# ooshyun/Speech-Enhancement-Pytorch

Measured on AMD Instinct MI355X. Metric: audio-sec/sec training, DCCRN 16kHz 2s bs32, higher is better.
Workload: dtype bf16; 1 GPU; DCCRN (kernel_num 16-32-64-128-256-256, complex LSTM 128, mask E) train step, 16 kHz 2-s clips, SI-SNR, Adam 3e-4, clip 5; per_gpu_batch=32, global_batch=32, samples_per_clip=32000, parallelism=dp1, launch=eager, inputs=resident in HBM

## Files before the change

### include/sehip.h

```cpp
#ifndef SEHIP_H
#define SEHIP_H
#include <stdint.h>

#ifdef __cplusplus
extern "C" {
#endif

const char* sehip_last_error(void);
const char* sehip_last_kernel(void);
int sehip_version(void);
int sehip_check_device(int device);

void* sehip_event_create(void);
int sehip_event_destroy(void* event);
int sehip_stream_depend(void* to_stream, void* from_stream, void* event);
int sehip_event_record(void* event, void* stream);
int sehip_stream_wait_event(void* stream, void* event);
void* sehip_stream_create(int priority_class);
int sehip_stream_destroy(void* stream);

int sehip_stft_frames(int n_samples, int win_len, int hop);
int sehip_stft_fwd(const float* wav , const float* window , int B, int N, int win_len, int hop,
                   int fft_len, float* spec , void* enc_in_bf16 , void* stream);
int sehip_istft_fwd(const float* spec, const float* mask , const float* window,
                    const float* inv_coff , int B, int T, int win_len, int hop, int fft_len, int length,
                    int masking_mode , float* frames_ws , float* wav ,
                    void* stream);
int sehip_istft_bwd(const float* dwav, const float* wav, const float* spec, const float* mask, const float* window,
                    const float* inv_coff, int B, int T, int win_len, int hop, int fft_len, int length,
                    int masking_mode, void* dmask_bf16 , void* stream);

int sehip_stft_custom_frames(int n_samples, int n_fft, int hop, int center);
int sehip_stft_custom_fwd(const float* wav, int rows, int n_samples, int n_fft, int hop, int win_length, int center,
                          float* spec, void* stream);
int sehip_istft_custom_fwd(const float* spec, int rows, int n_frames, int n_fft, int hop, int win_length, int center,
                           int length, float* frames_ws, float* wav, void* stream);

int sehip_wav_row_stats(const float* raw, const long* row_off, int rows, float* stats, void* stream);
int sehip_wav_collate(const float* raw, const long* row_off, const int* out_row, const long* out_start, const int* out_valid,
                      const float* stats, int mode, float eps, int seg, int out_rows, float* out, void* stream);

long sehip_resample_out_len(long n, int old_sr, int new_sr);
int sehip_resample_frac(const float* raw, const long* row_off, int rows, const float* kernels, int old_sr, int new_sr, int width,
                        float* out, const long* out_off, void* stream);

int sehip_sisnr_fwd(const float* est, const float* ref, int rows, int n, float* rowstat, float* loss, void* stream);
int sehip_sisdr_metric(const float* reference, const float* estimation, int rows, int n, float* ratios, float* out, void* stream);
int sehip_sisnr_bwd(const float* est, const float* ref, const float* rowstat, const float* upstream ,
                    int rows, int n, float* dest, void* stream);

int sehip_sisnr_pit_fwd(const float* est, const float* ref, int B, int S, int C, int n, float* rowstat, float* pairloss,
                        int* perm, float* loss, void* stream);
int sehip_sisnr_pit_bwd(const float* est, const float* ref, const float* rowstat, const int* perm, const float* upstream ,
                        int B, int S, int C, int n, float* dest, void* stream);

int sehip_pit_pointwise_blocks(int B, int S, int C, int n);
int sehip_pit_pointwise_fwd(const float* est, const float* ref, int B, int S, int C, int n, int mode, float* partials,
                            float* pairloss, int* perm, float* loss, void* stream);
int sehip_pit_pointwise_bwd(const float* est, const float* ref, const int* perm, const float* upstream ,
                            int B, int S, int C, int n, int mode, float* dest, void* stream);

int sehip_psa_loss_fwd(const float* enh, const float* tgt, const float* mix, long ncomplex, double* acc, float* loss, void* stream);
int sehip_psa_loss_bwd(const float* enh, const float* tgt, const float* mix, long ncomplex, const float* upstream, float* denh, void* stream);
int sehip_pointwise_loss_fwd(const float* x, const float* y, long n, int mode, double* acc_scratch, float* loss, void* stream);
int sehip_pointwise_loss_bwd(const float* x, const float* y, long n, int mode, const float* upstream, float* dx, void* stream);

int sehip_grad_sumsq(const float* grads, long n, double* sumsq_out, void* stream);
int sehip_opt_step(float* params, float* grads, float* m, float* v, long n, const double* sumsq, float max_norm,
                   float lr, float beta1, float beta2, float eps, int step, const int* step_dev ,
                   float weight_decay, int mode, float grad_scale, void* stream);
int sehip_opt_step_g(float* params, float* grads, float* m, float* v, long n, const double* sumsq, float max_norm,
                     float lr, float beta1, float beta2, float eps, int step, const int* step_dev, float weight_decay, int mode,
                     float grad_scale, const unsigned* guard, void* stream);
int sehip_opt_step_m(float* params, float* grads, float* m, float* v, long n, const double* sumsq, float max_norm, float lr,
                     float beta1, float beta2, float eps, int step, const int* step_dev, float weight_decay, int mode,
                     float grad_scale, const unsigned* guard, const float* tensor_sums, int ntensors, float* metric,
                     double* next_sumsq, float* next_tensor_sums, void* stream);
int sehip_opt_begin_g(int* counter, int value, double* sumsq, float* tensor_sums, int ntensors, const unsigned* guard, void* stream);
int sehip_counter_add(int* counter, int value, void* stream);
int sehip_zero_regions(void* p0, long b0, void* p1, long b1, void* p2, long b2, void* p3, long b3, void* stream);
int sehip_init(void);
int sehip_grad_metric(const float* grads, const long* offsets , int ntensors, long max_tensor_numel,
                      const double* sumsq,
                      float* tensor_sums , float* metric , void* stream);
int sehip_opt_begin(int* counter, int value, double* sumsq, float* tensor_sums, int ntensors, void* stream);
int sehip_grad_sumsq_acc(const float* grads, long n, double* sumsq_out, void* stream);
int sehip_grad_metric_acc(const float* grads, const long* offsets, int ntensors, long max_tensor_numel, const double* sumsq,
                          float* tensor_sums, float* metric, void* stream);

int sehip_comm_unique_id(void* id128);
int sehip_comm_init(const void* id128, int world, int rank, void** comm_out);
int sehip_allreduce_f32(void* comm, float* buf, long n, void* stream);
int sehip_allreduce_i32_max(void* comm, int* buf, long n, void* stream);
int sehip_comm_info(void* comm, int* nranks, int* rank, int* device);
int sehip_comm_destroy(void* comm);

typedef struct {
    const void* ptr;
    int32_t T;
    int32_t tlo, thi;
    int32_t F;
    int32_t C;
    int32_t pad_;
} sehip_src;

typedef struct {
    int32_t src;
    int32_t toff;
    int32_t fadd;
    int32_t coff;
} sehip_kchunk;

typedef struct {
    void* ptr;
    int32_t T, F, C;
    int32_t toff;
    int32_t fmul, fadd;
    int32_t is_f32;
    int32_t tmul;
} sehip_dst;

typedef struct {
    int32_t dst;
    int32_t coff;
    int32_t nvalid;
    int32_t pad_;
} sehip_nchunk;

typedef struct {
    sehip_src src[4];
    sehip_dst dst[2];
    const sehip_kchunk* ktab;
    const sehip_nchunk* ntab;
    const void* W;
    const float* bias;
    float* dW;
    float* dbias;
    int32_t M, N, Npad, K;
    int32_t TT, J, fmul;
    int32_t tmul;
    int32_t cv_nf, cv_fadd;
    int32_t cv_toff[2][2];
    const void* res;
    float* stats;
    int32_t stats_cr;
    int32_t cv2_nkt, cv2_nf, cv2_fadd, cv2_t0;
    int32_t w_tiled;
    int32_t wg_hint;
    int32_t dense_rows;
    int64_t dw_split_stride;
    const void* bn_dz;
    const void* bn_y;
    const float* bn_coef;
    const float* bn_bcoef;
    const float* bn_slope;
    const void* bnr_y;
    const float* bnr_coef;
    const float* bnr_slope;
    float* bnr_part;
    double* gln_stats;
    const float* gln_slope;
} sehip_gemm_desc;

int sehip_gemm_desc_size(void);
int sehip_bnr_rows(const sehip_gemm_desc* a, const sehip_gemm_desc* b );
int sehip_gemm_takes_gln_stats(const sehip_gemm_desc* desc);
int sehip_set_deterministic(int on);
int sehip_get_deterministic(void);
int sehip_gemm(const sehip_gemm_desc* desc, void* stream);
int sehip_gemm_pair(const sehip_gemm_desc* a, const sehip_gemm_desc* b, void* stream);
int sehip_conv_small_takes(const sehip_gemm_desc* a, const sehip_gemm_desc* b );
int sehip_wgrad(const sehip_gemm_desc* desc, void* stream);
int sehip_wgrad_pair(const sehip_gemm_desc* a, const sehip_gemm_desc* b, void* stream);
long sehip_wgrad_group_bytes(int n);
int sehip_wgrad_group_prepare(const sehip_gemm_desc* descs, int n, void* dev_buf, int* total_blocks);
int sehip_wgrad_group(const void* dev_buf, int n, int total_blocks, void* stream);
long sehip_wgrad_dense_group_bytes(int n);
int sehip_wgrad_dense_group_prepare(const sehip_gemm_desc* descs, int n, void* dev_buf, long dev_bytes, int* info);
int sehip_wgrad_dense_group(const void* dev_buf, int n, const int* info, float* scratch, void* stream);

int sehip_pack_bf16(const float* params, const int* table, long n, void* out_bf16, void* stream);
int sehip_pack_f32(const float* params, const int* table2 , long n, float* out, void* stream);
int sehip_pack_head(const float* params, const int* wtable, long nw, void* wout_bf16, const int* btable2, long nb, float* bout,
                    float* zero, long nz, void* stream);
int sehip_unpack_grad(const float* packed, const int* table4 , long n, float* grads, void* stream);
int sehip_unpack_grad_sums(const float* packed, const int* table4, long n, float* grads, const long* offsets, int ntensors,
                           double* sumsq, float* tensor_sums, int* counter, const unsigned* guard, void* stream);
int sehip_unpack_grad_sums_perm(const float* packed, const int* table4, const int* perm, long n, float* grads, const long* offsets,
                                int ntensors, double* sumsq, float* tensor_sums, int* counter, const unsigned* guard, void* stream);
int sehip_unpack_grad1_sums(const float* packed, const int* table1, long n, float* grads, const long* offsets, int ntensors, double* sumsq,
                            float* tensor_sums, int* counter, const unsigned* guard, void* stream);
int sehip_unpack_grad_list_sums(const float* packed, const int* list, const int* table4, long m, float* grads, const long* offsets,
                                int ntensors, double* sumsq, float* tensor_sums, void* stream);
int sehip_unpack_grad1(const float* packed, const int* table1, long n, float* grads, void* stream);
int sehip_unpack_grad_list(const float* packed, const int* list, const int* table4, long m, float* grads, void* stream);
int sehip_pack_bf16_runs(const float* params, const int* runs2 , const int* side, long n, void* out_bf16, void* stream);
int sehip_pack_bf16_runs_to(const float* params, const int* runs2 , const int* dst_run , const int* side, long n,
                            void* out_base, void* stream);

long sehip_cbn_scratch_floats(long rows, int Cr);
int sehip_cbn_stats(const void* y, long rows, int Cr, float* part, void* stream);
int sehip_cbn_finalize(const float* part, const float* Wrr, const float* Wri, const float* Wii, const float* Br,
                       const float* Bi, float* RMr, float* RMi, float* RVrr, float* RVri, float* RVii, long* nbt,
                       long rows, int Cr, float eps, float momentum, int training, float* coef , void* stream);
int sehip_cbn_finalize_n(const float* part, int nblk, const float* Wrr, const float* Wri, const float* Wii, const float* Br,
                       const float* Bi, float* RMr, float* RMi, float* RVrr, float* RVri, float* RVii, long* nbt,
                       long rows, int Cr, float eps, float momentum, int training, float* coef , void* stream);
int sehip_cbn_apply(const void* y, const float* coef, const float* slope, long rows, int Cr, void* z, void* stream);
int sehip_cbn_finalize_apply_n(const void* y, const float* part, int nblk, const float* Wrr, const float* Wri, const float* Wii,
                               const float* Br, const float* Bi, float* RMr, float* RMi, float* RVrr, float* RVri, float* RVii,
                               long* nbt, long rows, int Cr, float eps, float momentum, int training, float* coef ,
                               const float* slope, void* z, void* stream);
int sehip_cbn_bwd_reduce(const void* dz, const void* dz2 , const void* y, const float* coef, const float* slope,
                         long rows, int Cr, int F, int Tst, int tfirst, float* part, void* stream);
int sehip_cbn_bwd_finalize(const float* part, const float* coef, const float* Wrr, const float* Wri, const float* Wii,
                           long rows, int Cr, float* gWrr, float* gWri, float* gWii, float* gBr, float* gBi, float* gslope,
                           float* bcoef , void* stream);
int sehip_cbn_bwd_finalize_n(const float* part, int nblk, const float* coef, const float* Wrr, const float* Wri, const float* Wii,
                             long rows, int Cr, float* gWrr, float* gWri, float* gWii, float* gBr, float* gBi, float* gslope,
                             float* bcoef , void* stream);
int sehip_cbn_bwd_fused(const void* dz, const void* dz2 , const void* y, const float* coef, const float* Wrr, const float* Wri,
                        const float* Wii, const float* slope, long rows, int Cr, int F, int Tst, int tfirst, float* rep, float* rep_next,
                        int nrep,
                        float* gWrr, float* gWri, float* gWii, float* gBr, float* gBi, float* gslope, void* dy, void* stream);
int sehip_cbn_bwd_reduce_fin(const void* dz, const void* dz2 , const void* y, const float* coef, const float* Wrr,
                             const float* Wri, const float* Wii, const float* slope, long rows, int Cr, int F, int Tst, int tfirst,
                             float* rep, int nrep, unsigned* ticket, float* gWrr, float* gWri, float* gWii, float* gBr, float* gBi,
                             float* gslope, float* bcoef , void* stream);
int sehip_cbn_bwd_apply(const void* dz, const void* dz2, const void* y, const float* coef, const float* bcoef,
                        const float* slope, long rows, int Cr, int F, int Tst, int tfirst, void* dy, void* stream);

long sehip_rbn_scratch_floats(long rows, int Cs);
int sehip_rbn_stats(const void* y, long rows, int Cs, int Cr, float* part, void* stream);
int sehip_rbn_finalize(const float* part, const float* w_re, const float* b_re, const float* w_im, const float* b_im, float* rm_re,
                       float* rv_re, float* rm_im, float* rv_im, long* nbt_re, long* nbt_im, long rows, int Cs, int Cr, float eps,
                       float momentum, int training, float* coef, void* stream);
int sehip_rbn_finalize_s(const float* part, const float* w_re, const float* b_re, const float* w_im, const float* b_im, float* rm_re,
                         float* rv_re, float* rm_im, float* rv_im, long* nbt_re, long* nbt_im, long rows, int Cs, int Cr, float eps,
                         float momentum, int training, const float* shift, float* coef, void* stream);
int sehip_rbn_apply(const void* y, const float* coef, long rows, int Cs, int Cr, void* z, void* stream);
int sehip_rbn_bwd_reduce(const void* dz, const void* y, const float* coef, long rows, int Cs, int Cr, float* part, void* stream);
int sehip_rbn_bwd_reduce_fin(const void* dz, const void* y, const float* coef, long rows, int Cs, int Cr, float* part, unsigned* ticket,
                             float* gw_re, float* gb_re, float* gw_im, float* gb_im, float* bcoef, void* stream);
int sehip_rbn_bwd_finalize(const float* part, const float* coef, long rows, int Cs, int Cr, float* gw_re, float* gb_re, float* gw_im,
                           float* gb_im, float* bcoef, void* stream);
int sehip_rbn_bwd_apply(const void* dz, const void* y, const float* coef, const float* bcoef, long rows, int Cs, int Cr, void* dy,
                        void* stream);

int sehip_dcunet_pack_input(const float* spec, int R, int F, int T, void* out_bf16, void* stream);
int sehip_dcunet_mask_fwd(const void* z_bf16, const float* w_re, const float* w_im, const float* b_re, const float* b_im,
                          const float* spec, int R, int F, int T, int Cs, int Cr, int mode, float* mask_ws, float* out, void* stream);
int sehip_dcunet_mask_bwd(const float* dout, const float* spec, const float* mask_ws, const void* z_bf16, const float* w_re,
                          const float* w_im, int R, int F, int T, int Cs, int Cr, int mode, void* dz_bf16, float* gacc, void* stream);
int sehip_dcunet_mask_fwd_bn(const void* y_bf16, const float* coef, const float* w_re, const float* w_im, const float* b_re,
                             const float* b_im, const float* spec, int R, int F, int T, int Cs, int Cr, int mode, float* mask_ws,
                             float* out, void* stream);
long sehip_dcunet_tail_scratch_floats(int R, int F, int T, int Cs);
int sehip_dcunet_tail_bwd(const float* dout, const float* spec, float* mask_ws, const void* y_bf16, const float* coef, const float* w_re,
                          const float* w_im, int R, int F, int T, int Cs, int Cr, int mode, float* scratch, float* gw_re, float* gb_re,
                          float* gw_im, float* gb_im, float* bcoef, void* dy_bf16, float* gacc, void* stream);

int sehip_ctn_encoder_fwd(const float* wav, const float* U, const float* gamma, const float* beta, int M, int ac, int T, int N, int L,
                          float* w, void* cln_bf16, void* stream);
long sehip_ctn_codec_bwd_scratch_floats(int M, int K, int N, int L, int ac);
int sehip_ctn_encoder_bwd(const float* wav, const float* w, const void* dcln_bf16, const float* dw_dec, const float* gamma, int M, int ac,
                          int T, int N, int L, float* gacc, float* scratch, void* stream);
int sehip_ctn_gln_stats(const void* h, const float* slope, int M, int K, int C, double* stats, void* stream);
int sehip_ctn_dwconv_fwd(const void* h1, const float* slope1, const double* stats1, const float* gamma, const float* beta, const float* Wd,
                         int P, int dilation, const float* slope2, int M, int K, int C, void* h2, double* stats2, void* stream);
int sehip_ctn_gln_apply(const void* h, const float* slope, const double* stats, const float* gamma, const float* beta, int M, int K, int C,
                        void* u, void* stream);
long sehip_ctn_gln_bwd_scratch_floats(int M, int K, int C);
int sehip_ctn_gln_bwd(const void* g, const void* h, const float* slope, const double* stats, const float* gamma, const float* beta,
                      const float* Wd, int P, int dilation, int dw, int M, int K, int C, double* sums, float* gch, void* dh, float* dslope,
                      float* scratch, void* stream);
int sehip_ctn_dwconv_fwd_causal(const void* h1, const float* slope1, const double* stats1, const float* gamma, const float* beta,
                                const float* Wd, int P, int dilation, const float* slope2, int M, int K, int C, void* h2, double* stats2,
                                void* stream);
int sehip_ctn_gln_bwd_causal(const void* g, const void* h, const float* slope, const double* stats, const float* gamma, const float* beta,
                             const float* Wd, int P, int dilation, int dw, int M, int K, int C, double* sums, float* gch, void* dh,
                             float* dslope, float* scratch, void* stream);
int sehip_ctn_cln_apply(const void* h, const float* slope, const float* gamma, const float* beta, int M, int K, int C, void* u, void* stream);
int sehip_ctn_cln_dwconv_fwd(const void* h1, const float* slope1, const float* gamma, const float* beta, const float* Wd, int P,
                             int dilation, int causal, int M, int K, int C, void* h2, void* stream);
long sehip_ctn_cln_bwd_scratch_floats(int M, int K, int C);
int sehip_ctn_cln_bwd(const void* g, const void* h, const float* slope, const float* gamma, const float* beta, const float* Wd, int P,
                      int dilation, int dw, int causal, int M, int K, int C, float* gch, void* dh, float* dslope, float* scratch,
                      void* stream);
int sehip_ctns_encoder(const float* x, float* carry, const int* phase, const float* U, const float* gamma, const float* beta, int S, int ac,
                       int Kc, int N, int L, float* w, void* cln_bf16, void* stream);
int sehip_ctns_dwconv(const void* h1, void* hist, const int* phase, const int* pos, const float* slope1, const float* gamma,
                      const float* beta, const float* Wd, int P, int dilation, int S, int Kc, int C, void* h2, void* stream);
int sehip_ctns_decoder(const float* w, const void* mask_bf16, const float* V, float* tail, const int* phase, const int* pos, int S, int Kc,
                       int N, int L, int ac, int Cs, float* out, void* stream);
int sehip_ctns_advance(int* pos, int* phase, int S, int Kc, void* stream);
int sehip_dcs_analysis(const float* x, float* carry, const int* phase, const float* window, int S, int Kc, int win, int hop, float* spec,
                       float* ring, void* enc_bf16, void* enc_hist_bf16, void* stream);
int sehip_dcs_norm_hist(const void* y, const float* coef, const float* slope, void* hist, const int* phase, const int* pos, const int* end,
                        int lag, int S, int Kc, int H, int F, int Cr, void* z, void* stream);
int sehip_dcs_lstm_carry(void* h_bf16, float* c, int S, int Kc, int hidden, void* stream);
int sehip_dcs_synthesis(const float* spec, const float* ring, const float* mask, const float* window, const float* inv_coff, float* tail,
                        const int* phase, const int* pos, const int* end, int S, int Kc, int win, int hop, int mode, float* frames_ws,
                        float* out, void* stream);
int sehip_dcs_mark_end(const int* pos, int* end, int S, int extra, void* stream);
int sehip_dcs_advance(int* pos, int* phase, int S, int Kc, void* stream);
int sehip_ctn_mask_softmax_fwd(const void* score_bf16, long rows, int Cs, int N, void* out_bf16, void* stream);
int sehip_ctn_mask_softmax_bwd(const void* soft_bf16, void* g_bf16, long rows, int Cs, int N, void* stream);
int sehip_ctn_decoder_fwd(const float* w, const void* mlin_bf16, const float* V, int M, int K, int N, int L, int ac, int Cs, int T,
                          float* out, void* stream);
int sehip_ctn_decoder_bwd(const float* dout, const float* w, const void* mlin_bf16, const float* V, int M, int K, int N, int L, int ac,
                          int Cs, int T, void* dmlin_bf16, float* dw_dec, float* gacc, float* scratch, void* stream);

int sehip_lstm_fwd(const float* pre_r, const float* pre_i, const void* whh_bf16 , int B, int T, int hidden,
                   void* h_bf16, void* gates_bf16, float* c, void* stream);
int sehip_lstm_bwd(const void* dh_a_bf16, const void* dh_b_bf16, const void* whhT_bf16 ,
                   const void* gates_bf16, const float* c, int B, int T, int hidden, void* dpre_r_bf16, void* dpre_i_bf16,
                   void* stream);
int sehip_lstm_fwd_chunk(const float* pre_r, const float* pre_i, const void* whh_bf16, int B, int T, int hidden, int t0, int t1,
                         void* h_bf16, void* gates_bf16, float* c, void* stream);
int sehip_lstm_bwd_chunk(const void* dh_a_bf16, const void* dh_b_bf16, const void* whhT_bf16, const void* gates_bf16,
                         const float* c, int B, int T, int hidden, int t0, int t1, float* state, void* dpre_r_bf16,
                         void* dpre_i_bf16, void* stream);
int sehip_rlstm_fwd(const float* pre, const void* whh_bf16, int B, int T, int hidden, void* h_bf16, void* gates_bf16, float* c, void* stream);
int sehip_rlstm_bwd(const void* dh_bf16, const void* whhT_bf16, const void* gates_bf16, const float* c, int B, int T, int hidden,
                    void* dpre_bf16, void* stream);
long sehip_lstm2_gran_bytes(int B, int T, int backward);
int sehip_lstm2_sync_bytes(void);
int sehip_lstm2_fwd(const float* pre_r, const float* pre_i, const void* whh1, const void* whh2, const void* wih2, const float* bias2,
                    int B, int T, int hidden, void* h1, void* gates1, float* c1, void* h2, void* gates2, float* c2, void* gran,
                    unsigned* sync, unsigned epoch, void* stream);
int sehip_lstm2_bwd(const void* dh_a, const void* dh_b, const void* whhT1, const void* whhT2, const void* wihT2, const void* gates1,
                    const float* c1, const void* gates2, const float* c2, int B, int T, int hidden, void* dpre1_r, void* dpre1_i,
                    void* dpre2_r, void* dpre2_i, void* gran, unsigned* sync, unsigned epoch, void* stream);

int sehip_dmx_prep(const float* mix, int B, int ac, int acp, int T, int padl, int Tv, int normalize, int up, const float* kup, int width,
                   int KL, double* acc , float* ms, void* x_bf16, void* stream);
int sehip_dmx_post(const float* y, const float* ms, int B, int co, int cop, long Tf, int padl, int T, int down, const float* kdn, int width,
                   int KL, float* out, void* stream);
int sehip_dmx_post_bwd(const float* dout, const float* ms, int B, int co, int cop, long Tf, int padl, int T, int down, const float* kdn,
                       int width, int KL, void* dy_bf16, void* stream);
int sehip_dmx_gn_stats(const void* y, int B, int T, int C, int G, double* stats, void* stream);
int sehip_dmx_act_fwd(const void* y, const double* stats, const float* gamma, const float* beta, int G, float eps, int mode,
                      const float* scale, const void* resid, const void* add, int B, int T, int C, void* out, void* stream);
int sehip_dmx_act_bwd(const void* dz, const void* y, const double* stats, const float* gamma, const float* beta, int G, float eps, int mode,
                      const float* scale, int B, int T, int C, double* sums, float* gch, void* dy, void* stream);
int sehip_dmx_add(const void* a, const void* b, long n, void* out, void* stream);
int sehip_dmx_f32_to_bf16(const float* a, long n, void* out, void* stream);
int sehip_dmx_frames(int mode, const void* a, const void* b, int B, int T, int C, int nf, int W, int S, void* out, void* stream);
int sehip_dmx_lstm_sync_bytes(void);
// ... 109 lines not shown
```

### speech-enhancement-pytorch_amd/sehip/_lib.py

```python
import ctypes as C
import os

import torch

_HERE = os.path.dirname(os.path.abspath(__file__))
LIB_PATH = os.environ.get("SEHIP_LIB") or os.path.join(_HERE, "libsehip.so")


class SehipError(RuntimeError):
    pass


_lib = None

P = C.c_void_p
I = C.c_int
L = C.c_long
F = C.c_float
U = C.c_uint
D = C.c_double

_PROTOS = {
    "sehip_version": [],
    "sehip_check_device": [I],
    "sehip_set_deterministic": [I],
    "sehip_get_deterministic": [],
    "sehip_event_create": [],
    "sehip_stream_create": [C.c_int],
    "sehip_stream_destroy": [P],
    "sehip_event_destroy": [P],
    "sehip_stream_depend": [P, P, P],
    "sehip_event_record": [P, P],
    "sehip_stream_wait_event": [P, P],
    "sehip_stft_frames": [I, I, I],
    "sehip_stft_custom_frames": [I, I, I, I],
    "sehip_stft_custom_fwd": [P, I, I, I, I, I, I, P, P],
    "sehip_istft_custom_fwd": [P, I, I, I, I, I, I, I, P, P, P],
    "sehip_comm_unique_id": [P],
    "sehip_comm_init": [P, I, I, P],
    "sehip_allreduce_f32": [P, P, L, P],
    "sehip_allreduce_i32_max": [P, P, L, P],
    "sehip_comm_info": [P, P, P, P],
    "sehip_comm_destroy": [P],
    "sehip_wav_row_stats": [P, P, I, P, P],
    "sehip_wav_collate": [P, P, P, P, P, P, I, F, I, I, P, P],
    "sehip_resample_out_len": [L, I, I],
    "sehip_resample_frac": [P, P, I, P, I, I, I, P, P, P],
    "sehip_sisnr_fwd": [P, P, I, I, P, P, P],
    "sehip_sisdr_metric": [P, P, I, I, P, P, P],
    "sehip_stoi_out_len": [L, I],
    "sehip_stoi_frames": [L],
    "sehip_stoi_segment_blocks": [I, I],
    "sehip_stoi_resample": [P, P, I, L, P, I, I, I, P, P],
    "sehip_stoi_levels": [P, I, L, P, P],
    "sehip_stoi_select": [P, I, I, P, P, P],
    "sehip_stoi_bands": [P, P, I, L, P, P, P, P],
    "sehip_stoi_segments": [P, P, I, I, I, P, P, P, P],
    "sehip_sisnr_bwd": [P, P, P, P, I, I, P, P],
    "sehip_sisnr_pit_fwd": [P, P, I, I, I, I, P, P, P, P, P],
    "sehip_sisnr_pit_bwd": [P, P, P, P, P, I, I, I, I, P, P],
    "sehip_pit_pointwise_blocks": [I, I, I, I],
    "sehip_pit_pointwise_fwd": [P, P, I, I, I, I, I, P, P, P, P, P],
    "sehip_pit_pointwise_bwd": [P, P, P, P, I, I, I, I, I, P, P],
    "sehip_psa_loss_fwd": [P, P, P, L, P, P, P],
    "sehip_psa_loss_bwd": [P, P, P, L, P, P, P],
    "sehip_pointwise_loss_fwd": [P, P, L, I, P, P, P],
    "sehip_pointwise_loss_bwd": [P, P, L, I, P, P, P],
    "sehip_grad_sumsq": [P, L, P, P],
    "sehip_opt_step": [P, P, P, P, L, P, F, F, F, F, F, I, P, F, I, F, P],
    "sehip_opt_step_g": [P, P, P, P, L, P, F, F, F, F, F, I, P, F, I, F, P, P],
    "sehip_opt_step_m": [P, P, P, P, L, P, F, F, F, F, F, I, P, F, I, F, P, P, I, P, P, P, P],
    "sehip_opt_begin_g": [P, I, P, P, I, P, P],
    "sehip_counter_add": [P, I, P],
    "sehip_zero_regions": [P, L, P, L, P, L, P, L, P],
    "sehip_gemm_takes_gln_stats": [P],
    "sehip_init": [],
    "sehip_grad_metric": [P, P, I, L, P, P, P, P],
    "sehip_opt_begin": [P, I, P, P, I, P],
    "sehip_grad_sumsq_acc": [P, L, P, P],
    "sehip_grad_metric_acc": [P, P, I, L, P, P, P, P],
    "sehip_cbn_scratch_floats": [L, I],
    "sehip_stft_fwd": [P, P, I, I, I, I, I, P, P, P],
    "sehip_istft_fwd": [P, P, P, P, I, I, I, I, I, I, I, P, P, P],
    "sehip_istft_bwd": [P, P, P, P, P, P, I, I, I, I, I, I, I, P, P],
    "sehip_gemm": [P, P],
    "sehip_gemm_pair": [P, P, P],
    "sehip_wgrad": [P, P],
    "sehip_wgrad_pair": [P, P, P],
    "sehip_bnr_rows": [P, P],
    "sehip_cbn_bwd_finalize_n": [P, I, P, P, P, P, L, I, P, P, P, P, P, P, P, P],
    "sehip_wgrad_group_bytes": [I],
    "sehip_wgrad_group_prepare": [P, I, P, P],
    "sehip_wgrad_group": [P, I, I, P],
    "sehip_wgrad_dense_group_bytes": [I],
    "sehip_wgrad_dense_group_prepare": [P, I, P, L, P],
    "sehip_wgrad_dense_group": [P, I, P, P, P],
    "sehip_gemm_desc_size": [],
    "sehip_conv_small_takes": [P, P],
    "sehip_pack_bf16": [P, P, L, P, P],
    "sehip_pack_f32": [P, P, L, P, P],
    "sehip_pack_head": [P, P, L, P, P, L, P, P, L, P],
    "sehip_unpack_grad": [P, P, L, P, P],
    "sehip_unpack_grad_sums": [P, P, L, P, P, I, P, P, P, P, P],
    "sehip_unpack_grad_sums_perm": [P, P, P, L, P, P, I, P, P, P, P, P],
    "sehip_unpack_grad1": [P, P, L, P, P],
    "sehip_unpack_grad1_sums": [P, P, L, P, P, I, P, P, P, P, P],
    "sehip_unpack_grad_list_sums": [P, P, P, L, P, P, I, P, P, P],
    "sehip_unpack_grad_list": [P, P, P, L, P, P],
    "sehip_pack_bf16_runs": [P, P, P, L, P, P],
    "sehip_pack_bf16_runs_to": [P, P, P, P, L, P, P],
    "sehip_cbn_stats": [P, L, I, P, P],
    "sehip_cbn_finalize": [P, P, P, P, P, P, P, P, P, P, P, P, L, I, F, F, I, P, P],
    "sehip_cbn_finalize_n": [P, I, P, P, P, P, P, P, P, P, P, P, P, L, I, F, F, I, P, P],
    "sehip_cbn_apply": [P, P, P, L, I, P, P],
    "sehip_cbn_finalize_apply_n": [P, P, I, P, P, P, P, P, P, P, P, P, P, P, L, I, F, F, I, P, P, P, P],
    "sehip_cbn_bwd_reduce": [P, P, P, P, P, L, I, I, I, I, P, P],
    "sehip_cbn_bwd_finalize": [P, P, P, P, P, L, I, P, P, P, P, P, P, P, P],
    "sehip_cbn_bwd_apply": [P, P, P, P, P, P, L, I, I, I, I, P, P],
    "sehip_cbn_bwd_fused": [P, P, P, P, P, P, P, P, L, I, I, I, I, P, P, I, P, P, P, P, P, P, P, P],
    "sehip_cbn_bwd_reduce_fin": [P, P, P, P, P, P, P, P, L, I, I, I, I, P, I, P, P, P, P, P, P, P, P, P],
    "sehip_rbn_scratch_floats": [L, I],
    "sehip_rbn_stats": [P, L, I, I, P, P],
    "sehip_rbn_finalize": [P, P, P, P, P, P, P, P, P, P, P, L, I, I, F, F, I, P, P],
    "sehip_rbn_finalize_s": [P, P, P, P, P, P, P, P, P, P, P, L, I, I, F, F, I, P, P, P],
    "sehip_rbn_apply": [P, P, L, I, I, P, P],
    "sehip_rbn_bwd_reduce": [P, P, P, L, I, I, P, P],
    "sehip_rbn_bwd_reduce_fin": [P, P, P, L, I, I, P, P, P, P, P, P, P, P],
    "sehip_rbn_bwd_finalize": [P, P, L, I, I, P, P, P, P, P, P],
    "sehip_rbn_bwd_apply": [P, P, P, P, L, I, I, P, P],
    "sehip_dcunet_pack_input": [P, I, I, I, P, P],
    "sehip_dcunet_mask_fwd": [P, P, P, P, P, P, I, I, I, I, I, I, P, P, P],
    "sehip_dcunet_mask_bwd": [P, P, P, P, P, P, I, I, I, I, I, I, P, P, P],
    "sehip_dcunet_mask_fwd_bn": [P, P, P, P, P, P, P, I, I, I, I, I, I, P, P, P],
    "sehip_dcunet_tail_scratch_floats": [I, I, I, I],
    "sehip_dcunet_tail_bwd": [P, P, P, P, P, P, P, I, I, I, I, I, I, P, P, P, P, P, P, P, P, P],
    "sehip_ctn_encoder_fwd": [P, P, P, P, I, I, I, I, I, P, P, P],
    "sehip_ctn_encoder_bwd": [P, P, P, P, P, I, I, I, I, I, P, P, P],
    "sehip_ctn_codec_bwd_scratch_floats": [I, I, I, I, I],
    "sehip_ctn_gln_stats": [P, P, I, I, I, P, P],
    "sehip_ctn_dwconv_fwd": [P, P, P, P, P, P, I, I, P, I, I, I, P, P, P],
    "sehip_ctn_gln_apply": [P, P, P, P, P, I, I, I, P, P],
    "sehip_ctn_gln_bwd": [P, P, P, P, P, P, P, I, I, I, I, I, I, P, P, P, P, P, P],
    "sehip_ctn_gln_bwd_scratch_floats": [I, I, I],
    "sehip_ctn_dwconv_fwd_causal": [P, P, P, P, P, P, I, I, P, I, I, I, P, P, P],
    "sehip_ctn_gln_bwd_causal": [P, P, P, P, P, P, P, I, I, I, I, I, I, P, P, P, P, P, P],
    "sehip_ctn_cln_apply": [P, P, P, P, I, I, I, P, P],
    "sehip_ctn_cln_dwconv_fwd": [P, P, P, P, P, I, I, I, I, I, I, P, P],
    "sehip_ctn_cln_bwd_scratch_floats": [I, I, I],
    "sehip_ctn_cln_bwd": [P, P, P, P, P, P, I, I, I, I, I, I, I, P, P, P, P, P],
    "sehip_ctn_mask_softmax_fwd": [P, L, I, I, P, P],
    "sehip_ctn_mask_softmax_bwd": [P, P, L, I, I, P],
    "sehip_ctn_decoder_fwd": [P, P, P, I, I, I, I, I, I, I, P, P],
    "sehip_ctn_decoder_bwd": [P, P, P, P, I, I, I, I, I, I, I, P, P, P, P, P],
    "sehip_ctns_encoder": [P, P, P, P, P, P, I, I, I, I, I, P, P, P],
    "sehip_ctns_dwconv": [P, P, P, P, P, P, P, P, I, I, I, I, I, P, P],
    "sehip_ctns_decoder": [P, P, P, P, P, P, I, I, I, I, I, I, P, P],
    "sehip_ctns_advance": [P, P, I, I, P],
    "sehip_dcs_analysis": [P, P, P, P, I, I, I, I, P, P, P, P, P],
    "sehip_dcs_norm_hist": [P, P, P, P, P, P, P, I, I, I, I, I, I, P, P],
    "sehip_dcs_lstm_carry": [P, P, I, I, I, P],
    "sehip_dcs_synthesis": [P, P, P, P, P, P, P, P, P, I, I, I, I, I, P, P, P],
    "sehip_dcs_mark_end": [P, P, I, I, P],
    "sehip_dcs_advance": [P, P, I, I, P],
    "sehip_dmx_prep": [P, I, I, I, I, I, I, I, I, P, I, I, P, P, P, P],
    "sehip_dmx_post": [P, P, I, I, I, L, I, I, I, P, I, I, P, P],
    "sehip_dmx_post_bwd": [P, P, I, I, I, L, I, I, I, P, I, I, P, P],
    "sehip_dmx_gn_stats": [P, I, I, I, I, P, P],
    "sehip_dmx_act_fwd": [P, P, P, P, I, F, I, P, P, P, I, I, I, P, P],
    "sehip_dmx_act_bwd": [P, P, P, P, P, I, F, I, P, I, I, I, P, P, P, P],
    "sehip_dmx_add": [P, P, L, P, P],
    "sehip_dmx_f32_to_bf16": [P, L, P, P],
    "sehip_dmx_frames": [I, P, P, I, I, I, I, I, I, P, P],
    "sehip_dmx_lstm_sync_bytes": [],
    "sehip_dmx_lstm_fwd": [P, P, I, I, I, P, P, P, P],
    "sehip_dmx_lstm_bwd": [P, P, P, P, I, I, I, P, P, P, P],
    "sehip_dmx_attn_fwd": [P, I, I, I, I, I, I, P, P],
    "sehip_dmx_attn_bwd_scratch_floats": [I, I, I],
    "sehip_dmx_attn_bwd": [P, P, I, I, I, I, I, I, P, P, P],
    "sehip_lstm_fwd": [P, P, P, I, I, I, P, P, P, P],
    "sehip_lstm_bwd": [P, P, P, P, P, I, I, I, P, P, P],
    "sehip_rlstm_fwd": [P, P, I, I, I, P, P, P, P],
    "sehip_rlstm_bwd": [P, P, P, P, I, I, I, P, P],
    "sehip_lstm2_gran_bytes": [I, I, I],
    "sehip_lstm2_sync_bytes": [],
    "sehip_lstm2_fwd": [P, P, P, P, P, P, I, I, I, P, P, P, P, P, P, P, P, U, P],
    "sehip_lstm2_bwd": [P, P, P, P, P, P, P, P, P, I, I, I, P, P, P, P, P, P, U, P],
    "sehip_lstm_fwd_chunk": [P, P, P, I, I, I, I, I, P, P, P, P],
    "sehip_lstm_bwd_chunk": [P, P, P, P, P, I, I, I, I, I, P, P, P, P],
    "sehip_wun_bn_scratch_floats": [L, I],
    "sehip_wun_enc0_wgrad_scratch_floats": [I, I, I],
    "sehip_wun_out_bwd_scratch_floats": [L, I],
    "sehip_wun_enc0_fwd": [P, P, P, I, I, I, P, P],
    "sehip_wun_enc0_wgrad": [P, P, I, I, I, P, P, P, P],
    "sehip_wun_bn_stats": [P, L, I, P, P],
    "sehip_wun_bn_finalize": [P, P, P, P, P, P, P, L, I, F, F, I, P, P],
    "sehip_wun_bn_apply": [P, P, L, I, P, P],
    "sehip_wun_bn_apply_up2": [P, P, I, I, I, P, P],
    "sehip_wun_up2_bwd": [P, I, I, I, P, P],
    "sehip_wun_bn_bwd_reduce": [P, P, P, P, L, I, P, P],
    "sehip_wun_bn_bwd_finalize": [P, P, L, I, P, P, P, P],
    "sehip_wun_bn_bwd_apply": [P, P, P, P, P, L, I, P, P],
    "sehip_wun_out_fwd": [P, P, P, P, L, I, P, P],
    "sehip_wun_out_bwd": [P, P, P, P, P, L, I, P, P, P, P, P],
    "sehip_rsm_sum_scratch_floats": [L, I],
    "sehip_rsm_counter_next": [P, P, P],
    "sehip_rsm_features": [P, I, I, I, I, P, P],
    "sehip_rsm_pack_w": [P, I, I, I, I, P, P],
    "sehip_rsm_gemm_nt": [P, I, P, I, I, I, I, I, P, P, I, P],
    "sehip_rsm_gemm_tn": [P, I, P, I, I, I, I, I, I, P, I, P],
    "sehip_rsm_rnn_fwd": [I, P, P, P, P, P, P, I, I, I, I, U, U, P, I, U, F, P],
    "sehip_rsm_rnn_bwd": [I, P, P, P, P, P, P, I, I, I, I, U, U, P, I, U, F, P],
    "sehip_rsm_colsum": [P, I, P, P, L, I, P, P],
    "sehip_rsm_colsum_finalize": [P, L, I, P, P, P, P, P, P],
    "sehip_rsm_bn_apply": [P, P, L, I, P, P],
    "sehip_rsm_bn_bwd_apply": [P, P, P, P, L, I, P, P],
    "sehip_rsm_mask_fwd": [P, P, I, I, I, I, I, I, P, P],
    "sehip_rsm_mask_bwd": [P, P, P, I, I, I, I, I, I, P, P],
    "sehip_rsm_elman_fwd": [P, P, P, P, I, I, I, I, P],
    "sehip_rsm_elman_bwd": [P, P, P, P, I, I, I, I, P],
    "sehip_rsm_gemm_nt_head": [P, I, P, I, I, I, I, I, P, P, I, P, I, P],
    "sehip_rsm_mask_bwd_sigmoid": [P, P, P, I, I, I, I, I, I, P, P],
    "sehip_ha_fir_fwd": [P, L, L, P, I, I, P, P, P],
    "sehip_ha_fir_adj": [P, L, L, P, I, I, P, P, P],
    "sehip_ha_compressor_ws_doubles": [L, L, I],
    "sehip_ha_compressor_fwd": [P, L, L, I, D, D, D, D, I, P, P, P, P],
    "sehip_ha_compressor_bwd": [P, P, P, L, I, P, P],
    "sehip_has_state_bytes": [L, I, I, I],
    "sehip_has_fir": [P, L, I, I, P, I, I, I, P, P, P, P, P, P],
    "sehip_has_compress": [P, L, I, I, I, P, P, D, D, D, D, I, P, P, P, P],
    "sehip_has_advance": [P, P, P, L, I, P],
    "sehip_rss_delay_frames": [I, I, I],
    "sehip_rss_state_bytes": [L, I, I, I, I],
    "sehip_rss_feed": [P, L, I, I, P, I, I, I, P, P, L, P, P],
    "sehip_rss_advance": [P, L, I, P],
    "sehip_unet_features": [P, I, I, I, I, I, P, P],
    "sehip_unet_mask_fwd": [P, P, P, I, I, I, I, I, P, P],
    "sehip_unet_mask_bwd": [P, P, I, I, I, I, I, P, P],
    "sehip_unet_bn_finalize": [P, P, P, P, P, P, P, L, I, I, F, F, I, P, P],
    "sehip_unet_bn_act": [P, P, L, I, U, U, P, I, U, F, P, P],
    "sehip_unet_bn_act_pool": [P, P, I, I, I, I, U, U, P, I, U, F, P, P, P],
    "sehip_unet_bn_bwd_reduce": [P, P, P, P, I, I, I, I, U, U, P, I, U, F, P, P],
    "sehip_unet_bn_bwd_apply": [P, P, P, P, P, I, I, I, I, U, U, P, I, U, F, P, P],
}
_RESTYPE = {"sehip_resample_out_len": C.c_long, "sehip_stoi_out_len": C.c_long,"sehip_ha_compressor_ws_doubles": C.c_long, "sehip_has_state_bytes": C.c_long, "sehip_rss_delay_frames": C.c_long, "sehip_rss_state_bytes": C.c_long, "sehip_rsm_sum_scratch_floats": C.c_long, "sehip_wun_bn_scratch_floats": C.c_long, "sehip_wun_enc0_wgrad_scratch_floats": C.c_long, "sehip_wun_out_bwd_scratch_floats": C.c_long,
            "sehip_lstm2_gran_bytes": C.c_long, "sehip_dmx_attn_bwd_scratch_floats": C.c_long, "sehip_ctn_codec_bwd_scratch_floats": C.c_long, "sehip_ctn_gln_bwd_scratch_floats": C.c_long, "sehip_ctn_cln_bwd_scratch_floats": C.c_long, "sehip_wgrad_group_bytes": C.c_long, "sehip_wgrad_dense_group_bytes": C.c_long, "sehip_cbn_scratch_floats": C.c_long, "sehip_rbn_scratch_floats": C.c_long, "sehip_dcunet_tail_scratch_floats": C.c_long, "sehip_event_create": C.c_void_p, "sehip_stream_create": C.c_void_p}


def lib():
    global _lib
    if _lib is None:
        if not os.path.exists(LIB_PATH):
            raise SehipError(
                f"{LIB_PATH} is missing: build it with `python {os.path.join(_HERE, 'build.py')}` "
                "(hipcc --offload-arch=gfx950). There is no CPU/PyTorch fallback for the HIP path.")
        _lib = C.CDLL(LIB_PATH)
        _lib.sehip_last_error.restype = C.c_char_p
        _lib.sehip_last_kernel.restype = C.c_char_p
        for name, args in _PROTOS.items():
            fn = getattr(_lib, name, None)
            if fn is None:
                continue
            fn.argtypes = args
            fn.restype = _RESTYPE.get(name, C.c_int)
    return _lib


def declared_symbols():
    return ["sehip_last_error", "sehip_last_kernel"] + list(_PROTOS)


def check(status, what=""):
    if status != 0:
        msg = lib().sehip_last_error().decode()
        raise SehipError(f"{what}: status {status}: {msg}")


def call(name, *args):
    fn = getattr(lib(), name)
    check(fn(*args), name)


def ptr(t):
    if t is None:
        return None
    assert t.is_contiguous(), "libsehip needs contiguous tensors"
    return t.data_ptr()


import threading

_tls = threading.local()


def stream():
    h = getattr(_tls, "handle", None)
    if h is not None:
        return h
    return torch.cuda.current_stream().cuda_stream


class stream_scope:

    def __enter__(self):
        self._prev = getattr(_tls, "handle", None)
        _tls.handle = torch.cuda.current_stream().cuda_stream
        return self

    def __exit__(self, *exc):
        cached = _tls.handle
        _tls.handle = self._prev
        if exc[0] is None and os.environ.get("SEHIP_DEBUG_STREAMS") and torch.cuda.current_stream().cuda_stream != cached:
            raise SehipError("stream_scope: torch's current stream changed inside the scope; library calls went to the stream "
                             "that was current at entry")
        return False


def require_gpu(t, what):
    if not t.is_cuda:
        raise SehipError(f"{what}: tensor is on {t.device}; the HIP path needs a gfx950 GPU (no CPU fallback)")
```

### speech-enhancement-pytorch_amd/sehip/csrc/loss.hip

```cpp
#include "common.h"

#define EPS 1e-8f

__device__ __forceinline__ float sisnr_residual(float x, float alpha, float s) {
    float t = alpha * s;
    asm volatile("" : "+v"(t));
    return x - t;
}

__global__ __launch_bounds__(1024) void sisnr_fwd_kernel(const float* __restrict__ est, const float* __restrict__ ref,
                                                        int n, int rows, float4* __restrict__ rowstat) {
    __shared__ float red[16];
    const int r = blockIdx.x;
    const float* x = est + (size_t)r * n;
    const float* s = ref + (size_t)r * n;
    float xs = 0.f, ss = 0.f;
    const int n4 = n >> 2;
    const float4* x4 = reinterpret_cast<const float4*>(x);
    const float4* s4 = reinterpret_cast<const float4*>(s);
    const bool vec = ((n & 3) == 0) && ((((uintptr_t)x | (uintptr_t)s) & 15) == 0);
    if (vec) {
        for (int i = threadIdx.x; i < n4; i += 1024) {
            float4 a = x4[i], b = s4[i];
            xs += a.x * b.x + a.y * b.y + a.z * b.z + a.w * b.w;
            ss += b.x * b.x + b.y * b.y + b.z * b.z + b.w * b.w;
        }
    } else {
        for (int i = threadIdx.x; i < n; i += 1024) { xs += x[i] * s[i]; ss += s[i] * s[i]; }
    }
    xs = block_sum<16>(xs, red);
    ss = block_sum<16>(ss, red);
    const float alpha = xs / (ss + EPS);
    float et = 0.f, en = 0.f, es = 0.f;
    if (vec) {
        for (int i = threadIdx.x; i < n4; i += 1024) {
            float4 a = x4[i], b = s4[i];
            float t0 = alpha * b.x, t1 = alpha * b.y, t2 = alpha * b.z, t3 = alpha * b.w;
            float e0 = sisnr_residual(a.x, alpha, b.x), e1 = sisnr_residual(a.y, alpha, b.y), e2 = sisnr_residual(a.z, alpha, b.z),
                  e3 = sisnr_residual(a.w, alpha, b.w);
            et += t0 * t0 + t1 * t1 + t2 * t2 + t3 * t3;
            en += e0 * e0 + e1 * e1 + e2 * e2 + e3 * e3;
            es += e0 * b.x + e1 * b.y + e2 * b.z + e3 * b.w;
        }
    } else {
        for (int i = threadIdx.x; i < n; i += 1024) {
            float t = alpha * s[i], e = sisnr_residual(x[i], alpha, s[i]);
            et += t * t; en += e * e; es += e * s[i];
        }
    }
    et = block_sum<16>(et, red);
    en = block_sum<16>(en, red);
    es = block_sum<16>(es, red);
    if (threadIdx.x == 0) {
        const float ratio = et / (en + EPS);
        const float l = 10.f * log10f(ratio + EPS);
        const float c = -(1.0f / rows) * 10.f / (2.302585092994046f * (ratio + EPS));
        const float q = et / ((en + EPS) * (en + EPS));
        const float a = c * (-2.f * q);
        const float b = c * (2.f * alpha * ss / ((ss + EPS) * (en + EPS)) + 2.f * q * es / (ss + EPS));
        rowstat[r] = make_float4(a, b, l, alpha);
    }
}

__global__ void sisnr_finalize_kernel(const float4* __restrict__ rowstat, int rows, float* __restrict__ loss) {
    float acc = 0.f;
    for (int i = threadIdx.x; i < rows; i += 64) acc += rowstat[i].z;
    acc = wave_sum(acc);
    if (threadIdx.x == 0) loss[0] = -acc / rows;
}

__global__ __launch_bounds__(256) void sisnr_bwd_kernel(const float* __restrict__ est, const float* __restrict__ ref,
                                                        const float4* __restrict__ rowstat, const float* __restrict__ upstream,
                                                        int n, float* __restrict__ dest) {
    const int r = blockIdx.y;
    const float4 st = rowstat[r];
    const float up = upstream ? upstream[0] : 1.f;
    const float a = st.x * up, b = st.y * up, alpha = st.w;
    const size_t base = (size_t)r * n;
    for (int i = blockIdx.x * 256 + threadIdx.x; i < n; i += gridDim.x * 256) {
        const float s = ref[base + i];
        dest[base + i] = a * sisnr_residual(est[base + i], alpha, s) + b * s;
    }
}

#define SDR_EPS 1.1920929e-07f
__global__ __launch_bounds__(256) void sisdr_metric_kernel(const float* __restrict__ ref, const float* __restrict__ est, int n,
                                                           float* __restrict__ ratios) {
    __shared__ float red[4];
    const int r = blockIdx.x;
    const float* s = ref + (size_t)r * n;
    const float* x = est + (size_t)r * n;
    float xs = 0.f, ss = 0.f;
    for (int i = threadIdx.x; i < n; i += 256) { xs += x[i] * s[i]; ss += s[i] * s[i]; }
    xs = block_sum<4>(xs, red);
    ss = block_sum<4>(ss, red);
    const float alpha = xs / (ss + SDR_EPS);
    float et = 0.f, en = 0.f;
    for (int i = threadIdx.x; i < n; i += 256) {
        const float t = alpha * s[i], e = x[i] - t;
        et += t * t; en += e * e;
    }
    et = block_sum<4>(et, red);
    en = block_sum<4>(en, red);
    if (threadIdx.x == 0) ratios[r] = et / (en + SDR_EPS);
}

__global__ void sisdr_metric_finalize_kernel(const float* __restrict__ ratios, int rows, float* __restrict__ out) {
    float acc = 0.f;
    for (int i = threadIdx.x; i < rows; i += 64) acc += ratios[i];
    acc = wave_sum(acc);
    if (threadIdx.x == 0) out[0] = 10.f * log10f(acc / rows + SDR_EPS);
}

extern "C" int sehip_sisdr_metric(const float* reference, const float* estimation, int rows, int n, float* ratios, float* out,
                                  void* stream) {
    SEHIP_REQUIRE(rows > 0 && n > 0, "sisdr_metric: empty input (rows=%d n=%d)", rows, n);
    hipStream_t st = (hipStream_t)stream;
    sisdr_metric_kernel<<<rows, 256, 0, st>>>(reference, estimation, n, ratios);
    sisdr_metric_finalize_kernel<<<1, 64, 0, st>>>(ratios, rows, out);
    SEHIP_CHECK_LAUNCH("sisdr_metric");
    return 0;
}

extern "C" int sehip_sisnr_fwd(const float* est, const float* ref, int rows, int n, float* rowstat, float* loss,
                               void* stream) {
    SEHIP_REQUIRE(rows > 0 && n > 0, "sisnr_fwd: empty input (rows=%d n=%d)", rows, n);
    hipStream_t st = (hipStream_t)stream;
    sisnr_fwd_kernel<<<rows, 1024, 0, st>>>(est, ref, n, rows, (float4*)rowstat);
    sisnr_finalize_kernel<<<1, 64, 0, st>>>((const float4*)rowstat, rows, loss);
    SEHIP_CHECK_LAUNCH("sisnr_fwd");
    return 0;
}

extern "C" int sehip_sisnr_bwd(const float* est, const float* ref, const float* rowstat, const float* upstream, int rows,
                               int n, float* dest, void* stream) {
    SEHIP_REQUIRE(rows > 0 && n > 0, "sisnr_bwd: empty input (rows=%d n=%d)", rows, n);
    dim3 grid(cdiv(n, 256 * 8), rows);
    sisnr_bwd_kernel<<<grid, 256, 0, (hipStream_t)stream>>>(est, ref, (const float4*)rowstat, upstream, n, dest);
    SEHIP_CHECK_LAUNCH("sisnr_bwd");
    return 0;
}

#define PIT_MAXS 6
__global__ __launch_bounds__(256) void sisnr_pit_rows_kernel(const float* __restrict__ est, const float* __restrict__ ref, int B, int S,
                                                             int C, int n, float4* __restrict__ rowstat) {
    __shared__ float red[4];
    const int R = B * C;
    const int r = blockIdx.x, pair = blockIdx.y;
    const int i = pair / S, j = pair - i * S;
    const int b = r / C, c = r - b * C;
    const float* x = est + (((size_t)b * S + i) * C + c) * n;
    const float* s = ref + (((size_t)b * S + j) * C + c) * n;
    float xs = 0.f, ss = 0.f;
    for (int k = threadIdx.x; k < n; k += 256) { xs += x[k] * s[k]; ss += s[k] * s[k]; }
    xs = block_sum<4>(xs, red);
    ss = block_sum<4>(ss, red);
    const float alpha = xs / (ss + EPS);
    float et = 0.f, en = 0.f, es = 0.f;
    for (int k = threadIdx.x; k < n; k += 256) {
        const float t = alpha * s[k], e = sisnr_residual(x[k], alpha, s[k]);
        et += t * t; en += e * e; es += e * s[k];
    }
    et = block_sum<4>(et, red);
    en = block_sum<4>(en, red);
    es = block_sum<4>(es, red);
    if (threadIdx.x == 0) {
        const float ratio = et / (en + EPS);
        const float l = 10.f * log10f(ratio + EPS);
        const float cc = -(1.0f / ((float)S * (float)R)) * 10.f / (2.302585092994046f * (ratio + EPS));
        const float q = et / ((en + EPS) * (en + EPS));
        const float a = cc * (-2.f * q);
        const float bb = cc * (2.f * alpha * ss / ((ss + EPS) * (en + EPS)) + 2.f * q * es / (ss + EPS));
        rowstat[(size_t)pair * R + r] = make_float4(a, bb, l, alpha);
    }
}

__device__ void pit_best_permutation(const float* m, int S, int* best) {
    int cur[PIT_MAXS];
    for (int k = 0; k < S; ++k) cur[k] = best[k] = k;
    float lmin = 1e9f;
    for (;;) {
        float l = 0.f;
        for (int j = 0; j < S; ++j) l += m[cur[j] * S + j];
        if (lmin > l) {
            lmin = l;
            for (int k = 0; k < S; ++k) best[k] = cur[k];
        }
        int k = S - 2;
        while (k >= 0 && cur[k] > cur[k + 1]) --k;
        if (k < 0) break;
        int l2 = S - 1;
        while (cur[l2] < cur[k]) --l2;
        int t = cur[k]; cur[k] = cur[l2]; cur[l2] = t;
        for (int a = k + 1, b = S - 1; a < b; ++a, --b) { t = cur[a]; cur[a] = cur[b]; cur[b] = t; }
    }
}

__global__ void sisnr_pit_select_kernel(const float4* __restrict__ rowstat, int R, int S, float* __restrict__ pairloss,
                                        int* __restrict__ perm, float* __restrict__ loss) {
    __shared__ float m[PIT_MAXS * PIT_MAXS];
    for (int pair = 0; pair < S * S; ++pair) {
        float acc = 0.f;
        for (int r = threadIdx.x; r < R; r += 64) acc += rowstat[(size_t)pair * R + r].z;
        acc = wave_sum(acc);
        if (threadIdx.x == 0) { m[pair] = -acc / R; pairloss[pair] = -acc / R; }
    }
    __syncthreads();
    if (threadIdx.x != 0) return;
    int best[PIT_MAXS];
    pit_best_permutation(m, S, best);
    float tot = 0.f;
    for (int j = 0; j < S; ++j) { perm[j] = best[j]; tot += m[best[j] * S + j]; }
    loss[0] = tot / S;
}

__global__ __launch_bounds__(256) void sisnr_pit_bwd_kernel(const float* __restrict__ est, const float* __restrict__ ref,
                                                            const float4* __restrict__ rowstat, const int* __restrict__ perm,
                                                            const float* __restrict__ upstream, int B, int S, int C, int n,
                                                            float* __restrict__ dest) {
    const int R = B * C;
    const int r = blockIdx.y, i = blockIdx.z;
    int j = 0;
    for (int k = 0; k < S; ++k)
        if (perm[k] == i) j = k;
    const int b = r / C, c = r - b * C;
    const float4 st = rowstat[(size_t)(i * S + j) * R + r];
    const float up = upstream ? upstream[0] : 1.f;
    const float a = st.x * up, bb = st.y * up, alpha = st.w;
    const size_t xb = (((size_t)b * S + i) * C + c) * n, sb = (((size_t)b * S + j) * C + c) * n;
    for (int k = blockIdx.x * 256 + threadIdx.x; k < n; k += gridDim.x * 256) {
        const float s = ref[sb + k];
        dest[xb + k] = a * sisnr_residual(est[xb + k], alpha, s) + bb * s;
    }
}

extern "C" int sehip_sisnr_pit_fwd(const float* est, const float* ref, int B, int S, int C, int n, float* rowstat, float* pairloss,
                                   int* perm, float* loss, void* stream) {
    SEHIP_REQUIRE(B > 0 && C > 0 && n > 0 && S >= 1 && S <= PIT_MAXS, "sisnr_pit_fwd: bad shape (B=%d S=%d C=%d n=%d; S <= %d)", B, S,
                  C, n, PIT_MAXS);
    hipStream_t st = (hipStream_t)stream;
    sisnr_pit_rows_kernel<<<dim3(B * C, S * S), 256, 0, st>>>(est, ref, B, S, C, n, (float4*)rowstat);
    sisnr_pit_select_kernel<<<1, 64, 0, st>>>((const float4*)rowstat, B * C, S, pairloss, perm, loss);
    SEHIP_CHECK_LAUNCH("sisnr_pit_fwd");
    return 0;
}

extern "C" int sehip_sisnr_pit_bwd(const float* est, const float* ref, const float* rowstat, const int* perm, const float* upstream,
                                   int B, int S, int C, int n, float* dest, void* stream) {
    SEHIP_REQUIRE(B > 0 && C > 0 && n > 0 && S >= 1 && S <= PIT_MAXS, "sisnr_pit_bwd: bad shape (B=%d S=%d C=%d n=%d)", B, S, C, n);
    dim3 grid(cdiv(n, 256 * 8), B * C, S);
    sisnr_pit_bwd_kernel<<<grid, 256, 0, (hipStream_t)stream>>>(est, ref, (const float4*)rowstat, perm, upstream, B, S, C, n, dest);
    SEHIP_CHECK_LAUNCH("sisnr_pit_bwd");
    return 0;
}

__global__ __launch_bounds__(256) void pointwise_loss_fwd_kernel(const float* __restrict__ x, const float* __restrict__ y, long n,
                                                                 int mode, double* __restrict__ acc) {
    __shared__ float red[4];
    float a = 0.f;
    for (long i = blockIdx.x * 256L + threadIdx.x; i < n; i += gridDim.x * 256L) {
        const float d = x[i] - y[i];
        a += mode == 0 ? fabsf(d) : d * d;
    }
    a = block_sum<4>(a, red);
    if (threadIdx.x == 0) atomicAdd(acc, (double)a);
}

__global__ void pointwise_loss_finalize_kernel(const double* __restrict__ acc, long n, float* __restrict__ loss) {
    loss[0] = (float)(acc[0] / (double)n);
}

__global__ __launch_bounds__(256) void pointwise_loss_bwd_kernel(const float* __restrict__ x, const float* __restrict__ y, long n,
                                                                 int mode, const float* __restrict__ upstream,
                                                                 float* __restrict__ dx) {
    const float up = (upstream ? upstream[0] : 1.f) / (float)n;
    for (long i = blockIdx.x * 256L + threadIdx.x; i < n; i += gridDim.x * 256L) {
        const float d = x[i] - y[i];
        dx[i] = mode == 0 ? (d > 0.f ? up : (d < 0.f ? -up : 0.f)) : 2.f * d * up;
    }
}

__device__ __forceinline__ float psa_residual(float2 e, float2 t, float2 m, float& ae) {
    const float am = tanhf(m.y / (m.x + 1e-9f)), at = tanhf(t.y / (t.x + 1e-9f));
    ae = sqrtf(e.y * e.y + e.x * e.x);
    return ae - sqrtf(t.y * t.y + t.x * t.x) * cosf(at - am);
}

__global__ __launch_bounds__(256) void psa_loss_fwd_kernel(const float2* __restrict__ enh, const float2* __restrict__ tgt,
                                                           const float2* __restrict__ mix, long n, double* __restrict__ acc) {
    __shared__ float red[4];
    float a = 0.f;
    for (long i = blockIdx.x * 256L + threadIdx.x; i < n; i += gridDim.x * 256L) {
        float ae;
        const float d = psa_residual(enh[i], tgt[i], mix[i], ae);
        a += d * d;
    }
    a = block_sum<4>(a, red);
    if (threadIdx.x == 0) atomicAdd(acc, (double)a);
}

__global__ __launch_bounds__(256) void psa_loss_bwd_kernel(const float2* __restrict__ enh, const float2* __restrict__ tgt,
                                                           const float2* __restrict__ mix, long n, const float* __restrict__ upstream,
                                                           float2* __restrict__ denh) {
    const float up = 2.f * (upstream ? upstream[0] : 1.f) / (float)n;
    for (long i = blockIdx.x * 256L + threadIdx.x; i < n; i += gridDim.x * 256L) {
        const float2 e = enh[i];
        float ae;
        const float d = psa_residual(e, tgt[i], mix[i], ae);
        const float k = ae > 0.f ? up * d / ae : 0.f;
        denh[i] = make_float2(k * e.x, k * e.y);
    }
}

extern "C" int sehip_psa_loss_fwd(const float* enh, const float* tgt, const float* mix, long ncomplex, double* acc, float* loss, void* stream) {
    SEHIP_REQUIRE(ncomplex > 0 && enh && tgt && mix, "psa_loss_fwd: bad arguments (n=%ld)", ncomplex);
    hipStream_t st = (hipStream_t)stream;
    hipError_t e = hipMemsetAsync(acc, 0, sizeof(double), st);
    SEHIP_REQUIRE(e == hipSuccess, "psa_loss_fwd: memset failed: %s", hipGetErrorString(e));
    int grid = cdiv(ncomplex, 256 * 8);
    if (grid > 1024) grid = 1024;
    if (sehip_deterministic()) grid = 1;
    psa_loss_fwd_kernel<<<grid, 256, 0, st>>>((const float2*)enh, (const float2*)tgt, (const float2*)mix, ncomplex, acc);
    pointwise_loss_finalize_kernel<<<1, 1, 0, st>>>(acc, ncomplex, loss);
    SEHIP_CHECK_LAUNCH("psa_loss_fwd");
    return 0;
}

extern "C" int sehip_psa_loss_bwd(const float* enh, const float* tgt, const float* mix, long ncomplex, const float* upstream, float* denh,
                                  void* stream) {
    SEHIP_REQUIRE(ncomplex > 0 && enh && tgt && mix && denh, "psa_loss_bwd: bad arguments (n=%ld)", ncomplex);
    int grid = cdiv(ncomplex, 256 * 4);
    if (grid > 2048) grid = 2048;
    psa_loss_bwd_kernel<<<grid, 256, 0, (hipStream_t)stream>>>((const float2*)enh, (const float2*)tgt, (const float2*)mix, ncomplex, upstream,
                                                             (float2*)denh);
    SEHIP_CHECK_LAUNCH("psa_loss_bwd");
    return 0;
}

extern "C" int sehip_pointwise_loss_fwd(const float* x, const float* y, long n, int mode, double* acc, float* loss,
                                        void* stream) {
    SEHIP_REQUIRE(n > 0 && (mode == 0 || mode == 1), "pointwise_loss_fwd: bad arguments (n=%ld mode=%d)", n, mode);
    hipStream_t st = (hipStream_t)stream;
    hipError_t e = hipMemsetAsync(acc, 0, sizeof(double), st);
    SEHIP_REQUIRE(e == hipSuccess, "pointwise_loss_fwd: memset failed: %s", hipGetErrorString(e));
    int grid = cdiv(n, 256 * 16);
    if (grid > 1024) grid = 1024;
    if (sehip_deterministic()) grid = 1;
    pointwise_loss_fwd_kernel<<<grid, 256, 0, st>>>(x, y, n, mode, acc);
    pointwise_loss_finalize_kernel<<<1, 1, 0, st>>>(acc, n, loss);
    SEHIP_CHECK_LAUNCH("pointwise_loss_fwd");
    return 0;
}

extern "C" int sehip_pointwise_loss_bwd(const float* x, const float* y, long n, int mode, const float* upstream, float* dx,
                                        void* stream) {
    SEHIP_REQUIRE(n > 0 && (mode == 0 || mode == 1), "pointwise_loss_bwd: bad arguments (n=%ld mode=%d)", n, mode);
    int grid = cdiv(n, 256 * 8);
    if (grid > 2048) grid = 2048;
    pointwise_loss_bwd_kernel<<<grid, 256, 0, (hipStream_t)stream>>>(x, y, n, mode, upstream, dx);
    SEHIP_CHECK_LAUNCH("pointwise_loss_bwd");
    return 0;
}

#define PITPW_THREADS 256
#define PITPW_CHUNK 2048L
#define PITPW_MAXBLOCKS 1024L
#define PITPW_MAXROWS (1L << 20)
#define PITPW_MAXN (0x7fffffff - 64 * 4 * PITPW_THREADS)

static long pitpw_chunk(long rows, long n) {
    long chunk = PITPW_CHUNK;
    while (rows * ((n + chunk - 1) / chunk) > PITPW_MAXBLOCKS && chunk < n) chunk *= 2;
    return chunk;
}

extern "C" int sehip_pit_pointwise_blocks(int B, int S, int C, int n) {
    if (B <= 0 || C <= 0 || n <= 0 || S < 1 || S > PIT_MAXS || (long)B * C > PITPW_MAXROWS || n > PITPW_MAXN) return 0;
    const long rows = (long)B * C, chunk = pitpw_chunk(rows, n);
    return (int)(rows * ((n + chunk - 1) / chunk));
}

template <int MODE>
__device__ __forceinline__ float pitpw_term(float e, float t) {
    const float d = e - t;
    return MODE == 0 ? fabsf(d) : d * d;
}

template <int S, int MODE, bool VEC>
__global__ __launch_bounds__(PITPW_THREADS) void pit_pointwise_pairs_kernel(const float* __restrict__ est, const float* __restrict__ ref,
                                                                            int C, int n, int chunk, float* __restrict__ partials) {
    __shared__ float red[PITPW_THREADS / 64][S * S];
    const int r = blockIdx.x, b = r / C, c = r - b * C;
    const size_t row0 = ((size_t)b * S * C + c) * n, sstride = (size_t)C * n;
    const int k0 = blockIdx.y * chunk;
    const int k1 = n - k0 < chunk ? n : k0 + chunk;
    float acc[S * S];
#pragma unroll
    for (int p = 0; p < S * S; ++p) acc[p] = 0.f;
    if (VEC) {
        for (int k = k0 + 4 * (int)threadIdx.x; k < k1; k += 4 * PITPW_THREADS) {
            float4 e[S], t[S];
#pragma unroll
            for (int i = 0; i < S; ++i) {
                e[i] = *reinterpret_cast<const float4*>(est + row0 + i * sstride + k);
                t[i] = *reinterpret_cast<const float4*>(ref + row0 + i * sstride + k);
            }
#pragma unroll
            for (int i = 0; i < S; ++i)
#pragma unroll
                for (int j = 0; j < S; ++j)
                    acc[i * S + j] += (pitpw_term<MODE>(e[i].x, t[j].x) + pitpw_term<MODE>(e[i].y, t[j].y)) +
                                      (pitpw_term<MODE>(e[i].z, t[j].z) + pitpw_term<MODE>(e[i].w, t[j].w));
        }
    } else {
        for (int k = k0 + (int)threadIdx.x; k < k1; k += PITPW_THREADS) {
            float e[S], t[S];
#pragma unroll
            for (int i = 0; i < S; ++i) {
                e[i] = est[row0 + i * sstride + k];
                t[i] = ref[row0 + i * sstride + k];
            }
#pragma unroll
            for (int i = 0; i < S; ++i)
#pragma unroll
                for (int j = 0; j < S; ++j) acc[i * S + j] += pitpw_term<MODE>(e[i], t[j]);
        }
    }
    const int w = threadIdx.x >> 6;
#pragma unroll
    for (int p = 0; p < S * S; ++p) {
        const float v = wave_sum(acc[p]);
        if ((threadIdx.x & 63) == 0) red[w][p] = v;
    }
// ... 128 lines not shown
```

### speech-enhancement-pytorch_amd/sehip/csrc/stft.hip

```cpp
#include "common.h"

#include "fft512.h"
#include "mask.h"

__global__ __launch_bounds__(256) void stft_fwd_kernel(const float* __restrict__ wav, const float* __restrict__ window,
                                                       int B, int N, int T, int win, int hop,
                                                       float2* __restrict__ spec, unsigned* __restrict__ enc_in) {
    const int lane = threadIdx.x & 63;
    const int frame = blockIdx.x * 4 + (threadIdx.x >> 6);
    if (frame >= B * T) return;
    const int b = frame / T, t = frame - b * T;
    FftTw tw;
    fft_twiddles<-1>(tw, lane);
    float re[8], im[8];
    const int pad = win - hop;
    const float* x = wav + (size_t)b * N;
#pragma unroll
    for (int r = 0; r < 8; ++r) {
        const int n = lane + 64 * r;
        const int s = t * hop + n - pad;
        float v = 0.f;
        if (n < win && s >= 0 && s < N) v = x[s] * window[n];
        re[r] = v; im[r] = 0.f;
    }
    fft512_wave<-1>(re, im, tw, lane);
    __shared__ float2 srow[4][264 + 33];
    __shared__ unsigned senc[4][256];
    const int w = threadIdx.x >> 6;
    const int k0 = 8 * brev6(lane);
    constexpr int brev3[8] = {0, 4, 2, 6, 1, 5, 3, 7};
    if (k0 <= 256) {
#pragma unroll
        for (int j = 0; j < 8; ++j) {
            const int k = k0 + brev3[j];
            if (k <= 256) {
                srow[w][k + (k >> 3)] = make_float2(re[j], im[j]);
                if (k >= 1) senc[w][k - 1] = pack_bf2(re[j], im[j]);
            }
        }
    }
    __builtin_amdgcn_fence(__ATOMIC_RELEASE, "wavefront");
    __builtin_amdgcn_wave_barrier();
    __builtin_amdgcn_fence(__ATOMIC_ACQUIRE, "wavefront");
    float2* so = spec + (size_t)frame * NBIN;
    unsigned* eo = enc_in + (size_t)frame * 256;
#pragma unroll
    for (int j = 0; j < 4; ++j) {
        const int k = lane + 64 * j;
        so[k] = srow[w][k + (k >> 3)];
    }
    if (lane == 0) so[256] = srow[w][256 + 32];
    *reinterpret_cast<uint4*>(eo + 4 * lane) = *reinterpret_cast<const uint4*>(&senc[w][4 * lane]);
}

__global__ __launch_bounds__(256) void istft_frames_kernel(const float2* __restrict__ spec, const float2* __restrict__ mask,
                                                           const float* __restrict__ window, int nframes, int win, int mode,
                                                           float* __restrict__ frames) {
    const int lane = threadIdx.x & 63;
    const int frame = blockIdx.x * 4 + (threadIdx.x >> 6);
    if (frame >= nframes) return;
    FftTw tw;
    fft_twiddles<1>(tw, lane);
    float re[8], im[8];
    const float2* sp = spec + (size_t)frame * NBIN;
    const float2* mk = mask + (size_t)frame * 256;
#pragma unroll
    for (int r = 0; r < 8; ++r) {
        const int k = lane + 64 * r;
        float er = 0.f, ei = 0.f;
        if (k >= 1 && k <= 256) {
            const float2 z = sp[k];
            const float2 m = mk[k - 1];
            apply_mask(mode, z.x, z.y, m.x, m.y, er, ei);
        }
        re[r] = er; im[r] = ei;
    }
    fft512_wave<1>(re, im, tw, lane);
    const int n0 = 8 * brev6(lane);
    constexpr int brev3[8] = {0, 4, 2, 6, 1, 5, 3, 7};
    float u[8];
    float s1 = 0.f, s2 = 0.f;
#pragma unroll
    for (int j = 0; j < 8; ++j) {
        const int n = n0 + brev3[j];
        u[brev3[j]] = re[j];
        if (n < win) { s1 += re[j]; s2 += (n & 1) ? -re[j] : re[j]; }
    }
    s1 = wave_sum(s1);
    s2 = wave_sum(s2);
    const float c = 1.0f / (float)(FFT_N + win);
    float* fo = frames + (size_t)frame * win;
    if (n0 + 8 <= win && (win & 3) == 0) {
        float o[8];
#pragma unroll
        for (int q = 0; q < 8; ++q) {
            const int n = n0 + q;
            const float corr = c * (s1 + ((n & 1) ? -s2 : s2));
            o[q] = window[n] * (1.0f / 256.0f) * (u[q] - corr);
        }
        *reinterpret_cast<float4*>(fo + n0) = make_float4(o[0], o[1], o[2], o[3]);
        *reinterpret_cast<float4*>(fo + n0 + 4) = make_float4(o[4], o[5], o[6], o[7]);
        return;
    }
#pragma unroll
    for (int q = 0; q < 8; ++q) {
        const int n = n0 + q;
        if (n < win) {
            const float corr = c * (s1 + ((n & 1) ? -s2 : s2));
            fo[n] = window[n] * (1.0f / 256.0f) * (u[q] - corr);
        }
    }
}

__global__ __launch_bounds__(256) void istft_ola_kernel(const float* __restrict__ frames, const float* __restrict__ inv_coff,
                                                        int T, int win, int hop, int length, float* __restrict__ wav) {
    const int b = blockIdx.y;
    const int pad = win - hop;
    for (int i = blockIdx.x * 256 + threadIdx.x; i < length; i += gridDim.x * 256) {
        const int s = i + pad;
        int t_hi = s / hop;
        int t_lo = (s - win + hop) / hop;
        if (s - win + 1 <= 0) t_lo = 0;
        if (t_hi > T - 1) t_hi = T - 1;
        float acc = 0.f;
        for (int t = t_lo; t <= t_hi; ++t) acc += frames[((size_t)b * T + t) * win + (s - t * hop)];
        acc *= inv_coff[i];
        wav[(size_t)b * length + i] = fminf(1.f, fmaxf(-1.f, acc));
    }
}

__global__ __launch_bounds__(256) void istft_bwd_kernel(const float* __restrict__ dwav, const float* __restrict__ wav,
                                                        const float* __restrict__ inv_coff, const float* __restrict__ window,
                                                        const float2* __restrict__ spec, const float2* __restrict__ mask,
                                                        int B, int T, int win, int hop, int length, int mode,
                                                        unsigned* __restrict__ dmask_bf16) {
    const int lane = threadIdx.x & 63;
    const int frame = blockIdx.x * 4 + (threadIdx.x >> 6);
    if (frame >= B * T) return;
    const int b = frame / T, t = frame - b * T;
    FftTw tw;
    fft_twiddles<-1>(tw, lane);
    const int pad = win - hop;
    float re[8], im[8];
    float s1 = 0.f, s2 = 0.f;
#pragma unroll
    for (int r = 0; r < 8; ++r) {
        const int n = lane + 64 * r;
        const int i = t * hop + n - pad;
        float v = 0.f;
        if (n < win && i >= 0 && i < length) {
            const size_t o = (size_t)b * length + i;
            const float y = wav[o];
            if (y > -1.f && y < 1.f) v = dwav[o] * inv_coff[i] * window[n] * (1.0f / 256.0f);
        }
        re[r] = v; im[r] = 0.f;
        s1 += v; s2 += (n & 1) ? -v : v;
    }
    s1 = wave_sum(s1);
    s2 = wave_sum(s2);
    const float c = 1.0f / (float)(FFT_N + win);
#pragma unroll
    for (int r = 0; r < 8; ++r) {
        const int n = lane + 64 * r;
        if (n < win) re[r] -= c * (s1 + ((n & 1) ? -s2 : s2));
    }
    const float2* sp = spec + (size_t)frame * NBIN;
    const float2* mk = mask + (size_t)frame * 256;
    float2 spv[4], mkv[4];
#pragma unroll
    for (int j = 0; j < 4; ++j) { spv[j] = sp[1 + lane + 64 * j]; mkv[j] = mk[lane + 64 * j]; }
    fft512_wave<-1>(re, im, tw, lane);
    __shared__ float2 ssp[4][256 + 32], smk[4][256 + 32];
    __shared__ unsigned sdm[4][256];
    const int w = threadIdx.x >> 6;
#pragma unroll
    for (int j = 0; j < 4; ++j) {
        const int i = lane + 64 * j;
        ssp[w][i + (i >> 3)] = spv[j];
        smk[w][i + (i >> 3)] = mkv[j];
    }
    __builtin_amdgcn_fence(__ATOMIC_RELEASE, "wavefront");
    __builtin_amdgcn_wave_barrier();
    __builtin_amdgcn_fence(__ATOMIC_ACQUIRE, "wavefront");
    const int k0 = 8 * brev6(lane);
    constexpr int brev3[8] = {0, 4, 2, 6, 1, 5, 3, 7};
    if (k0 <= 256) {
#pragma unroll
        for (int j = 0; j < 8; ++j) {
            const int k = k0 + brev3[j];
            if (k < 1 || k > 256) continue;
            const float dr = re[j], di = im[j];
            const int i = k - 1;
            const float2 z = ssp[w][i + (i >> 3)];
            const float2 m = smk[w][i + (i >> 3)];
            float gmr, gmi;
            mask_grad(mode, z.x, z.y, m.x, m.y, dr, di, gmr, gmi);
            sdm[w][i] = pack_bf2(gmr, gmi);
        }
    }
    __builtin_amdgcn_fence(__ATOMIC_RELEASE, "wavefront");
    __builtin_amdgcn_wave_barrier();
    __builtin_amdgcn_fence(__ATOMIC_ACQUIRE, "wavefront");
    unsigned* dm = dmask_bf16 + (size_t)frame * 256;
    *reinterpret_cast<uint4*>(dm + 4 * lane) = *reinterpret_cast<const uint4*>(&sdm[w][4 * lane]);
}

static int check_stft_cfg(const char* who, int win, int hop, int fft) {
    SEHIP_REQUIRE(fft == FFT_N, "%s: only fft_len 512 is built (got %d)", who, fft);
    SEHIP_REQUIRE(win > 0 && win <= FFT_N && (win % 2) == 0, "%s: win_len must be even and <= 512 (got %d)", who, win);
    SEHIP_REQUIRE(hop > 0 && hop <= win, "%s: bad hop %d", who, hop);
    return 0;
}

extern "C" int sehip_stft_frames(int n_samples, int win, int hop) { return (n_samples + 2 * (win - hop) - win) / hop + 1; }

extern "C" int sehip_stft_fwd(const float* wav, const float* window, int B, int N, int win, int hop, int fft, float* spec,
                              void* enc_in_bf16, void* stream) {
    if (int e = check_stft_cfg("stft_fwd", win, hop, fft)) return e;
    SEHIP_REQUIRE(B > 0 && N > 0, "stft_fwd: empty input");
    const int T = sehip_stft_frames(N, win, hop);
    SEHIP_REQUIRE(T > 0, "stft_fwd: input shorter than one frame");
    stft_fwd_kernel<<<cdiv((long)B * T, 4), 256, 0, (hipStream_t)stream>>>(wav, window, B, N, T, win, hop, (float2*)spec,
                                                                           (unsigned*)enc_in_bf16);
    SEHIP_CHECK_LAUNCH("stft_fwd");
    return 0;
}

extern "C" int sehip_istft_fwd(const float* spec, const float* mask, const float* window, const float* inv_coff, int B,
                               int T, int win, int hop, int fft, int length, int mode, float* frames_ws, float* wav,
                               void* stream) {
    if (int e = check_stft_cfg("istft_fwd", win, hop, fft)) return e;
    SEHIP_REQUIRE(B > 0 && T > 0 && length > 0, "istft_fwd: empty input");
    SEHIP_REQUIRE(mode >= 0 && mode <= 2, "istft_fwd: masking mode must be 0(E) 1(C) 2(R)");
    SEHIP_REQUIRE(length <= (T - 1) * hop + win - (win - hop), "istft_fwd: length %d exceeds the synthesised signal", length);
    hipStream_t st = (hipStream_t)stream;
    istft_frames_kernel<<<cdiv((long)B * T, 4), 256, 0, st>>>((const float2*)spec, (const float2*)mask, window, B * T, win,
                                                             mode, frames_ws);
    dim3 grid(cdiv(length, 256 * 4), B);
    istft_ola_kernel<<<grid, 256, 0, st>>>(frames_ws, inv_coff, T, win, hop, length, wav);
    SEHIP_CHECK_LAUNCH("istft_fwd");
    return 0;
}

extern "C" int sehip_istft_bwd(const float* dwav, const float* wav, const float* spec, const float* mask,
                               const float* window, const float* inv_coff, int B, int T, int win, int hop, int fft,
                               int length, int mode, void* dmask_bf16, void* stream) {
    if (int e = check_stft_cfg("istft_bwd", win, hop, fft)) return e;
    SEHIP_REQUIRE(B > 0 && T > 0 && length > 0, "istft_bwd: empty input");
    SEHIP_REQUIRE(mode >= 0 && mode <= 2, "istft_bwd: masking mode must be 0(E) 1(C) 2(R)");
    istft_bwd_kernel<<<cdiv((long)B * T, 4), 256, 0, (hipStream_t)stream>>>(dwav, wav, inv_coff, window, (const float2*)spec,
                                                                            (const float2*)mask, B, T, win, hop, length, mode,
                                                                            (unsigned*)dmask_bf16);
    SEHIP_CHECK_LAUNCH("istft_bwd");
    return 0;
}
```

### speech-enhancement-pytorch_amd/sehip/model/dccrn.py

```python
import os
import numpy as np
import torch
from torch import nn

from .. import plan, ops
from .._lib import SehipError
from .flat import FlatModule, _Node

class DCCRN(FlatModule):
    plan_name = "DCCRN"

    def __init__(self, rnn_layers=2, rnn_units=128, win_len=400, win_inc=100, fft_len=512, length=16384, win_type="hann",
                 masking_mode="E", use_clstm=True, use_cbn=True, kernel_size=5, kernel_num=[16, 32, 64, 128, 256, 256],
                 *args, **kwargs):
        super().__init__()
        self.cfg = cfg = plan.DCCRNConfig(rnn_layers=rnn_layers, rnn_units=rnn_units, win_len=win_len, win_inc=win_inc,
                                          fft_len=fft_len, length=length, win_type=win_type, masking_mode=masking_mode,
                                          use_clstm=use_clstm, use_cbn=use_cbn, kernel_size=kernel_size,
                                          kernel_num=list(kernel_num))
        self.win_len, self.win_inc, self.fft_len, self.rnn_units = win_len, win_inc, fft_len, rnn_units
        self.masking_mode, self.kernel_num = masking_mode, cfg.kernel_num
        self.static = self._static_for(cfg)
        self.grad_range_hook = None

        an, sy, win = _stft_bases(win_len, fft_len, win_type)
        self.stft = _Node()
        self.stft.register_buffer("weight", torch.from_numpy(an[:, None, :]))
        self.istft = _Node()
        self.istft.register_buffer("weight", torch.from_numpy(sy[:, None, :]))
        self.istft.register_buffer("window", torch.from_numpy(win[None, :, None]))
        self.istft.register_buffer("enframe", torch.eye(win_len)[:, None, :])
        self._build_flat(list_roots=("encoder", "decoder"))
        self.reset_parameters()

    def _static_for(self, cfg, deterministic=False):
        switches = tuple(os.environ.get(k) for k in ("SEHIP_NO_FUSE_STATS", "SEHIP_NO_FUSE_STATS64", "SEHIP_NO_FUSE_STATS32", "SEHIP_DEC_SPLIT"))
        key = (tuple(cfg.kernel_num), cfg.rnn_layers, cfg.rnn_units, cfg.win_len, cfg.win_inc, cfg.fft_len, cfg.length, cfg.masking_mode, str(cfg.win_type), bool(cfg.use_cbn), bool(cfg.use_clstm), switches,
               bool(deterministic))
        return self._static(key, lambda: plan.DCCRNStatic(cfg, deterministic=deterministic))

    def reset_parameters(self):
        h = self.cfg.hid
        with torch.no_grad():
            for name, p in self._params:
                leaf = name.split(".")[-1]
                if "conv.weight" in name:
                    p.normal_(0.0, 0.05)
                elif "conv.bias" in name or leaf in ("Br", "Bi") or name.endswith(".1.bias"):
                    p.zero_()
                elif leaf in ("Wrr", "Wii") or name.endswith(".1.weight"):
                    p.fill_(1.0)
                elif leaf == "Wri":
                    p.uniform_(-0.9, 0.9)
                elif name.endswith("2.weight"):
                    p.fill_(0.25)
                elif "lstm" in name or name.startswith("enhance."):
                    p.uniform_(-1.0 / h ** 0.5, 1.0 / h ** 0.5)
                elif "trans" in name or name.startswith("tranform."):
                    p.uniform_(-1.0 / h ** 0.5, 1.0 / h ** 0.5)
                else:
                    raise KeyError(name)
            for name, node, leaf in self._buffers_named:
                getattr(node, leaf).fill_(1.0 if leaf in ("RVrr", "RVii", "running_var") else 0.0)
            self._nbt.zero_()

    def workspace(self, batch, nsample):
        dev = self._require_gpu()
        if self._tables is None:
            self._tables = plan.DeviceTables(self.static, dev)
        return self._lru_get((batch, nsample), lambda: plan.DCCRNWorkspace(self.static, self._tables, batch, nsample, dev))

    def set_deterministic(self, on=True):
        on = bool(on)
        if on == self.static.deterministic:
            return self
        self.static = self._static_for(self.cfg, deterministic=on)
        self._tables = None
        for ws in list(self._ws.values()):
            ws.close()
        self._ws.clear()
        self._last_ws = None
        return self

    step_guard_early = True

    def step_guard(self):
        ws = getattr(self, "_last_ws", None)
        return ws.l2_sync[0:1] if ws is not None and hasattr(ws, "l2_sync") else None

    def check_health(self):
        from ..distrib import global_flag
        ws = getattr(self, "_last_ws", None)
        if ws is None:
            return global_flag(False, self._flat.device if self._flat is not None else None)
        lost = bool(ws.check_lstm_handoffs(recover=True, global_flag=global_flag))
        self._note_graph_epoch(ws)
        return lost

    def _run_forward(self, wav):
        ws = self.workspace(wav.shape[0], wav.shape[-1])
        self._last_ws = ws
        ws.generation += 1
        x = wav.reshape(wav.shape[0], wav.shape[-1]).contiguous().float()
        ws.forward(x, self._flat, self._bflat, self._nbt, training=self.training)
        return ws

    def _output(self, ws, x):
        return ws.wav.view(x.shape[0], 1, -1).clone()

    def _run_backward(self, ws, grad_out):
        if not self.training:
            raise SehipError("DCCRN.backward in eval mode (running-statistics BatchNorm) is not built")
        g = grad_out.reshape(ws.B, ws.length).contiguous().float()
        hook = self.grad_range_hook if not (self._grads_live and self._params[0][1].grad is not None) else None
        tail = self._tail_for_backward()
        self._backward_into_flat(lambda dst: ws.backward(g, self._flat, dst, range_ready=hook, tail=tail))
        self._tail_mark(tail)

    def forward(self, inputs, lens=None):
        if inputs.dim() == 2:
            inputs = inputs.unsqueeze(1)
        return self._run_plan(inputs, torch.is_grad_enabled() and self.training)

    def get_params(self, weight_decay=0.0):
        weights, biases = [], []
        for name, p in self.named_parameters():
            (biases if "bias" in name else weights).append(p)
        return [{"params": weights, "weight_decay": weight_decay}, {"params": biases, "weight_decay": 0.0}]


def _stft_bases(win_len, fft_len, win_type="hann"):
    n = np.arange(win_len, dtype=np.float64)[None, :]
    k = np.arange(fft_len // 2 + 1, dtype=np.float64)[:, None]
    ang = 2.0 * np.pi * k * n / fft_len
    basis = np.concatenate([np.cos(ang), -np.sin(ang)], axis=0)
    win = ops.window_of(win_type, win_len).astype(np.float64)
    return ((basis * win).astype(np.float32), (np.linalg.pinv(basis).T * win).astype(np.float32), win.astype(np.float32))
```

### speech-enhancement-pytorch_amd/sehip/model/flat.py

```python
import os
from collections import OrderedDict

import numpy as np
import torch
from torch import nn

from .._lib import SehipError, stream_scope

_STATIC_CACHE = {}


class _Node(nn.Module):

    def __getitem__(self, idx):
        return getattr(self, str(idx))


def _clone_state_hook(module, state_dict, prefix, local_metadata):
    for k in list(state_dict.keys()):
        state_dict[k] = state_dict[k].detach().clone()
    return state_dict


class _PlanFunction(torch.autograd.Function):

    @staticmethod
    def forward(ctx, model, x, anchor):
        ctx.model = model
        ctx.ws = model._run_forward(x)
        ctx.generation = ctx.ws.generation
        return model._output(ctx.ws, x)

    @staticmethod
    def backward(ctx, grad_out):
        if ctx.generation != ctx.ws.generation or ctx.ws.closed:
            raise SehipError(f"{ctx.model.plan_name}.backward: the workspace of this forward was overwritten by a later forward of the same "
                             "shape (or evicted); run backward before the next forward of that shape")
        with stream_scope():
            ctx.model._run_backward(ctx.ws, grad_out)
        return None, None, None


class _EvalGuard(torch.autograd.Function):

    @staticmethod
    def forward(ctx, x, name):
        ctx.name = name
        return x.view_as(x)

    @staticmethod
    def backward(ctx, g):
        raise SehipError(f"{ctx.name}.backward in eval mode: the backward pass is built for batch statistics only (call model.train())")


class FlatModule(nn.Module):
    plan_name = None
    ws_cache_default = 4

    def _static(self, key, make):
        key = (type(self), key)
        if key not in _STATIC_CACHE:
            _STATIC_CACHE[key] = make()
        return _STATIC_CACHE[key]

    def _build_flat(self, list_roots=()):
        L = self.static.layout
        self._flat = torch.zeros(L.n_params)
        self._gflat = self._tables = None
        self._bflat = torch.zeros(max(L.n_buffers, 1))
        self._nbt = torch.zeros(len(L.nbt_names), dtype=torch.int64)
        self._ws = OrderedDict()
        self._ws_cap = max(1, int(os.environ.get("SEHIP_WS_CACHE", self.ws_cache_default)))
        self.storage_epoch = 0
        self._anchor = None
        self._grads_live = False
        self._tail_sink, self._tail_done = None, False
        self._tail_counted = self._tail_dirty = False
        for name in list_roots:
            setattr(self, name, nn.ModuleList())
        self._params, self._buffers_named, self._nbt_named = [], [], []
        for name, shape, kind in L.specs:
            parts = name.split(".")
            node = self._descend(parts[:-1])
            if kind == "param":
                off, _ = L.param_off[name]
                p = nn.Parameter(self._flat[off:off + int(np.prod(shape))].view(shape))
                node.register_parameter(parts[-1], p)
                self._params.append((name, p))
            elif kind == "buffer":
                off, _ = L.buffer_off[name]
                node.register_buffer(parts[-1], self._bflat[off:off + int(np.prod(shape))].view(shape))
                self._buffers_named.append((name, node, parts[-1]))
            else:
                node.register_buffer(parts[-1], self._nbt[L.nbt_idx[name]])
                self._nbt_named.append((name, node, parts[-1]))
        self._register_state_dict_hook(_clone_state_hook)

    def _tail_for_backward(self):
        accumulating = self._grads_live and self._params[0][1].grad is not None
        if accumulating or getattr(self, "grad_range_hook", None) is not None:
            return None
        return self._tail_sink

    def _tail_mark(self, tail):
        if tail is not None:
            self._tail_done = self._tail_counted = self._tail_dirty = True
        else:
            self._tail_done = False

    def _descend(self, parts):
        node = self
        for key in parts:
            if isinstance(node, nn.ModuleList):
                while len(node) <= int(key):
                    node.append(_Node())
                node = node[int(key)]
            else:
                if not hasattr(node, key):
                    node.add_module(key, _Node())
                node = getattr(node, key)
        return node

    def _apply(self, fn, *a, **k):
        super()._apply(fn, *a, **k)
        L = self.static.layout
        dev = self._params[0][1].device
        flat = torch.zeros(L.n_params, device=dev)
        for name, p in self._params:
            off, shape = L.param_off[name]
            v = flat[off:off + p.numel()].view(shape)
            v.copy_(p.data)
            p.data = v
            p.grad = None
        bflat = torch.zeros(max(L.n_buffers, 1), device=dev)
        for name, node, leaf in self._buffers_named:
            off, shape = L.buffer_off[name]
            v = bflat[off:off + int(np.prod(shape))].view(shape)
            v.copy_(getattr(node, leaf))
            node._buffers[leaf] = v
        nbt = torch.zeros(len(L.nbt_names), dtype=torch.int64, device=dev)
        for name, node, leaf in self._nbt_named:
            i = L.nbt_idx[name]
            nbt[i] = getattr(node, leaf).to(torch.int64)
            node._buffers[leaf] = nbt[i]
        self._flat, self._bflat, self._nbt = flat, bflat, nbt
        for ws in self._ws.values():
            ws.close()
        self._gflat, self._tables, self._ws, self._anchor, self._grads_live = None, None, OrderedDict(), None, False
        self.storage_epoch += 1
        return self

    @property
    def flat_params(self):
        return self._flat

    @property
    def flat_grads(self):
        if self._gflat is None or self._gflat.device != self._flat.device:
            self._gflat = torch.zeros_like(self._flat)
        return self._gflat

    def bind_grads(self):
        L = self.static.layout
        g = self.flat_grads
        for name, p in self._params:
            off, shape = L.param_off[name]
            p.grad = g[off:off + p.numel()].view(shape)

    def _require_gpu(self):
        dev = self._flat.device
        if dev.type != "cuda":
            raise SehipError(f"{self.plan_name} parameters are on {dev}: the HIP path needs a gfx950 GPU (no CPU fallback); "
                             "call model.to('cuda') first")
        return dev

    def _grad_anchor(self, device):
        if self._anchor is None or self._anchor.device != device:
            self._anchor = torch.zeros(1, device=device, requires_grad=True)
        return self._anchor

    def _output(self, ws, x):
        return ws.out.clone()

    def _run_plan(self, x, train_step, **forward_only):
        if not x.is_cuda:
            raise SehipError(f"{self.plan_name}.forward got a CPU tensor: the HIP path needs a gfx950 GPU (no CPU fallback)")
        if train_step:
            return _PlanFunction.apply(self, x, self._grad_anchor(x.device))
        return self._output(self._run_forward(x, **forward_only), x)

    def _eval_guarded(self, out):
        return _EvalGuard.apply(out.requires_grad_(True), self.plan_name)

    def _lru_get(self, key, make):
        ws = self._ws.get(key)
        if ws is None:
            while len(self._ws) >= self._ws_cap:
                victim = next((k for k, w in self._ws.items() if not w.pinned), None)
                if victim is None:
                    break
                self._ws.pop(victim).close()
            ws = self._ws[key] = make()
        else:
            self._ws.move_to_end(key)
        return ws

    def _note_graph_epoch(self, ws):
        ge = getattr(ws, "graph_epoch", 0)
        if ws is not None and ge != getattr(ws, "_graph_epoch_seen", 0):
            ws._graph_epoch_seen = ge
            self.storage_epoch += 1

    def _backward_into_flat(self, run):
        accumulate = self._grads_live and self._params[0][1].grad is not None
        if accumulate:
            tmp = torch.empty_like(self.flat_grads)
            run(tmp)
            self.flat_grads.add_(tmp)
        else:
            run(self.flat_grads)
        self.bind_grads()
        self._grads_live = True
```

### speech-enhancement-pytorch_amd/sehip/plan.py

```python
import ctypes as C
import os
import math

import numpy as np
import torch

from . import _lib
from ._lib import call, ptr, stream, SehipError
from . import ops
from .gemmdesc import (BF16, CSrc, CDst, CGemmDesc, ParamLayout, Arena, enc_entry, npad_of, round_up, dense_ntab, wide_chunks, pad_ktab,
                       bind_chunk_table, upload_chunk_table, row_ptr, fill_desc, wgrad_twin, UnpackTable, check_unpack_coverage)
from .workspace import Buf, GemmDeviceTables, GemmWorkspace, gather_ordered_unpack_table


FUSE_SKIP_GRAD = not os.environ.get("SEHIP_NO_FUSE_SKIP")
FUSE_ENC0_BN_WGRAD = FUSE_SKIP_GRAD and bool(os.environ.get("SEHIP_FUSE_ENC0_BN"))
BWD_REPLICAS = int(os.environ.get("SEHIP_BWD_REPLICAS", "8"))
PARALLEL_HEAD = not os.environ.get("SEHIP_NO_PARALLEL_HEAD")
L2_GRAPH_EPOCH = 65535
TILE_WEIGHTS = not any(os.environ.get(k) for k in ("SEHIP_NO_CONV_V3", "SEHIP_NO_PATCH", "SEHIP_NO_TILE_WEIGHTS"))


class DCCRNConfig:

# ... 327 lines not shown
            last = j == 5
            for p in (0, 1):
                ds = (-1, 0, 1) if p == 0 else (0, 1)
                rows = []
                cols_i, cols_n = [], []
                for kt in (0, 1):
                    for d in ds:
                        kf = p + 2 - 2 * d
                        base_t = (1 if last else 0) - kt
                        rows += wide_chunks(0, base_t + (0 if j == 0 else 1), d, 0, c1)
                        rows += wide_chunks(1, base_t, d, 0, c2)
                        cols_i += [full[cat1, :, kf, kt].T, full[cat2, :, kf, kt].T]
                        cols_n += [neg[cat1, :, kf, kt].T, neg[cat2, :, kf, kt].T]
                widx, wneg = np.concatenate(cols_i, 1), np.concatenate(cols_n, 1)
                if last:
                    nt = np.zeros((4, 4), dtype=np.int32)
                    nt[0] = (0, 0, 2, 0)
                    dst = [("mask", 0, 2, p)]
                    tt = "T"
                else:
                    nt = None
                    dst = [(f"yd{j}", 0, 2, p)]
                    tt = "T+1"
                bt = 1 if last else 0
                self.specs[f"dec{j}.fwd{p}"] = GemmSpec(f"dec{j}.fwd{p}", rows, widx, wneg, co, eff_bias(pre, co // 2), tt,
                                                        f_in, 1, [(s1, s1_mode), (s2, "all")], dst, ntab=nt,
                                                        conv=(len(ds), ds[0], [[bt + (0 if j == 0 else 1), bt - 1 + (0 if j == 0 else 1)],
                                                                               [bt, bt - 1]]))
            if not last:
                self.bn.append((pre, co // 2))
                self._maybe_fuse_stats(pre, [f"dec{j}.fwd0", f"dec{j}.fwd1"], co, [c1, c2], f_in)
                self._maybe_split_decoder(j, pre, full, neg, cat1, cat2, c1, c2, co, f_in, s1, s1_mode, s2, eff_bias(pre, co // 2))
            gsrc = "dmask" if last else f"dyd{j}"
            if co >= 8:
                rows = []
                for kt in (0, 1):
                    for kf in range(5):
                        rows += wide_chunks(0, kt, kf - 2, 0, co)
                w = full.transpose(0, 3, 2, 1).reshape(c1 + c2, -1)
                wn = neg.transpose(0, 3, 2, 1).reshape(c1 + c2, -1)
            else:
                assert co == 2
                rows, w, wn = [], np.full((c1 + c2, 32), -1, np.int64), np.zeros((c1 + c2, 32), np.int64)
                for kt in (0, 1):
                    rows += [(0, kt - 1, -2, 4), (0, kt - 1, 2, 1)]
                    for kf in range(5):
                        for c in range(2):
                            w[:, kt * 16 + kf * 2 + c] = full[:, c, kf, kt]
                            wn[:, kt * 16 + kf * 2 + c] = neg[:, c, kf, kt]
            order = np.concatenate([cat1, cat2])
            d1 = ("dP", 0, 1, 0) if j == 0 else (f"dzd{j - 1}", 1, 1, 0)
            nt = np.concatenate([dense_ntab(c1, c1, 0, 0), dense_ntab(c2, c2, 1, 0)])
            assert npad_of(c1 + c2) == c1 + c2
            self.specs[f"dec{j}.dg"] = GemmSpec(f"dec{j}.dg", rows, w[order], wn[order], c1 + c2, None, "T", f_in, 2,
                                                [(gsrc, "all")], [d1, (f"dskip{5 - j}", 0, 1, 0)], ntab=nt, kind="dgrad",
                                                conv=(5, -2, [[0, 1], [0, 0]]) if co >= 8 else (5, -2, [[-1, 0], [0, 0]]))

        c5 = kn[6]
        cp = c5 // 2
        h = cfg.hid
        lstm = ("real_lstm", "imag_lstm")

        if not cfg.use_clstm:
            def bias_pairs_real(layer):
                bp = np.empty((4 * h, 2), dtype=np.int32)
                bp[:, 0] = enc_entry(ia(f"enhance.bias_ih_l{layer}"), 0)
                bp[:, 1] = enc_entry(ia(f"enhance.bias_hh_l{layer}"), 0)
                return bp

            zero = lambda a: np.zeros_like(a)
            w1 = ia("enhance.weight_ih_l0").reshape(4 * h, c5, 4).transpose(0, 2, 1).reshape(4 * h, -1)
            rows = []
            for f in range(4):
                rows += wide_chunks(0, 0, f, 0, c5)
            self.specs["ih1"] = GemmSpec("ih1", rows, w1, zero(w1), 4 * h, bias_pairs_real(0), "T", 1, 1, [("z5", "all")],
                                         [("pre1", 0, 1, 0)])
            self.specs["dx1"] = GemmSpec("dx1", wide_chunks(0, 0, 0, 0, 4 * h), w1.T.copy(), zero(w1.T), 4 * c5, None, "T", 1, 1,
                                         [("dpre1", "all")], [("dz5l", 0, 1, 0)], kind="dgrad", res="dskip5" if FUSE_SKIP_GRAD else None)
            w2 = ia("enhance.weight_ih_l1")
            self.specs["ih2"] = GemmSpec("ih2", wide_chunks(0, 0, 0, 0, h), w2, zero(w2), 4 * h, bias_pairs_real(1), "T", 1, 1,
                                         [("h1_0", "all")], [("pre2", 0, 1, 0)])
            self.specs["dx2"] = GemmSpec("dx2", wide_chunks(0, 0, 0, 0, 4 * h), w2.T.copy(), zero(w2.T), h, None, "T", 1, 1,
                                         [("dpre2", "all")], [("dx2", 0, 1, 0)], kind="dgrad")
            tr = ia("tranform.weight")
            wt = tr.reshape(c5, 4, h).transpose(1, 0, 2).reshape(4 * c5, h)
            bp = np.full((4 * c5, 2), -1, dtype=np.int32)
            bp[:, 0] = enc_entry(ia("tranform.bias").reshape(c5, 4).T.reshape(-1), 0)
            self.specs["proj"] = GemmSpec("proj", wide_chunks(0, 0, 0, 0, h), wt, zero(wt), 4 * c5, bp, "T", 1, 1, [("h2_0", "all")],
                                          [("P", 0, 1, 0)])
            rows = []
            for d in range(4):
                rows += wide_chunks(0, 0, d, 0, c5)
            self.specs["dproj"] = GemmSpec("dproj", rows, wt.T.copy(), zero(wt.T), h, None, "T", 1, 1, [("dP", "all")],
                                           [("dxo", 0, 1, 0)], kind="dgrad")
            for layer in (1, 2):
                hh = ia(f"enhance.weight_hh_l{layer - 1}")
                self.specs[f"hh{layer}"] = GemmSpec(f"hh{layer}", wide_chunks(0, -1, 0, 0, h), hh, zero(hh), 4 * h, None, "T", 1, 1,
                                                    [(f"h{layer}_0", "all")], [(f"dpre{layer}", 0, 1, 0)],
                                                    ntab=dense_ntab(4 * h, 4 * h, 0, 0), kind="wgrad_only")
        else:
            def ih(layer, l):
                return ia(f"enhance.{layer}.{lstm[l]}.weight_ih_l0")

            def bias_pairs_lstm(layer):
                bp = np.empty((2 * 4 * h, 2), dtype=np.int32)
                for l in (0, 1):
                    bp[l * 4 * h:(l + 1) * 4 * h, 0] = enc_entry(ia(f"enhance.{layer}.{lstm[l]}.bias_ih_l0"), 0)
                    bp[l * 4 * h:(l + 1) * 4 * h, 1] = enc_entry(ia(f"enhance.{layer}.{lstm[l]}.bias_hh_l0"), 0)
                return bp

            zero = lambda a: np.zeros_like(a)
            w1 = np.concatenate([ih(0, l).reshape(4 * h, cp, 4).transpose(0, 2, 1).reshape(4 * h, -1) for l in (0, 1)])
            for q, tag in enumerate("ri"):
                rows = []
                for f in range(4):
                    rows += wide_chunks(0, 0, f, q * cp, cp)
                self.specs[f"ih1_{tag}"] = GemmSpec(f"ih1_{tag}", rows, w1, zero(w1), 8 * h, bias_pairs_lstm(0), "T", 1, 1,
                                                    [("z5", "all")], [(f"pre1_{tag}", 0, 1, 0)])
                nt = np.zeros((4 * cp // 4, 4), dtype=np.int32)
                for n4 in range(4 * cp // 4):
                    f, c = divmod(4 * n4, cp)
                    nt[n4] = (0, f * c5 + q * cp + c, 4, 0)
                self.specs[f"dx1_{tag}"] = GemmSpec(f"dx1_{tag}", wide_chunks(0, 0, 0, 0, 8 * h), w1.T.copy(), zero(w1.T), 4 * cp,
                                                    None, "T", 1, 1, [(f"dpre1_{tag}", "all")], [("dz5l", 0, 1, 0)], ntab=nt,
                                                    kind="dgrad", res="dskip5" if FUSE_SKIP_GRAD else None)
            combos = {"r": (0, 3, 1), "i": (2, 1, 0)}
            L = cfg.rnn_layers
            for tag, (ca, cb, ng) in combos.items():
                rows = wide_chunks(0, 0, 0, 0, h) + wide_chunks(1, 0, 0, 0, h)
                for layer in range(2, L + 1):
                    w2 = np.concatenate([ih(layer - 1, l) for l in (0, 1)])
                    wi = np.concatenate([w2, w2], 1)
                    wn = np.concatenate([zero(w2), zero(w2) + ng], 1)
                    self.specs[f"ih{layer}_{tag}"] = GemmSpec(f"ih{layer}_{tag}", rows, wi, wn, 8 * h, bias_pairs_lstm(layer - 1), "T", 1, 1,
                                                              [(f"h{layer - 1}_{ca}", "all"), (f"h{layer - 1}_{cb}", "all")],
                                                              [(f"pre{layer}_{tag}", 0, 1, 0)])
                    self.specs[f"dx{layer}_{tag}"] = GemmSpec(f"dx{layer}_{tag}", wide_chunks(0, 0, 0, 0, 8 * h), w2.T.copy(), zero(w2.T), h,
                                                              None, "T", 1, 1, [(f"dpre{layer}_{tag}", "all")],
                                                              [(f"dx{layer}_{tag}", 0, 1, 0)], kind="dgrad")
                q = 0 if tag == "r" else 1
                tr = ia(f"enhance.{L - 1}.{tag}_trans.weight")
                trb = ia(f"enhance.{L - 1}.{tag}_trans.bias")
                wt = tr.reshape(cp, 4, h).transpose(1, 0, 2).reshape(4 * cp, h)
                bt = trb.reshape(cp, 4).T.reshape(-1)
                bp = np.full((4 * cp, 2), -1, dtype=np.int32)
                bp[:, 0] = enc_entry(bt, 0)
                nt = np.zeros((4 * cp // 4, 4), dtype=np.int32)
                for n4 in range(4 * cp // 4):
                    d, c = divmod(4 * n4, cp)
                    nt[n4] = (0, d * c5 + q * cp + c, 4, 0)
                self.specs[f"proj_{tag}"] = GemmSpec(f"proj_{tag}", rows, np.concatenate([wt, wt], 1),
                                                     np.concatenate([zero(wt), zero(wt) + ng], 1), 4 * cp, bp, "T", 1, 1,
                                                     [(f"h{L}_{ca}", "all"), (f"h{L}_{cb}", "all")], [("P", 0, 1, 0)], ntab=nt)
                rows = []
                for d in range(4):
                    rows += wide_chunks(0, 0, d, q * cp, cp)
                self.specs[f"dproj_{tag}"] = GemmSpec(f"dproj_{tag}", rows, wt.T.copy(), zero(wt.T), h, None, "T", 1, 1,
                                                      [("dP", "all")], [(f"dxo_{tag}", 0, 1, 0)], kind="dgrad")
            for layer in range(1, L + 1):
                for combo in range(4):
                    part, l = combo >> 1, combo & 1
                    hh = ia(f"enhance.{layer - 1}.{lstm[l]}.weight_hh_l0")
                    nt = dense_ntab(4 * h, 4 * h, 0, l * 4 * h)
                    self.specs[f"hh{layer}_{combo}"] = GemmSpec(f"hh{layer}_{combo}", wide_chunks(0, -1, 0, 0, h), hh, zero(hh),
                                                                4 * h, None, "T", 1, 1, [(f"h{layer}_{combo}", "all")],
                                                                [(f"dpre{layer}_{'ri'[part]}", 0, 1, 0)], ntab=nt, kind="wgrad_only")

        wa, ba, ga = Arena(64), Arena(16), Arena(16)
        kta, nta = Arena(1), Arena(1)
        self.wgrad_of = {}
        for name, s in self.specs.items():
            s.kt_off = kta.add(s.ktab)
            s.nt_off = nta.add(s.ntab)
            if s.kind != "wgrad_only":
                if TILE_WEIGHTS and s.v3_channels() is not None and not s.stream_takes():
                    s.tile_weights()
                    s.w_off = wa.add(enc_entry(s.widx_packed, s.wneg_packed).reshape(-1))
                else:
                    s.w_off = wa.add(enc_entry(s.widx, s.wneg).reshape(-1))
            if s.bias_pairs is not None:
                s.b_off = ba.add(s.bias_pairs)
            if s.kind in ("fwd", "wgrad_only"):
                s.dw_off = ga.reserve(s.Npad * s.K)
                if s.bias_pairs is not None:
                    s.db_off = ga.reserve(s.Npad)
        self.whh_off, self.whhT_off = {}, {}
        for layer in range(1, cfg.rnn_layers + 1):
            if cfg.use_clstm:
                hh = np.stack([ia(f"enhance.{layer - 1}.{lstm[l]}.weight_hh_l0") for l in (0, 1)])
            else:
                hh = ia(f"enhance.weight_hh_l{layer - 1}")
            self.whh_off[layer] = wa.add(enc_entry(hh, 0).reshape(-1))
            self.whhT_off[layer] = wa.add(enc_entry(np.swapaxes(hh, -1, -2), 0).reshape(-1))
        if cfg.use_clstm and cfg.rnn_layers == 2 and h == 64:
            ih2 = np.stack([ia(f"enhance.1.{lstm[l]}.weight_ih_l0") for l in (0, 1)])
            self.wih2_off = wa.add(enc_entry(ih2, 0).reshape(-1))
            self.wihT2_off = wa.add(enc_entry(ih2.transpose(0, 2, 1), 0).reshape(-1))
        self.bn_g_off = {}
        for pre, cr in self.bn:
            self.bn_g_off[pre] = {k: ga.reserve(cr) for k in ("Wrr", "Wri", "Wii", "Br", "Bi")}
            self.bn_g_off[pre]["slope"] = ga.reserve(1)
        self.n_wpack, self.n_bpack, self.n_gpack = wa.size, ba.size, ga.size
        self.wtab = wa.build(np.int32)
        self.btab = ba.build(np.int32, 2)
        self.ktab = kta.build(np.int32, 4)
        self.ntab = nta.build(np.int32, 4, fill=0)
        self.utab = self._build_unpack_table()

    def _build_unpack_table(self):
        L = self.layout
        ut = UnpackTable(L.n_params)
        for s in self.specs.values():
            if s.dw_off is not None:
                s.put_unpack(ut)
        for pre, cr in self.bn:
            for k in ("Wrr", "Wri", "Wii", "Br", "Bi"):
                f = L.bn_field(pre, "1." + k, cr)
                if f is None:
                    continue
                ut.put(L.index_array(f[0]).reshape(-1)[f[1]:f[1] + cr], self.bn_g_off[pre][k] + np.arange(cr))
            ut.put(L.index_array(pre + "2.weight"), self.bn_g_off[pre]["slope"])
        check_unpack_coverage(L, ut.count, what="DCCRN")
        return ut.tab


class DeviceTables(GemmDeviceTables):
    def __init__(self, st: DCCRNStatic, device):
        super().__init__(st, st.layout, device)
        self.ktab = self.to_device(st.ktab)
        self.window = self.to_device(ops.window_of(st.cfg.win_type, st.cfg.win_len))


class DCCRNWorkspace(GemmWorkspace):
    event_attrs = ("_events", "_fs_events")
    event_pool = 32

    def __init__(self, st: DCCRNStatic, tables: DeviceTables, B, N, device):
        super().__init__()
        cfg = st.cfg
        self.st, self.tb, self.B, self.N, self.device = st, tables, B, N, device
        self.side, self._side_handle = None, None
        self.T = T = ops.stft_frames(N, cfg.win_len, cfg.win_inc)
        if T < 1:
            raise SehipError(f"input of {N} samples is shorter than one frame")
        max_len = (T - 1) * cfg.win_inc + cfg.win_len - (cfg.win_len - cfg.win_inc)
        self.length = min(cfg.length, max_len)
        kn = cfg.kernel_num
        F0 = st.F0
        self.bufs = {}

        Bp = round_up(B, 16)

        def add(name, tst, f, c, t0=0, dtype=BF16, lead=None, batch=None):
            bb = B if batch is None else batch
            shape = (bb, tst, f, c) if lead is None else (lead, bb, tst, f, c)
            t = torch.zeros(shape, dtype=dtype, device=device)
            if lead is None:
                self.bufs[name] = Buf(t, tst, f, c, t0)
            else:
                for q in range(lead):
                    self.bufs[f"{name}_{q}"] = Buf(t[q], tst, f, c, t0)
                self.bufs[name] = Buf(t, tst, f, c, t0)
            return t

        add("enc_in", T, F0, 2)
        for i in range(6):
            f, c = F0 >> (i + 1), kn[i + 1]
            add(f"y{i}", T, f, c); add(f"z{i}", T, f, c)
            add(f"dye{i}", T, f, c); add(f"dskip{i}", T, f, c)
            if i < 5:
                add(f"dz{i}", T, f, c)
        c5, h = kn[6], cfg.hid
        add("dz5l", T, 4, c5); add("P", T, 4, c5); add("dP", T, 4, c5)
        L = cfg.rnn_layers
        if not cfg.use_clstm:
            for layer in (1, 2):
                add(f"pre{layer}", T, 1, 4 * h, dtype=torch.float32)
                add(f"dpre{layer}", T, 1, 4 * h)
                add(f"h{layer}", T, 1, h, lead=1)
                add(f"gates{layer}", T, 1, 4 * h, lead=1, batch=Bp)
                add(f"c{layer}", T, 1, h, dtype=torch.float32, lead=1, batch=Bp)
            add("dxo", T, 1, h); add("dx2", T, 1, h)
        for layer in range(1, L + 1 if cfg.use_clstm else 0):
            for tag in "ri":
                add(f"pre{layer}_{tag}", T, 1, 8 * h, dtype=torch.float32)
                add(f"dpre{layer}_{tag}", T, 1, 8 * h)
            add(f"h{layer}", T, 1, h, lead=4)
            add(f"gates{layer}", T, 1, 4 * h, lead=4, batch=Bp)
            add(f"c{layer}", T, 1, h, dtype=torch.float32, lead=4, batch=Bp)
        for tag in ("ri" if cfg.use_clstm else ""):
            add(f"dxo_{tag}", T, 1, h)
            for layer in range(2, L + 1):
                add(f"dx{layer}_{tag}", T, 1, h)
        for j in range(5):
            idx = 6 - j
            f, c = (F0 >> idx) * 2, kn[idx - 1]
            add(f"yd{j}", T + 1, f, c, 1); add(f"zd{j}", T + 1, f, c, 1)
            add(f"dyd{j}", T + 1, f, c, 1); add(f"dzd{j}", T + 1, f, c, 1)
            if j in st.dec_split:
                add(f"pd{j}", T + 1, f, c, 1)
        add("mask", T, F0, 2, dtype=torch.float32)
        add("dmask", T, F0, 2)
        self.spec = torch.empty(B, T, 257, 2, dtype=torch.float32, device=device)
        self.frames = torch.empty(B, T, cfg.win_len, dtype=torch.float32, device=device)
        self.wav = torch.empty(B, self.length, dtype=torch.float32, device=device)
        self.inv_coff = torch.from_numpy(ops.inv_window_energy(cfg.win_len, cfg.win_inc, T, self.length, cfg.win_type)).to(device)
        self.gpack = torch.zeros(st.n_gpack, dtype=torch.float32, device=device)
        maxcr = max(cr for _, cr in st.bn)
        lib = _lib.lib()
        need = 16
        for pre, cr in st.bn:
            src = self.bufs[("y" if pre.startswith("encoder") else "yd") + pre.split(".")[1]]
            need = max(need, int(lib.sehip_cbn_scratch_floats(src.t.numel() // (2 * cr), cr)))
        self.bn_acc = torch.zeros(need, dtype=torch.float32, device=device)
        self.bn_coef = {pre: torch.zeros(cr, 16, dtype=torch.float32, device=device) for pre, cr in st.bn}
        offs, tot = {}, 0
        for pre, cr in st.bn:
            if pre in st.fused_stats or pre in st.small_stats:
                offs[pre] = tot
                tot += 8 * 5 * cr
        self.bn_stats_all = torch.zeros(max(tot, 1), dtype=torch.float32, device=device)
        self.fuse_finalize = not os.environ.get("SEHIP_NO_FUSE_FINALIZE")
        self.fuse_bwd_finalize = (self.fuse_finalize and not st.deterministic and bool(os.environ.get("SEHIP_FUSE_BWD_FINALIZE")))
        self.bn_reduce_fin = (self.fuse_finalize and not st.deterministic and not self.fuse_bwd_finalize
                              and bool(os.environ.get("SEHIP_BN_REDUCE_FIN")))
        self.bn_ticket = torch.zeros(len(st.bn) + 1, dtype=torch.int32, device=device)
        self._bn_index = {pre: i for i, (pre, _) in enumerate(st.bn)}
        self.fuse_bwd_all = bool(os.environ.get("SEHIP_FUSE_BWD_ALL"))
        self.bn_brep = {pre: torch.zeros(2, BWD_REPLICAS * (6 * cr + 1), dtype=torch.float32, device=device) for pre, cr in st.bn}
        self._brep_turn = {pre: 0 for pre, _ in st.bn}
        self.bn_stats = {pre: self.bn_stats_all[o:o + 8 * 5 * cr] for (pre, cr) in st.bn if pre in offs for o in [offs[pre]]}
        self.bn_bcoef = torch.zeros(maxcr, 16, dtype=torch.float32, device=device)
        self.bn_eps = 1e-5 if cfg.use_cbn else -1e-5
        self.bn_zero = torch.zeros(maxcr, dtype=torch.float32, device=device)
        self.bn_dummy = torch.zeros(maxcr, dtype=torch.float32, device=device)
        self._bn_cr = {pre: cr for pre, cr in st.bn}
        self.mode = {"E": 0, "C": 1, "R": 2}[cfg.masking_mode]
        if not os.environ.get("SEHIP_NO_SIDE_STREAM"):
            if os.environ.get("SEHIP_SIDE_PRIORITY"):
                with torch.cuda.device(device):
                    h = _lib.lib().sehip_stream_create(int(os.environ["SEHIP_SIDE_PRIORITY"]))
                if not h:
                    raise SehipError("sehip_stream_create: " + _lib.lib().sehip_last_error().decode())
                self._side_handle = h
                self.side = torch.cuda.ExternalStream(h, device=device)
            else:
                self.side = torch.cuda.Stream(device=device)
        self.comm = None
        chunk = int(os.environ.get("SEHIP_LSTM_CHUNK", "0"))
        if chunk < 0:
            chunk = (T + 2) // 3 if T >= 96 else 0
        self.lstm_chunks = [(t, min(T, t + chunk)) for t in range(0, T, chunk)] if chunk > 0 else [(0, T)]
        if len(self.lstm_chunks) > 1 and self.lstm_chunks[-1][1] - self.lstm_chunks[-1][0] < chunk // 4:
            last = self.lstm_chunks.pop()
            self.lstm_chunks[-1] = (self.lstm_chunks[-1][0], last[1])
        self.lstm_stream = self.lstm_gemm_stream = None
        if len(self.lstm_chunks) > 1 and not os.environ.get("SEHIP_NO_SIDE_STREAM"):
            hi = torch.cuda.Stream.priority_range()[1]
            self.lstm_stream = torch.cuda.Stream(device=device, priority=hi)
            self.lstm_gemm_stream = torch.cuda.Stream(device=device, priority=hi)
        self.lstm_state = {layer: torch.zeros(4 * ((B + 3) // 4) * 4 * st.cfg.hid * 2, dtype=torch.float32, device=device)
                           for layer in range(1, st.cfg.rnn_layers + 1)}
        self.lstm_fused = (len(self.lstm_chunks) == 1 and not os.environ.get("SEHIP_NO_LSTM_FUSE") and T < 65535
                           and st.cfg.rnn_layers == 2 and st.cfg.hid == 64 and st.cfg.use_clstm)
        self.l2_epoch = 0
        self.graph_epoch = 0
        if self.lstm_fused:
            lib_ = _lib.lib()
            self.l2_gran_f = torch.zeros(int(lib_.sehip_lstm2_gran_bytes(B, T, 0)) // 8, dtype=torch.int64, device=device)
            self.l2_gran_b = torch.zeros(int(lib_.sehip_lstm2_gran_bytes(B, T, 1)) // 8, dtype=torch.int64, device=device)
            self.l2_sync = torch.zeros(int(lib_.sehip_lstm2_sync_bytes()) // 4, dtype=torch.int32, device=device)
        self.enc0_bn_in_wgrad = (FUSE_ENC0_BN_WGRAD and not self.fuse_bwd_finalize and int(st.cfg.kernel_num[1]) == 16
                                 and (st.F0 >> 1) % 32 == 0 and (st.F0 >> 1) <= 128)
        self._bind()

    def close(self):
        super().close()
        if self._side_handle:
            _lib.lib().sehip_stream_destroy(self._side_handle)
            self._side_handle = None

    def _side_in_use(self):
        return self.side is not None

    def _bind(self):
        st, tb, B, T = self.st, self.tb, self.B, self.T
        self.desc = {}
        self._wgrad_on_chain = set((os.environ.get("SEHIP_WGRAD_ON_CHAIN", "enc0.fwd") or "").split(",")) - {"", "none"}
        self._chunk_cache = {}
        self._wg_groups = {}
        self.ktab_dev = upload_chunk_table(st.ktab, st.specs.values(), lambda s: [(self.bufs[b].F, self.bufs[b].C) for b, _ in s.srcs],
                                           self.device)
        for name, s in st.specs.items():
            tt = T if s.tt == "T" else T + 1
            srcs, dsts = [], []
            for bname, mode in s.srcs:
                b = self.bufs[bname]
                srcs.append((b.ptr, b.Tst, b.F, b.C) + ((1, T + 1) if mode == "drop1" else (0, b.Tst)))
            for bname, toff, fmul, fadd in s.dsts:
                b = self.bufs[bname]
                fc = (1, b.F * b.C) if s.J == 1 else (b.F, b.C)
                dsts.append((b.ptr, b.Tst) + fc + (toff, fmul, fadd, 0, 1 if b.t.dtype == torch.float32 else 0))
            res = None
            if s.res is not None:
                rb, db_ = self.bufs[s.res], self.bufs[s.dsts[0][0]]
                assert (rb.Tst, rb.F, rb.C) == (db_.Tst, db_.F, db_.C) and rb.t.dtype == torch.bfloat16
                res = rb.ptr
            d = fill_desc(srcs, dsts, row_ptr(self.ktab_dev, s.kt_off), row_ptr(tb.ntab, s.nt_off), row_ptr(tb.wpack, s.w_off),
                          row_ptr(tb.bpack, s.b_off), B * tt * s.J, s.N, s.Npad, s.K, tt, s.J, s.fmul, 0, res)
            d.w_tiled = 1 if s.w_tiled else 0
            if s.stats_of is not None:
                d.stats = self.bn_stats[s.stats_of].data_ptr()
                d.stats_cr = s.N // 2
            if s.conv is not None:
                d.cv_nf, d.cv_fadd = s.conv[0], s.conv[1]
                for q in range(2):
                    for kt in range(2):
                        d.cv_toff[q][kt] = s.conv[2][q][kt]
            self.desc[name] = d
            if s.dw_off is not None:
                w = wgrad_twin(d, row_ptr(self.gpack, s.dw_off), row_ptr(self.gpack, s.db_off),
                               self.bufs[self._grad_buffer_of(s.dsts[0][0])].ptr if s.kind == "fwd" else None)
                if name == "enc0.fwd" and self.enc0_bn_in_wgrad:
                    zb, yb, gb = self.bufs["dz0"], self.bufs["y0"], self.bufs["dye0"]
                    assert (zb.Tst, zb.F, zb.C) == (gb.Tst, gb.F, gb.C) == (yb.Tst, yb.F, yb.C) and zb.t.dtype == yb.t.dtype == BF16
                    w.bn_dz, w.bn_y = zb.ptr, yb.ptr
                    w.bn_coef, w.bn_bcoef = ptr(self.bn_coef["encoder.0."]), ptr(self.bn_bcoef)
                self.desc[name + ".wg"] = w
        self.fused_small = set()
        lib = _lib.lib()
        for pre, names in st.small_stats.items():
            ds = [self.desc[nm] for nm in names]
            for d in ds:
                d.stats = self.bn_stats[pre].data_ptr()
                d.stats_cr = d.Npad // 2
            if lib.sehip_conv_small_takes(C.byref(ds[0]), C.byref(ds[1]) if len(ds) == 2 else None):
                self.fused_small.add(pre)
            else:
                for d in ds:
                    d.stats = None
                    d.stats_cr = 0
        self.bnr_rows = {}
        if not os.environ.get("SEHIP_NO_BNR"):
            for j in range(1, 6):
                pre, cr = f"decoder.{j - 1}.", int(st.cfg.kernel_num[6 - j]) // 2
                d = self.desc[f"dec{j}.dg"]
                rows = int(lib.sehip_bnr_rows(C.byref(d), None))
                yb, zb = self.bufs[f"yd{j - 1}"], self.bufs[f"dzd{j - 1}"]
                if rows <= 0 or d.dst[0].ptr != zb.ptr or (yb.Tst, yb.F, yb.C) != (zb.Tst, zb.F, zb.C) or yb.C != 2 * cr:
                    continue
                if rows * (6 * cr + 1) > self.bn_acc.numel():
                    self.bn_acc = torch.zeros(rows * (6 * cr + 1), dtype=torch.float32, device=self.device)
                self.bnr_rows[pre] = (rows, f"dec{j}.dg")
            for pre, (rows, name) in self.bnr_rows.items():
                d = self.desc[name]
                d.bnr_y, d.bnr_coef, d.bnr_part = self.bufs["yd" + pre.split(".")[1]].ptr, ptr(self.bn_coef[pre]), ptr(self.bn_acc)
        if not os.environ.get("SEHIP_NO_WGRAD_GROUP"):
            nl = self.st.cfg.rnn_layers
            for layers in [(layer,) for layer in range(1, nl + 1)] + ([(2, 1)] if nl == 2 else []):
                self._wgrad_group_handle(self._lstm_wgrad_names(layers))

    def _chunk_desc(self, name, t0, t1):
        key = (name, t0, t1)
        if key in self._chunk_cache:
            return self._chunk_cache[key]
        d = CGemmDesc.from_buffer_copy(self.desc[name])
        s = self.st.specs[name]
        assert s.J == 1 and s.tt == "T"
        for q, (bname, mode) in enumerate(s.srcs):
            b = self.bufs[bname]
            d.src[q].ptr = b.ptr + t0 * b.F * b.C * b.t.element_size()
            d.src[q].thi = b.Tst - t0
        for q, (bname, toff, fmul, fadd) in enumerate(s.dsts):
            b = self.bufs[bname]
            d.dst[q].ptr = b.ptr + t0 * b.F * b.C * b.t.element_size()
        if s.res is not None:
            rb = self.bufs[s.res]
            d.res = rb.ptr + t0 * rb.F * rb.C * rb.t.element_size()
        d.TT = t1 - t0
        d.M = self.B * (t1 - t0)
        self._chunk_cache[key] = d
        return d

    @staticmethod
    def _grad_buffer_of(out_name):
        if out_name.startswith("yd"):
            return "dyd" + out_name[2:]
        if out_name.startswith("y"):
            return "dye" + out_name[1:]
        if out_name == "mask":
            return "dmask"
        if out_name.startswith("pre"):
            return "d" + out_name
        if out_name == "P":
            return "dP"
        raise KeyError(out_name)

    def gemm_pair(self, a, b):
        self._chain_dirty = True
        call("sehip_gemm_pair", C.byref(self.desc[a]), C.byref(self.desc[b]), stream())

    def wgrad(self, name):
        main = torch.cuda.current_stream()
        if self.side is None or name in self._wgrad_on_chain:
            call("sehip_wgrad", C.byref(self.desc[name + ".wg"]), main.cuda_stream)
            return
        if self._chain_dirty:
            call("sehip_stream_depend", self.side.cuda_stream, main.cuda_stream, self._event())
            self._chain_dirty = False
        call("sehip_wgrad", C.byref(self.desc[name + ".wg"]), self.side.cuda_stream)

    def wgrad_pair(self, a, b):
        main = torch.cuda.current_stream()
        if self.side is None or a in self._wgrad_on_chain:
            call("sehip_wgrad_pair", C.byref(self.desc[a + ".wg"]), C.byref(self.desc[b + ".wg"]), main.cuda_stream)
            return
        if self._chain_dirty:
            call("sehip_stream_depend", self.side.cuda_stream, main.cuda_stream, self._event())
            self._chain_dirty = False
        call("sehip_wgrad_pair", C.byref(self.desc[a + ".wg"]), C.byref(self.desc[b + ".wg"]), self.side.cuda_stream)

    def _lstm_wgrad_names(self, layers):
        if not self.st.cfg.use_clstm:
            return [nm for layer in layers for nm in (f"ih{layer}", f"hh{layer}")]
        return [nm for layer in layers for nm in [f"ih{layer}_{tag}" for tag in "ri"] + [f"hh{layer}_{combo}" for combo in range(4)]]

    def _wgrad_group_handle(self, names):
        key = tuple(names)
        g = self._wg_groups.get(key)
        if g is None:
            n = len(names)
            arr = (CGemmDesc * n)(*[CGemmDesc.from_buffer_copy(self.desc[nm + ".wg"]) for nm in names])
            buf = torch.empty(int(_lib.lib().sehip_wgrad_group_bytes(n)), dtype=torch.uint8, device=self.bufs["enc_in"].t.device)
            total = C.c_int(0)
            call("sehip_wgrad_group_prepare", C.cast(arr, C.c_void_p), n, ptr(buf), C.cast(C.pointer(total), C.c_void_p))
            dense = None
            if not os.environ.get("SEHIP_NO_DENSE_GROUP"):
                lib_ = _lib.lib()
                dbuf = torch.empty(int(lib_.sehip_wgrad_dense_group_bytes(n)), dtype=torch.uint8, device=buf.device)
                info = (C.c_int * 8)()
                call("sehip_wgrad_dense_group_prepare", C.cast(arr, C.c_void_p), n, ptr(dbuf), dbuf.numel(), C.cast(info, C.c_void_p))
                if info[0] == 1:
                    need = info[4] + (info[5] << 31)
                    if getattr(self, "_dtw_scratch", None) is None or self._dtw_scratch.numel() < need:
                        self._dtw_scratch = torch.empty(need, dtype=torch.float32, device=buf.device)
                    dense = (dbuf, info)
            g = self._wg_groups[key] = (buf, n, total.value, dense)
        return g

    def wgrad_group(self, names):
        if os.environ.get("SEHIP_NO_WGRAD_GROUP"):
            for nm in names:
                self.wgrad(nm)
            return
        buf, n, total, dense = self._wgrad_group_handle(names)
        if self.st.deterministic and dense is None:
            for nm in names:
                self.wgrad(nm)
            return
        main = torch.cuda.current_stream()

        def launch(st):
            if dense is not None:
                call("sehip_wgrad_dense_group", ptr(dense[0]), n, C.cast(dense[1], C.c_void_p), ptr(self._dtw_scratch), st)
            else:
                call("sehip_wgrad_group", ptr(buf), n, total, st)
        if self.side is None:
            launch(main.cuda_stream)
            return
        if self._chain_dirty:
            call("sehip_stream_depend", self.side.cuda_stream, main.cuda_stream, self._event())
            self._chain_dirty = False
        launch(self.side.cuda_stream)

    def launch_units(self):
        d, units = self.desc, []

        def one(fn, name):
            return (name, [name], lambda st, fn=fn, name=name: call(fn, C.byref(d[name]), st))

        def pair(fn, a, b):
            return (a + "+" + b, [a, b], lambda st, fn=fn, a=a, b=b: call(fn, C.byref(d[a]), C.byref(d[b]), st))
        for i in range(6):
            units.append(one("sehip_gemm", f"enc{i}.fwd"))
            units.append(one("sehip_wgrad", f"enc{i}.fwd.wg"))
            units.append(one("sehip_gemm", f"dec{i}.dg"))
            if i in self.st.dec_split and self.side is not None:
                units.append(pair("sehip_gemm_pair", f"dec{i}.fs0", f"dec{i}.fs1"))
                units.append(pair("sehip_gemm_pair", f"dec{i}.fm0", f"dec{i}.fm1"))
            else:
                units.append(pair("sehip_gemm_pair", f"dec{i}.fwd0", f"dec{i}.fwd1"))
            units.append(pair("sehip_wgrad_pair", f"dec{i}.fwd0.wg", f"dec{i}.fwd1.wg"))
            if i > 0:
                units.append(pair("sehip_gemm_pair", f"enc{i}.dg0", f"enc{i}.dg1"))
        if not self.st.cfg.use_clstm:
            for nm in ("ih1", "ih2", "proj", "dproj", "dx2", "dx1"):
                units.append(one("sehip_gemm", nm))
            units += [one("sehip_wgrad", nm + ".wg") for nm in ["proj"] + self._lstm_wgrad_names((2, 1))]
            return units
        for a, b in (("ih1_r", "ih1_i"), ("proj_r", "proj_i"), ("dproj_r", "dproj_i"), ("dx1_r", "dx1_i")):
            units.append(pair("sehip_gemm_pair", a, b))
        nl = self.st.cfg.rnn_layers
        if not self.lstm_fused:
            for layer in range(2, nl + 1):
                for a, b in ((f"ih{layer}_r", f"ih{layer}_i"), (f"dx{layer}_r", f"dx{layer}_i")):
                    units.append(pair("sehip_gemm_pair", a, b))
        for tag in "ri":
            units.append(one("sehip_wgrad", f"proj_{tag}.wg"))
        names = self._lstm_wgrad_names(tuple(range(nl, 0, -1)))
        if not os.environ.get("SEHIP_NO_WGRAD_GROUP") and nl <= 2:
            buf, n, total, dense = self._wgrad_group_handle(names)
            if dense is not None:
                units.append(("lstm.wg (dense group)", [nm + ".wg" for nm in names],
                              lambda st: call("sehip_wgrad_dense_group", ptr(dense[0]), n, C.cast(dense[1], C.c_void_p), ptr(self._dtw_scratch), st)))
            elif not self.st.deterministic:
                units.append(("lstm.wg (group)", [nm + ".wg" for nm in names], lambda st: call("sehip_wgrad_group", ptr(buf), n, total, st)))
            else:
                units += [one("sehip_wgrad", nm + ".wg") for nm in names]
        else:
            units += [one("sehip_wgrad", nm + ".wg") for nm in names]
        return units

    def _bn_ptrs(self, pre, params, buffers, nbt):
        L = self.st.layout
        cr = self._bn_cr[pre]

        def pp(k):
            f = L.bn_field(pre, k, cr)
            return ptr(self.bn_zero) if f is None else params.data_ptr() + 4 * (L.param_off[f[0]][0] + f[1])

        def bp(k):
            f = L.bn_field(pre, k, cr)
            return ptr(self.bn_dummy) if f is None else buffers.data_ptr() + 4 * (L.buffer_off[f[0]][0] + f[1])
        return pp, bp, nbt.data_ptr() + 8 * L.nbt_idx[pre + "1.num_batches_tracked"]

    def bn_forward(self, pre, cr, y, z, params, buffers, nbt, training):
        rows = y.t.numel() // (2 * cr)
        pp, bp, nb = self._bn_ptrs(pre, params, buffers, nbt)
        coef = self.bn_coef[pre]
        if pre in self.st.fused_stats or pre in self.fused_small:
            if self.fuse_finalize:
                call("sehip_cbn_finalize_apply_n", y.ptr, ptr(self.bn_stats[pre]), 8, pp("1.Wrr"), pp("1.Wri"), pp("1.Wii"), pp("1.Br"),
                     pp("1.Bi"), bp("1.RMr"), bp("1.RMi"), bp("1.RVrr"), bp("1.RVri"), bp("1.RVii"), nb, rows, cr, self.bn_eps, 0.1,
                     1 if training else 0, ptr(coef), pp("2.weight"), z.ptr, stream())
                return
            call("sehip_cbn_finalize_n", ptr(self.bn_stats[pre]), 8, pp("1.Wrr"), pp("1.Wri"), pp("1.Wii"), pp("1.Br"), pp("1.Bi"),
                 bp("1.RMr"), bp("1.RMi"), bp("1.RVrr"), bp("1.RVri"), bp("1.RVii"), nb, rows, cr, self.bn_eps, 0.1,
                 1 if training else 0, ptr(coef), stream())
            call("sehip_cbn_apply", y.ptr, ptr(coef), pp("2.weight"), rows, cr, z.ptr, stream())
            return
        if training:
            call("sehip_cbn_stats", y.ptr, rows, cr, ptr(self.bn_acc), stream())
        call("sehip_cbn_finalize", ptr(self.bn_acc), pp("1.Wrr"), pp("1.Wri"), pp("1.Wii"), pp("1.Br"), pp("1.Bi"),
             bp("1.RMr"), bp("1.RMi"), bp("1.RVrr"), bp("1.RVri"), bp("1.RVii"), nb, rows, cr, self.bn_eps, 0.1,
             1 if training else 0, ptr(coef), stream())
        call("sehip_cbn_apply", y.ptr, ptr(coef), pp("2.weight"), rows, cr, z.ptr, stream())

    def bn_backward(self, pre, cr, dz, dz2, y, dy, params, tfirst, apply=True):
        rows = y.t.numel() // (2 * cr)
        L, st = self.st.layout, self.st

        def pp(k):
            f = L.bn_field(pre, k, cr)
            return ptr(self.bn_zero) if f is None else params.data_ptr() + 4 * (L.param_off[f[0]][0] + f[1])
        g = lambda k: self.gpack.data_ptr() + 4 * st.bn_g_off[pre][k]
        coef = self.bn_coef[pre]
        dz2p = dz2.ptr if dz2 is not None else None
        self._chain_dirty = True
        if pre in self.bnr_rows and dz2 is None and not (self.fuse_bwd_finalize and self.fuse_bwd_all):
            call("sehip_cbn_bwd_finalize_n", ptr(self.bn_acc), self.bnr_rows[pre][0], ptr(coef), pp("1.Wrr"), pp("1.Wri"), pp("1.Wii"), rows, cr,
                 g("Wrr"), g("Wri"), g("Wii"), g("Br"), g("Bi"), g("slope"), ptr(self.bn_bcoef), stream())
            if apply:
                call("sehip_cbn_bwd_apply", dz.ptr, dz2p, y.ptr, ptr(coef), ptr(self.bn_bcoef), pp("2.weight"), rows, cr, y.F,
                     y.Tst, tfirst, dy.ptr, stream())
            return
        if self.fuse_bwd_finalize:
            rep = self.bn_brep[pre]
            if torch.cuda.is_current_stream_capturing():
                turn = 0
                rep[0].zero_()
            else:
                turn = self._brep_turn[pre]
                self._brep_turn[pre] = turn ^ 1
            call("sehip_cbn_bwd_fused", dz.ptr, dz2p, y.ptr, ptr(coef), pp("1.Wrr"), pp("1.Wri"), pp("1.Wii"), pp("2.weight"), rows, cr,
                 y.F, y.Tst, tfirst, ptr(rep[turn]), ptr(rep[turn ^ 1]), BWD_REPLICAS, g("Wrr"), g("Wri"), g("Wii"), g("Br"), g("Bi"),
                 g("slope"), dy.ptr, stream())
            return
        if self.bn_reduce_fin:
            rep = self.bn_brep[pre]
            call("sehip_cbn_bwd_reduce_fin", dz.ptr, dz2p, y.ptr, ptr(coef), pp("1.Wrr"), pp("1.Wri"), pp("1.Wii"), pp("2.weight"), rows, cr,
                 y.F, y.Tst, tfirst, ptr(rep[0]), BWD_REPLICAS, self.bn_ticket.data_ptr() + 4 * self._bn_index[pre], g("Wrr"), g("Wri"),
                 g("Wii"), g("Br"), g("Bi"), g("slope"), ptr(self.bn_bcoef), stream())
        else:
            call("sehip_cbn_bwd_reduce", dz.ptr, dz2p, y.ptr, ptr(coef), pp("2.weight"), rows, cr, y.F, y.Tst, tfirst,
                 ptr(self.bn_acc), stream())
            call("sehip_cbn_bwd_finalize", ptr(self.bn_acc), ptr(coef), pp("1.Wrr"), pp("1.Wri"), pp("1.Wii"), rows, cr,
                 g("Wrr"), g("Wri"), g("Wii"), g("Br"), g("Bi"), g("slope"), ptr(self.bn_bcoef), stream())
        if not apply:
            return
        call("sehip_cbn_bwd_apply", dz.ptr, dz2p, y.ptr, ptr(coef), ptr(self.bn_bcoef), pp("2.weight"), rows, cr, y.F,
             y.Tst, tfirst, dy.ptr, stream())

    def _lstm_fwd_call(self, layer, t0, t1, st_):
        b, cfg = self.bufs, self.st.cfg
        whh = self.tb.wpack.data_ptr() + 2 * self.st.whh_off[layer]
        call("sehip_lstm_fwd_chunk", b[f"pre{layer}_r"].ptr, b[f"pre{layer}_i"].ptr, whh, self.B, self.T, cfg.hid, t0, t1,
             b[f"h{layer}"].ptr, b[f"gates{layer}"].ptr, b[f"c{layer}"].ptr, st_)

    def _l2_next_epoch(self):
        if torch.cuda.is_current_stream_capturing():
            self.l2_gran_f.zero_(); self.l2_gran_b.zero_()
            return L2_GRAPH_EPOCH
        self.l2_epoch = self.l2_epoch % (L2_GRAPH_EPOCH - 1) + 1
        return self.l2_epoch

    def check_lstm_handoffs(self, recover=True, global_flag=None):
        has_word = hasattr(self, "l2_sync")
        tripped = has_word and int(self.l2_sync[0]) != 0
        if global_flag is not None:
            tripped = global_flag(tripped, self.device)
        if not tripped:
            return False
        if not has_word:
            return True
        if not recover:
            raise SehipError("DCCRN: a hand-off wait of the fused two-layer LSTM kernels timed out (results since then are invalid and "
                             "no optimizer step was applied); set SEHIP_NO_LSTM_FUSE=1 to use one launch per layer")
        import warnings
        warnings.warn("sehip DCCRN: a hand-off wait of the fused two-layer LSTM kernels timed out; the optimizer steps since then were "
                      "skipped on the device; falling back to one launch per LSTM layer for this workspace")
        self.lstm_fused = False
        self.l2_sync.zero_()
        self.graph_epoch += 1
        return True

    def _lstm_forward(self, B, T, h):
        self._chain_dirty = True
        main = stream()
        if not self.st.cfg.use_clstm:
            b, wp = self.bufs, self.tb.wpack.data_ptr()
            for layer in (1, 2):
                self.gemm(f"ih{layer}")
                call("sehip_rlstm_fwd", b[f"pre{layer}"].ptr, wp + 2 * self.st.whh_off[layer], B, T, h, b[f"h{layer}"].ptr,
                     b[f"gates{layer}"].ptr, b[f"c{layer}"].ptr, main)
            return
        self.gemm_pair("ih1_r", "ih1_i")
        if self.lstm_fused:
            b, st, tb = self.bufs, self.st, self.tb
            wp = tb.wpack.data_ptr()
            self._l2_cur_epoch = self._l2_next_epoch()
            call("sehip_lstm2_fwd", b["pre1_r"].ptr, b["pre1_i"].ptr, wp + 2 * st.whh_off[1], wp + 2 * st.whh_off[2],
                 wp + 2 * st.wih2_off, self.desc["ih2_r"].bias, B, T, h, b["h1"].ptr, b["gates1"].ptr, b["c1"].ptr, b["h2"].ptr,
                 b["gates2"].ptr, b["c2"].ptr, ptr(self.l2_gran_f), ptr(self.l2_sync), self._l2_cur_epoch, main)
            return
        nl = self.st.cfg.rnn_layers
        if self.lstm_stream is None or nl != 2 or torch.cuda.is_current_stream_capturing():
            self._lstm_fwd_call(1, 0, T, main)
            for layer in range(2, nl + 1):
                self.gemm_pair(f"ih{layer}_r", f"ih{layer}_i")
                self._lstm_fwd_call(layer, 0, T, main)
            return
        s2, s3 = self.lstm_stream.cuda_stream, self.lstm_gemm_stream.cuda_stream
        for (t0, t1) in self.lstm_chunks:
            self._lstm_fwd_call(1, t0, t1, main)
            call("sehip_stream_depend", s3, main, self._event())
            call("sehip_gemm_pair", C.byref(self._chunk_desc("ih2_r", t0, t1)), C.byref(self._chunk_desc("ih2_i", t0, t1)), s3)
            call("sehip_stream_depend", s2, s3, self._event())
            self._lstm_fwd_call(2, t0, t1, s2)
        call("sehip_stream_depend", main, s2, self._event())

    def _lstm_bwd_call(self, layer, t0, t1, st_):
        b, cfg = self.bufs, self.st.cfg
        dha, dhb = (b["dxo_r"], b["dxo_i"]) if layer == cfg.rnn_layers else (b[f"dx{layer + 1}_r"], b[f"dx{layer + 1}_i"])
        whhT = self.tb.wpack.data_ptr() + 2 * self.st.whhT_off[layer]
        call("sehip_lstm_bwd_chunk", dha.ptr, dhb.ptr, whhT, b[f"gates{layer}"].ptr, b[f"c{layer}"].ptr, self.B, self.T, cfg.hid,
             t0, t1, ptr(self.lstm_state[layer]), b[f"dpre{layer}_r"].ptr, b[f"dpre{layer}_i"].ptr, st_)

    def _lstm_backward(self, B, T, h):
        self._chain_dirty = True
        main = stream()
        if not self.st.cfg.use_clstm:
            b, wp = self.bufs, self.tb.wpack.data_ptr()
            for layer in (2, 1):
                dh = b["dxo"] if layer == 2 else b["dx2"]
                call("sehip_rlstm_bwd", dh.ptr, wp + 2 * self.st.whhT_off[layer], b[f"gates{layer}"].ptr, b[f"c{layer}"].ptr, B, T, h,
                     b[f"dpre{layer}"].ptr, main)
                self._chain_dirty = True
                self.wgrad_group(self._lstm_wgrad_names((layer,)))
                self.gemm(f"dx{layer}")
            return
        if self.lstm_fused:
            b, st, tb = self.bufs, self.st, self.tb
            wp = tb.wpack.data_ptr()
            call("sehip_lstm2_bwd", b["dxo_r"].ptr, b["dxo_i"].ptr, wp + 2 * st.whhT_off[1], wp + 2 * st.whhT_off[2],
                 wp + 2 * st.wihT2_off, b["gates1"].ptr, b["c1"].ptr, b["gates2"].ptr, b["c2"].ptr, B, T, h, b["dpre1_r"].ptr,
                 b["dpre1_i"].ptr, b["dpre2_r"].ptr, b["dpre2_i"].ptr, ptr(self.l2_gran_b), ptr(self.l2_sync),
                 getattr(self, "_l2_cur_epoch", 1), main)
            self._chain_dirty = True
            self.wgrad_group(self._lstm_wgrad_names((2, 1)))
            self.gemm_pair("dx1_r", "dx1_i")
            return
        nl = self.st.cfg.rnn_layers
        if self.lstm_stream is None or nl != 2 or torch.cuda.is_current_stream_capturing():
            for layer in range(nl, 0, -1):
                self._lstm_bwd_call(layer, 0, T, main)
                self.wgrad_group(self._lstm_wgrad_names((layer,)))
                self.gemm_pair(f"dx{layer}_r", f"dx{layer}_i")
            return
        s2, s3 = self.lstm_stream.cuda_stream, self.lstm_gemm_stream.cuda_stream
        for (t0, t1) in reversed(self.lstm_chunks):
            self._lstm_bwd_call(2, t0, t1, main)
            call("sehip_stream_depend", s3, main, self._event())
            call("sehip_gemm_pair", C.byref(self._chunk_desc("dx2_r", t0, t1)), C.byref(self._chunk_desc("dx2_i", t0, t1)), s3)
            call("sehip_stream_depend", s2, s3, self._event())
            self._lstm_bwd_call(1, t0, t1, s2)
        call("sehip_stream_depend", main, s2, self._event())
        self._chain_dirty = True
        self.wgrad_group(self._lstm_wgrad_names((2, 1)))
        self.gemm_pair("dx1_r", "dx1_i")

    def pack_weights(self, params):
        st, tb = self.st, self.tb
        call("sehip_pack_bf16", ptr(params), ptr(tb.wtab), st.n_wpack, ptr(tb.wpack), stream())
        call("sehip_pack_f32", ptr(params), ptr(tb.btab), st.n_bpack, ptr(tb.bpack), stream())

    def forward(self, wav_in, params, buffers, nbt, training=True):
        st, cfg, b, tb = self.st, self.st.cfg, self.bufs, self.tb
        B, T, h = self.B, self.T, cfg.hid
        zero = self.bn_stats_all if (self.st.fused_stats or self.fused_small) else None
        head = self.side.cuda_stream if (self.side is not None and PARALLEL_HEAD) else stream()
        if head != stream():
            call("sehip_stream_depend", head, stream(), self._event())
        call("sehip_pack_head", ptr(params), ptr(tb.wtab), st.n_wpack, ptr(tb.wpack), ptr(tb.btab), st.n_bpack, ptr(tb.bpack),
             ptr(zero) if zero is not None else None, zero.numel() if zero is not None else 0, head)
        if head != stream() and training:
            with torch.cuda.stream(self.side):
                self.gpack.zero_()
            self._gpack_clean = True
        call("sehip_stft_fwd", ptr(wav_in), ptr(tb.window), B, self.N, cfg.win_len, cfg.win_inc, cfg.fft_len,
             ptr(self.spec), b["enc_in"].ptr, stream())
        if head != stream():
            call("sehip_stream_depend", stream(), head, self._event())
        for i in range(6):
            self.gemm(f"enc{i}.fwd")
            self.bn_forward(f"encoder.{i}.", cfg.kernel_num[i + 1] // 2, b[f"y{i}"], b[f"z{i}"], params, buffers, nbt, training)
        split = st.dec_split if self.side is not None else []
        if split:
            sd = self.side.cuda_stream
            call("sehip_stream_depend", sd, stream(), self._event())
            if not self._fs_events:
                self._fs_events = [self._new_event() for _ in range(6)]
            for j in split:
                call("sehip_gemm_pair", C.byref(self.desc[f"dec{j}.fs0"]), C.byref(self.desc[f"dec{j}.fs1"]), sd)
                call("sehip_event_record", self._fs_events[j], sd)
        self._lstm_forward(B, T, h)
        if cfg.use_clstm:
            self.gemm_pair("proj_r", "proj_i")
        else:
            self.gemm("proj")
        for j in range(6):
            if j in split:
                call("sehip_stream_wait_event", stream(), self._fs_events[j])
                self.gemm_pair(f"dec{j}.fm0", f"dec{j}.fm1")
            else:
                self.gemm_pair(f"dec{j}.fwd0", f"dec{j}.fwd1")
            if j < 5:
                self.bn_forward(f"decoder.{j}.", cfg.kernel_num[5 - j] // 2, b[f"yd{j}"], b[f"zd{j}"], params, buffers, nbt,
                                training)
        call("sehip_istft_fwd", ptr(self.spec), b["mask"].ptr, ptr(tb.window), ptr(self.inv_coff), B, T, cfg.win_len,
             cfg.win_inc, cfg.fft_len, self.length, self.mode, ptr(self.frames), ptr(self.wav), stream())
        return self.wav

    def backward(self, dwav, params, grads, range_ready=None, tail=None):
        st, cfg, b, tb = self.st, self.st.cfg, self.bufs, self.tb
        B, T, h = self.B, self.T, cfg.hid
        if not getattr(self, "_gpack_clean", False):
            self.gpack.zero_()
        self._gpack_clean = False
        self._chain_dirty = True
        call("sehip_istft_bwd", ptr(dwav), ptr(self.wav), ptr(self.spec), b["mask"].ptr, ptr(tb.window), ptr(self.inv_coff),
             B, T, cfg.win_len, cfg.win_inc, cfg.fft_len, self.length, self.mode, b["dmask"].ptr, stream())
        for j in range(5, -1, -1):
            if j < 5:
                self.bn_backward(f"decoder.{j}.", cfg.kernel_num[5 - j] // 2, b[f"dzd{j}"], None, b[f"yd{j}"], b[f"dyd{j}"],
                                 params, 1)
            self.wgrad_pair(f"dec{j}.fwd0", f"dec{j}.fwd1")
            if j >= 1 and f"decoder.{j - 1}." in self.bnr_rows:
                self.desc[f"dec{j}.dg"].bnr_slope = params.data_ptr() + 4 * st.layout.param_off[f"decoder.{j - 1}.2.weight"][0]
            self.gemm(f"dec{j}.dg")
        if cfg.use_clstm:
            for tag in "ri":
                self.wgrad(f"proj_{tag}")
            self.gemm_pair("dproj_r", "dproj_i")
        else:
            self.wgrad("proj")
            self.gemm("dproj")
        self._lstm_backward(B, T, h)
        n_params = st.layout.n_params
        lo = st.layout.param_off["decoder.0.0.real_conv.weight"][0] if range_ready is not None else 0
        if range_ready is not None:
            L = st.layout
            if not getattr(st, "_dp_layout_checked", False):
                for nm in L.param_names:
                    early = L.param_off[nm][0] >= lo
                    if early != (not nm.startswith("encoder.")):
                        raise SehipError(f"DCCRN data-parallel hand-over: parameter {nm} at offset {L.param_off[nm][0]} is on the wrong "
                                         f"side of the decoder/LSTM split {lo}")
                st._dp_layout_checked = True
            if self.comm is None:
                self.comm = torch.cuda.Stream(device=self.device)
            cs = self.comm.cuda_stream
            call("sehip_stream_depend", cs, stream(), self._event())
            if self.side is not None:
                call("sehip_stream_depend", cs, self.side.cuda_stream, self._event())
            call("sehip_unpack_grad", ptr(self.gpack), tb.utab.data_ptr() + 16 * lo, n_params - lo, grads.data_ptr() + 4 * lo, cs)
            range_ready(lo, n_params, self.comm)
        for i in range(5, -1, -1):
            dz = b["dz5l"] if i == 5 else b[f"dz{i}"]
            dz2 = b[f"dskip{i}"] if not FUSE_SKIP_GRAD else None
            in_wgrad = i == 0 and self.enc0_bn_in_wgrad and dz2 is None
            self.bn_backward(f"encoder.{i}.", cfg.kernel_num[i + 1] // 2, dz, dz2, b[f"y{i}"], b[f"dye{i}"], params, 0, apply=not in_wgrad)
            if i == 0:
                wd = self.desc["enc0.fwd.wg"]
                wd.bn_dz = dz.ptr if in_wgrad else None
                wd.bn_slope = params.data_ptr() + 4 * self.st.layout.param_off["encoder.0.2.weight"][0] if in_wgrad else None
            self.wgrad(f"enc{i}.fwd")
            if i > 0:
                self.gemm_pair(f"enc{i}.dg0", f"enc{i}.dg1")
        self.join_side()
        if range_ready is None:
            self.unpack(grads, tail, guard=ptr(self.l2_sync) if hasattr(self, "l2_sync") else None)
        else:
            call("sehip_unpack_grad", ptr(self.gpack), ptr(tb.utab), lo, ptr(grads), stream())
            range_ready(0, lo, torch.cuda.current_stream())
            call("sehip_stream_depend", stream(), self.comm.cuda_stream, self._event())
        return grads
```

### speech-enhancement-pytorch_amd/sehip/solver.py

```python
import datetime
import json
import os
import time
from pathlib import Path
from shutil import copyfile

import numpy as np
import torch
import torch.distributed as dist

from . import distrib, plumbing
from ._lib import SehipError
from .model.types import MONARCH_SPEECH_SEPARTAION_MODELS, MULTI_SPEECH_SEPERATION_MODELS, STFT_MODELS
from .evaluate import stft_custom
from .optim import FlatOptimizer
from .utils import obj2dict

try:
    from torch.utils.tensorboard import SummaryWriter as _TBWriter
except Exception:
    _TBWriter = None


class ScalarLog:

    def __init__(self, *a, **k):
        self.scalars = []

    def add_text(self, *a, **k):
        pass

    def add_scalar(self, tag, value, step=None, *a, **k):
        self.scalars.append((tag, float(value), -1 if step is None else int(step)))

    def add_scalars(self, *a, **k):
        pass

    def add_figure(self, *a, **k):
        pass


def _cfg(obj, name, default):
    return getattr(obj, name, default)


class DevicePrefetcher:

    def __init__(self, loader, device, limit=None):
        self.it = iter(loader)
        self.device = device
        self.limit = limit
        self.taken = 0
        self.stream = torch.cuda.Stream(device=device)
        self.ready = None
        self._preload()

    def _preload(self):
        self.ready = None
        if self.limit is not None and self.taken >= self.limit:
            return
        try:
            batch = next(self.it)
        except StopIteration:
            return
        self.taken += 1
        with torch.cuda.stream(self.stream):
            self.ready = tuple(t.to(self.device, non_blocking=True) if torch.is_tensor(t) else t for t in batch)

    def __iter__(self):
        return self

    def __next__(self):
        if self.ready is None:
            raise StopIteration
        cur = torch.cuda.current_stream(self.device)
        cur.wait_stream(self.stream)
        batch = self.ready
        for t in batch:
            if torch.is_tensor(t) and t.is_cuda:
                t.record_stream(cur)
        self._preload()
        return batch


class Solver(object):
    def __init__(self, config, model, optimizer=None, loss_function=None, train_dataloader=None,
                 validation_dataloader=None, test_dataloader=None, device="gpu", writer=None):
        self.train_dataloader = train_dataloader
        self.validation_dataloader = validation_dataloader
        self.test_dataloader = test_dataloader
        self.audiogram_dataloader = None

        self.rank, self.world_size, self.local_rank = distrib.init_distributed() if device == "gpu" else (0, 1, 0)
        self.n_gpu = torch.cuda.device_count()
        if device == "gpu":
            if self.n_gpu == 0:
                raise SehipError("Solver(device='gpu'): no GPU visible and the HIP path has no CPU fallback")
            self.device = torch.device(f"cuda:{self.local_rank}")
            torch.cuda.set_device(self.device)
        else:
            self.device = torch.device(device) if not isinstance(device, torch.device) else device
            if self.device.type == "cpu" and config.model.name not in plumbing.TORCH_MODELS:
                raise SehipError(f"Solver(device='cpu'): model '{config.model.name}' runs on the HIP path only; the CPU "
                                 f"plumbing configuration exists for {plumbing.TORCH_MODELS} (BASELINE config C0)")
        self.is_main = self.rank == 0
        self.deterministic = bool(_cfg(config.solver, "cudnn_deterministic", False)) and device == "gpu"
        if self.deterministic and _cfg(config.solver, "use_graph", False):
            raise SehipError("solver.cudnn_deterministic and solver.use_graph cannot be combined: the deterministic schedule allocates its "
                             "partial-sum arrays on demand (not capturable); switch one of them off")
        if device == "gpu":
            from .utils import set_deterministic
            set_deterministic(self.deterministic)
            if hasattr(model, "set_deterministic"):
                model.set_deterministic(self.deterministic)
        if self.deterministic and not hasattr(model, "set_deterministic"):
            import warnings
            warnings.warn(f"solver.cudnn_deterministic: model '{config.model.name}' has no deterministic plan yet (its normalisation "
                          f"sums use fp32 atomics); the library-level reductions are deterministic, run-to-run bit equality is not guaranteed")

        self.optimizer = optimizer
        self.loss_function = loss_function
        self.model = model.to(self.device)
        self.flat_model = hasattr(self.model, "flat_params")
        if self.world_size > 1:
            if self.flat_model:
                distrib.broadcast_parameters(self.model.flat_params, self.model._bflat)
            else:
                for t in list(self.model.parameters()) + list(self.model.buffers()):
                    dist.broadcast(t.data, 0)

        self.epochs = config.solver.epochs
        self.save_checkpoint_interval = config.solver.save_checkpoint_interval
        self.validation_interval = config.solver.validation.interval
        self.test_interval = config.solver.test.interval
        self.log_interval = int(_cfg(config.solver, "log_interval", 1))

        self.find_max = config.solver.validation.metric in ("stoi", "pesq", "sisdr", "haspi", "hasqi")
        self.score = {"best_score": -np.inf if self.find_max else np.inf, "loss": 0, "loss_valid": 0, "grad_norm": 0,
                      "stoi": [], "pesq": [], "sisdr": [], "haspi": [], "hasqi": []}

        self.root_dir = Path(config.solver.root) / "result" / config.model.name / datetime.datetime.now().strftime("%Y%m%d-%H%M%S")
        self.checkpoints_dir = self.root_dir / "checkpoints"
        self.logs_dir = self.root_dir / "logs"
        if self.is_main:
            for d in (self.checkpoints_dir, self.logs_dir):
                d.mkdir(parents=True, exist_ok=True)
        if writer is not None:
            self.writer = writer
        elif _TBWriter is not None and self.is_main:
            self.writer = _TBWriter(log_dir=self.logs_dir.as_posix(), max_queue=5, flush_secs=30)
        else:
            self.writer = ScalarLog()
        self.writer.add_text(tag="Configuration",
                             text_string=f"<pre>  \n{json.dumps(obj2dict(config), indent=4, sort_keys=False)}  \n</pre>",
                             global_step=1)
        self.config = config
        if config.solver.preloaded_model:
            self._preload_model()
        elif config.solver.resume:
            self._resume_checkpoint()
        if self.is_main and getattr(config, "root", None) and os.path.exists(config.root):
            copyfile(config.root, (self.root_dir / "config.yaml").as_posix())
        self._print_networks([self.model])

    def _resume_checkpoint(self):
        latest = Path(self.config.solver.resume) / "checkpoints/latest_model.tar"
        assert latest.exists(), f"{latest} does not exist, can not load latest checkpoint."
        checkpoint = torch.load(latest.as_posix(), map_location=self.device, weights_only=False)
        self.best_score = checkpoint["best_score"]
        if self.config.optim.load:
            self.optimizer.load_state_dict(checkpoint["optimizer"])
        self.model.load_state_dict(checkpoint["model"])
        print(f"\tModel checkpoint loaded, {latest.as_posix()}")

    def _preload_model(self):
        path = Path(self.config.solver.preloaded_model)
        assert path.exists(), f"Preloaded *.pth file is not exist. Please check the file path: {path.as_posix()}"
        self.model.load_state_dict(torch.load(path, map_location=self.device, weights_only=False), strict=False)
        print(f"\tModel preloaded successfully from {path.as_posix()}.")

    @staticmethod
    def _print_networks(nets):
        total = 0
        for i, net in enumerate(nets, start=1):
            n = sum(p.numel() for p in net.parameters())
            print(f"\tNetwork {i}: {n / 1e6} million.")
            total += n
        print(f"The amount of parameters in the project is {total / 1e6} million.")

    def _model_health(self):
        fn = getattr(self.model, "check_health", None)
        if fn is not None and fn():
            self.lost_steps = getattr(self, "lost_steps", 0) + 1
            self.writer.add_scalar("Train/lost_steps", self.lost_steps, -1)

    def _save_checkpoint(self, epoch, is_best=False):
        self._model_health()
        if not self.is_main:
            return
        state_dict = {"epoch": epoch, "best_score": self.score["best_score"], "optimizer": self.optimizer.state_dict()}
        state_dict["model"] = {k: v.cpu() for k, v in self.model.state_dict().items()}
        torch.save(state_dict, (self.checkpoints_dir / "latest_model.tar").as_posix())
        torch.save(state_dict["model"], (self.checkpoints_dir /
                   f"model_{str(epoch).zfill(4)}_{self.config.solver.validation.metric}_{self.score['best_score']:2.8f}.pth").as_posix())
        with open(self.checkpoints_dir / "state.json", "w") as tmp:
            json.dump(self.score, tmp, indent=4)
        if is_best:
            torch.save(state_dict, (self.checkpoints_dir / "best_model.tar").as_posix())

    def _is_best(self, score, find_max=True):
        if find_max and score >= self.score["best_score"]:
            self.score["best_score"] = score
            return True
        if not find_max and score <= self.score["best_score"]:
            self.score["best_score"] = score
            return True
        return False

    def train(self):
        patience = self.config.solver.patience
        early_stopping = 0
        for epoch in range(self.epochs):
            start_time = time.time()
            score = self._run_one_epoch(epoch, self.epochs, train=True)
            if epoch % self.save_checkpoint_interval == 0:
                self._save_checkpoint(epoch)
            if epoch % self.validation_interval == 0:
                score = self._run_one_epoch(epoch, self.epochs, train=False)
                score = distrib.allreduce_mean_scalar(score)
                if self._is_best(score, find_max=self.find_max):
                    self._save_checkpoint(epoch, is_best=True)
                    early_stopping = 0
                else:
                    early_stopping += 1
            if early_stopping > patience:
                break
            print(f"[{int(time.time() - start_time)} seconds] End this epoch.")

    def _prepare_batch(self, mixture, sources, wave=False):
        cfg = self.config
        mixture = mixture.to(self.device, non_blocking=True)
        sources = sources.to(self.device, non_blocking=True)
        batch, nchannel, nsample = mixture.shape
        num_spk = sources.shape[1]
        assert cfg.model.audio_channels == nchannel, f"Channel between {cfg.dset.name} and {cfg.model.name} did not match..."
        assert cfg.model.num_spk == num_spk, f"number of speakers between {cfg.dset.name} and {cfg.model.name} did not match..."
        if cfg.model.name in MULTI_SPEECH_SEPERATION_MODELS:
            assert num_spk == len(cfg.model.sources)
        if cfg.model.name in MONARCH_SPEECH_SEPARTAION_MODELS:
            sources = torch.squeeze(sources, dim=1)
            mixture = torch.reshape(mixture, shape=(batch * nchannel, 1, nsample))
            sources = torch.reshape(sources, shape=(batch * num_spk * nchannel, 1, nsample))
        if wave:
            return mixture, sources
        if cfg.model.name in STFT_MODELS:
            stft = plumbing.stft_custom if mixture.device.type == "cpu" else stft_custom
            mixture = stft(tensor=mixture, config=cfg.model)
            sources = stft(tensor=sources, config=cfg.model)
        return mixture, sources

    def _metric_functions(self):
        from . import metric
        return {"sisdr": metric.SI_SDR, "stoi": metric.STOI}

    def _sample_rate(self):
        return int(_cfg(getattr(self.config, "dset", None), "sample_rate", 16000))

    def compute_metric(self, mixture, enhanced, clean):
        sr = self._sample_rate()
        score, score_reference = {}, {}
        with torch.no_grad():
            for name, fn in self._metric_functions().items():
                score_reference[name] = [fn(reference=clean, estimation=mixture, sr=sr)]
                score[name] = [fn(reference=clean, estimation=enhanced, sr=sr)]
        return score, score_reference

    def _validation_metric(self, name, enhanced, wave_sources):
        if self.config.model.name in STFT_MODELS:
            from .evaluate import istft_custom
            enhanced = istft_custom(enhanced.contiguous(), wave_sources.shape[-1], self.config.model)
        if enhanced.shape != wave_sources.shape:
            if enhanced.numel() != wave_sources.numel():
                raise SehipError(f"validation metric '{name}': output {tuple(enhanced.shape)} and sources {tuple(wave_sources.shape)} "
                                 "do not pair up")
            enhanced = enhanced.reshape(wave_sources.shape)
        return self._metric_functions()[name](reference=wave_sources, estimation=enhanced, sr=self._sample_rate())

    def train_step(self, mixture, sources):
        if mixture.is_cuda:
            from ._lib import stream_scope
            with stream_scope():
                return self._train_step(mixture, sources)
        return self._train_step(mixture, sources)

    def _unit_grad(self, loss):
        if os.environ.get("SEHIP_NO_UNIT_GRAD"):
            return None
        g = getattr(self, "_unit", None)
        if g is None or g.device != loss.device or g.dtype != loss.dtype or g.shape != loss.shape:
            g = self._unit = torch.ones_like(loss)
        return g

    def _loss(self, enhanced, sources, mixture):
        if _cfg(self.config.optim, "loss", None) != "psa":
            return self.loss_function(enhanced, sources)
        if sources.dim() == mixture.dim() + 1:
            mixture = mixture.unsqueeze(1).expand_as(sources)
        return self.loss_function(enhanced, sources, mixture)

    def _pit_applies(self, sources):
        return bool(_cfg(self.config.optim, "pit_apply", False)) and sources.dim() >= 3 and sources.shape[1] >= 2 and \
            self.config.model.name in MULTI_SPEECH_SEPERATION_MODELS

    def _step_loss(self, enhanced, sources, mixture):
        if self._pit_applies(sources):
            from .loss import pit_loss
            return pit_loss(enhanced, sources, self.loss_function)
        return self._loss(enhanced, sources, mixture)

    def _train_step(self, mixture, sources):
        if not self.model.training:
            self.model.train()
        enhanced = self.model(mixture)
        loss = self._step_loss(enhanced, sources, mixture)
        self.optimizer.zero_grad()
        fused = isinstance(self.optimizer, FlatOptimizer)
        works, early_guard = [], False
        if self.world_size > 1 and self.flat_model and fused:
            self.optimizer.grad_scale = 1.0 / self.world_size
            if hasattr(self.model, "_tail_sink"):
                self.model._tail_sink = None
            works = []
            early_guard = bool(getattr(self.model, "step_guard_early", False)) and hasattr(self.model, "step_guard")
            if hasattr(self.model, "grad_range_hook"):
                def hook(lo, hi, st):
                    if early_guard and not works:
                        works.append(distrib.allreduce_step_guard_async(self.model.step_guard(), st))
                    works.append(distrib.allreduce_range_async(self.model.flat_grads, lo, hi, st))
                self.model.grad_range_hook = hook
            loss.backward(self._unit_grad(loss))
            if hasattr(self.model, "grad_range_hook"):
                self.model.grad_range_hook = None
            if works:
                for w in works:
                    w.wait()
            else:
                distrib.allreduce_gradients(self.model.flat_grads, scale=False)
        else:
            loss.backward(self._unit_grad(loss))
            if self.world_size > 1:
                if self.flat_model:
                    distrib.allreduce_gradients(self.model.flat_grads)
                else:
                    distrib.allreduce_module_gradients(self.model)
        if self.world_size > 1 and hasattr(self.model, "step_guard") and not (fused and self.flat_model and works and early_guard):
            distrib.allreduce_step_guard(self.model.step_guard())
        if self.config.optim.clip_grad:
            if fused:
                self.optimizer.clip_grad_norm_(self.config.optim.clip_grad)
            else:
                torch.nn.utils.clip_grad_norm_(self.model.parameters(), self.config.optim.clip_grad)
        self.optimizer.step()
        if fused:
            metric = self.optimizer.grad_metric()
        else:
            sums = torch.stack([p.grad.sum() for p in self.model.parameters() if p.grad is not None])
            metric = torch.stack([sums.square().sum().sqrt(), sums.new_zeros(())])
        return loss.detach(), metric

    def train_step_graphed(self, mixture, sources):
        key = (tuple(mixture.shape), tuple(sources.shape))
        if not hasattr(self, "_graphs"):
            self._graphs = {}
        g = self._graphs.get(key)
        if g is not None and g["epoch"] != self.model.storage_epoch:
            g = None
        if g is None:
            g = self._graphs[key] = self._capture_step(mixture, sources)
        g["mix"].copy_(mixture)
        g["src"].copy_(sources)
        g["fb"].replay()
        if self.world_size > 1:
            distrib.allreduce_gradients(self.model.flat_grads, scale=False)
            if hasattr(self.model, "step_guard"):
                distrib.allreduce_step_guard(self.model.step_guard())
        g["upd"].replay()
        return g["loss"], g["metric"]

    def _capture_step(self, mixture, sources):
        from ._lib import call
        if not isinstance(self.optimizer, FlatOptimizer):
            raise SehipError("train_step_graphed needs the fused FlatOptimizer")
        call("sehip_init")
        self.model.train()
        self.optimizer.grad_scale = 1.0 / self.world_size
        self.model.workspace(mixture.shape[0], mixture.shape[-1]).pinned = True
        self.optimizer._ensure_state()
        self.model.flat_grads
        self.model._grad_anchor(mixture.device)
        mix, src = mixture.clone(), sources.clone()
        if self._pit_applies(src):
            from . import loss as loss_module
            if self.loss_function in (loss_module.l1_loss, loss_module.mse_loss) and src.shape[1] <= loss_module.PIT_MAX_SPEAKERS:
                loss_module.pit_pointwise_workspace(src.shape, src.device)
            elif self.loss_function is not loss_module.loss_sisdr:
                raise SehipError("solver.use_graph with optim.pit_apply needs optim.loss si-sdr, l1 or mse and at most "
                                 f"{loss_module.PIT_MAX_SPEAKERS} speakers: the permutation of any other loss is picked on the host")
        torch.cuda.synchronize()
        fb, upd = torch.cuda.CUDAGraph(), torch.cuda.CUDAGraph()
        with torch.cuda.graph(fb):
            enhanced = self.model(mix)
            loss = self._step_loss(enhanced, src, mix)
            self.optimizer.zero_grad()
            loss.backward()
            loss_out = loss.detach().clone()
        with torch.cuda.graph(upd, pool=fb.pool()):
            if self.config.optim.clip_grad:
                self.optimizer.clip_grad_norm_(self.config.optim.clip_grad)
            self.optimizer.step()
            metric_out = self.optimizer.grad_metric().clone()
        self.optimizer._step -= 1
        return dict(fb=fb, upd=upd, mix=mix, src=src, loss=loss_out, metric=metric_out, epoch=self.model.storage_epoch)

    def _run_one_epoch(self, epoch, total_epoch, train=False):
        cfg = self.config
        loss_total = 0.0
        grad_norm_total = 0.0
        dataloader = self.train_dataloader if train else self.validation_dataloader
        total_step = len(dataloader)
        if not cfg.solver.all_steps:
            if train and total_step > cfg.solver.total_steps:
                total_step = cfg.solver.total_steps
            elif not train and total_step > cfg.solver.validation.total_steps:
                total_step = cfg.solver.validation.total_steps
        pending = []
        valid_metric = cfg.solver.validation.metric if not train and cfg.solver.validation.metric in ("stoi", "sisdr") else None
        score_total, score_steps = 0.0, 0

        def flush():
            nonlocal loss_total, grad_norm_total, score_total, score_steps
            for step_, loss_t, metric_t in pending:
                loss = float(loss_t)
                loss_total += loss
                if valid_metric is not None:
                    score_total += float(metric_t)
                    score_steps += 1
                    self.score[valid_metric] = score_total / score_steps
                if train:
                    grad_norm = float(metric_t[0]) if metric_t is not None else 0.0
                    grad_norm_total += grad_norm
                    self.writer.add_scalar("Train/Loss_step", loss, epoch * total_step + step_)
                    self.writer.add_scalar("Train/grad_norm_step", grad_norm, epoch * total_step + step_)
                else:
                    self.writer.add_scalar("Validation/Loss_step", loss, epoch * total_step + step_)
            pending.clear()
            self._model_health()

        batches = dataloader
        if self.device.type == "cuda" and _cfg(cfg.solver, "prefetch", True) and not os.environ.get("SEHIP_NO_PREFETCH"):
            batches = DevicePrefetcher(dataloader, self.device, limit=total_step)
        for step, batch in enumerate(batches):
            if step >= total_step:
                break
            mixture, sources = batch[0], batch[1]
            if valid_metric is not None and cfg.model.name in STFT_MODELS:
                wave_sources = self._prepare_batch(mixture, sources, wave=True)[1]
            mixture, sources = self._prepare_batch(mixture, sources)
            if train:
                step_fn = self.train_step_graphed if _cfg(cfg.solver, "use_graph", False) else self.train_step
                loss_t, metric_t = step_fn(mixture, sources)
                pending.append((step, loss_t.clone(), metric_t.clone() if metric_t is not None else None))
            else:
                self.model.eval()
                with torch.no_grad():
                    enhanced = self.model(mixture)
                    loss_t = self._loss(enhanced, sources, mixture)
                    score_t = None
                    if valid_metric is not None:
                        score_t = self._validation_metric(valid_metric, enhanced,
                                                          wave_sources if cfg.model.name in STFT_MODELS else sources)
                pending.append((step, loss_t.detach().clone(), score_t))
            if (step + 1) % self.log_interval == 0:
                flush()
        flush()
        if train:
            self.score["loss"] = loss_total / total_step
            self.score["grad_norm"] = grad_norm_total / total_step
            self.writer.add_scalar("Train/Loss", self.score["loss"], epoch)
            self.writer.add_scalar("Train/Grad_norm", self.score["grad_norm"], epoch)
        else:
            self.score["loss_valid"] = loss_total / total_step
            self.writer.add_scalar("Validation/Loss", self.score["loss_valid"], epoch)
        return self.score["loss"] if train else self.score[cfg.solver.validation.metric]
```

Measured before the change: 20180 audio-s/s.

## Fuse SI-SNR loss with iSTFT forward/backward and add a last-block finalize

When the training loss is SI-SDR and no PIT is involved, the model now computes the loss directly inside its own plan. The forward loss kernel finalizes the mean in its last block using an atomic ticket. The SI-SNR gradient is computed inside the iSTFT backward kernel, so the dwav tensor and the separate sisnr_bwd launch are no longer needed. The iSTFT forward also fuses frame synthesis with overlap-add through shared memory and skips the frames buffer when overlap is small. This removes several launches and a full-waveform round trip through memory, at the cost of more complex kernels and a cross-block atomic that must be reset correctly.

```diff
diff --git a/include/sehip.h b/include/sehip.h
--- a/include/sehip.h
+++ b/include/sehip.h
@@ -29,6 +29,9 @@
 int sehip_istft_bwd(const float* dwav, const float* wav, const float* spec, const float* mask, const float* window,
                     const float* inv_coff, int B, int T, int win_len, int hop, int fft_len, int length,
                     int masking_mode, void* dmask_bf16 , void* stream);
+int sehip_sisnr_istft_bwd(const float* wav, const float* ref, const float* rowstat, const float* upstream ,
+                          const float* spec, const float* mask, const float* window, const float* inv_coff, int B, int T,
+                          int win_len, int hop, int fft_len, int length, int masking_mode, void* dmask_bf16, void* stream);
 
 int sehip_stft_custom_frames(int n_samples, int n_fft, int hop, int center);
 int sehip_stft_custom_fwd(const float* wav, int rows, int n_samples, int n_fft, int hop, int win_length, int center,
@@ -45,6 +48,8 @@
                         float* out, const long* out_off, void* stream);
 
 int sehip_sisnr_fwd(const float* est, const float* ref, int rows, int n, float* rowstat, float* loss, void* stream);
+int sehip_sisnr_fwd_fin(const float* est, const float* ref, int rows, int n, float* rowstat, unsigned* ticket, float* loss,
+                        void* stream);
 int sehip_sisdr_metric(const float* reference, const float* estimation, int rows, int n, float* ratios, float* out, void* stream);
 int sehip_sisnr_bwd(const float* est, const float* ref, const float* rowstat, const float* upstream ,
                     int rows, int n, float* dest, void* stream);
diff --git a/speech-enhancement-pytorch_amd/sehip/_lib.py b/speech-enhancement-pytorch_amd/sehip/_lib.py
--- a/speech-enhancement-pytorch_amd/sehip/_lib.py
+++ b/speech-enhancement-pytorch_amd/sehip/_lib.py
@@ -47,6 +47,8 @@
     "sehip_resample_out_len": [L, I, I],
     "sehip_resample_frac": [P, P, I, P, I, I, I, P, P, P],
     "sehip_sisnr_fwd": [P, P, I, I, P, P, P],
+    "sehip_sisnr_fwd_fin": [P, P, I, I, P, P, P, P],
+    "sehip_sisnr_istft_bwd": [P, P, P, P, P, P, P, P, I, I, I, I, I, I, I, P, P],
     "sehip_sisdr_metric": [P, P, I, I, P, P, P],
     "sehip_stoi_out_len": [L, I],
     "sehip_stoi_frames": [L],
diff --git a/speech-enhancement-pytorch_amd/sehip/csrc/loss.hip b/speech-enhancement-pytorch_amd/sehip/csrc/loss.hip
--- a/speech-enhancement-pytorch_amd/sehip/csrc/loss.hip
+++ b/speech-enhancement-pytorch_amd/sehip/csrc/loss.hip
@@ -1,15 +1,23 @@
 #include "common.h"
 
+#include "sisnr.h"
+
 #define EPS 1e-8f
 
-__device__ __forceinline__ float sisnr_residual(float x, float alpha, float s) {
-    float t = alpha * s;
-    asm volatile("" : "+v"(t));
-    return x - t;
-}
-
+template <bool COHERENT>
+__device__ __forceinline__ void sisnr_mean_of_rows(const float4* rowstat, int rows, float* __restrict__ loss) {
+    float acc = 0.f;
+    for (int i = threadIdx.x; i < rows; i += 64)
+        acc += COHERENT ? __hip_atomic_load(reinterpret_cast<const float*>(rowstat + i) + 2, __ATOMIC_RELAXED, __HIP_MEMORY_SCOPE_AGENT)
+                        : rowstat[i].z;
+    acc = wave_sum(acc);
+    if (threadIdx.x == 0) loss[0] = -acc / rows;
+}
+
+template <bool FIN>
 __global__ __launch_bounds__(1024) void sisnr_fwd_kernel(const float* __restrict__ est, const float* __restrict__ ref,
-                                                        int n, int rows, float4* __restrict__ rowstat) {
+                                                        int n, int rows, float4* rowstat, unsigned* __restrict__ ticket,
+                                                        float* __restrict__ loss) {
     __shared__ float red[16];
     const int r = blockIdx.x;
     const float* x = est + (size_t)r * n;
@@ -60,13 +68,23 @@
         const float b = c * (2.f * alpha * ss / ((ss + EPS) * (en + EPS)) + 2.f * q * es / (ss + EPS));
         rowstat[r] = make_float4(a, b, l, alpha);
     }
+    if (!FIN) return;
+    __shared__ unsigned is_last;
+    if (threadIdx.x == 0) {
+        __builtin_amdgcn_fence(__ATOMIC_RELEASE, "agent");
+        asm volatile("s_waitcnt vmcnt(0)" ::: "memory");
+        is_last = __hip_atomic_fetch_add(ticket, 1u, __ATOMIC_RELAXED, __HIP_MEMORY_SCOPE_AGENT) == gridDim.x - 1 ? 1u : 0u;
+    }
+    __syncthreads();
+    if (!is_last || threadIdx.x >= 64) return;
+    __builtin_amdgcn_fence(__ATOMIC_ACQUIRE, "agent");
+    asm volatile("s_waitcnt vmcnt(0)" ::: "memory");
+    if (threadIdx.x == 0) __hip_atomic_store(ticket, 0u, __ATOMIC_RELAXED, __HIP_MEMORY_SCOPE_AGENT);
+    sisnr_mean_of_rows<true>(rowstat, rows, loss);
 }
 
 __global__ void sisnr_finalize_kernel(const float4* __restrict__ rowstat, int rows, float* __restrict__ loss) {
-    float acc = 0.f;
-    for (int i = threadIdx.x; i < rows; i += 64) acc += rowstat[i].z;
-    acc = wave_sum(acc);
-    if (threadIdx.x == 0) loss[0] = -acc / rows;
+    sisnr_mean_of_rows<false>(rowstat, rows, loss);
 }
 
 __global__ __launch_bounds__(256) void sisnr_bwd_kernel(const float* __restrict__ est, const float* __restrict__ ref,
@@ -79,7 +97,7 @@
     const size_t base = (size_t)r * n;
     for (int i = blockIdx.x * 256 + threadIdx.x; i < n; i += gridDim.x * 256) {
         const float s = ref[base + i];
-        dest[base + i] = a * sisnr_residual(est[base + i], alpha, s) + b * s;
+        dest[base + i] = sisnr_grad(est[base + i], s, a, b, alpha);
     }
 }
 
@@ -126,9 +144,18 @@
                                void* stream) {
     SEHIP_REQUIRE(rows > 0 && n > 0, "sisnr_fwd: empty input (rows=%d n=%d)", rows, n);
     hipStream_t st = (hipStream_t)stream;
-    sisnr_fwd_kernel<<<rows, 1024, 0, st>>>(est, ref, n, rows, (float4*)rowstat);
+    sisnr_fwd_kernel<false><<<rows, 1024, 0, st>>>(est, ref, n, rows, (float4*)rowstat, nullptr, nullptr);
     sisnr_finalize_kernel<<<1, 64, 0, st>>>((const float4*)rowstat, rows, loss);
     SEHIP_CHECK_LAUNCH("sisnr_fwd");
+    return 0;
+}
+
+extern "C" int sehip_sisnr_fwd_fin(const float* est, const float* ref, int rows, int n, float* rowstat, unsigned* ticket, float* loss,
+                                   void* stream) {
+    SEHIP_REQUIRE(rows > 0 && n > 0, "sisnr_fwd_fin: empty input (rows=%d n=%d)", rows, n);
+    SEHIP_REQUIRE(est && ref && rowstat && ticket && loss, "sisnr_fwd_fin: null pointer");
+    sisnr_fwd_kernel<true><<<rows, 1024, 0, (hipStream_t)stream>>>(est, ref, n, rows, (float4*)rowstat, ticket, loss);
+    SEHIP_CHECK_LAUNCH("sisnr_fwd_fin");
     return 0;
 }
 
diff --git a/speech-enhancement-pytorch_amd/sehip/csrc/sisnr.h b/speech-enhancement-pytorch_amd/sehip/csrc/sisnr.h
--- /dev/null
+++ b/speech-enhancement-pytorch_amd/sehip/csrc/sisnr.h
@@ -0,0 +1,12 @@
+#pragma once
+#include "common.h"
+
+__device__ __forceinline__ float sisnr_residual(float x, float alpha, float s) {
+    float t = alpha * s;
+    asm volatile("" : "+v"(t));
+    return x - t;
+}
+
+__device__ __forceinline__ float sisnr_grad(float x, float s, float a, float b, float alpha) {
+    return a * sisnr_residual(x, alpha, s) + b * s;
+}
diff --git a/speech-enhancement-pytorch_amd/sehip/csrc/stft.hip b/speech-enhancement-pytorch_amd/sehip/csrc/stft.hip
--- a/speech-enhancement-pytorch_amd/sehip/csrc/stft.hip
+++ b/speech-enhancement-pytorch_amd/sehip/csrc/stft.hip
@@ -2,6 +2,7 @@
 
 #include "fft512.h"
 #include "mask.h"
+#include "sisnr.h"
 
 __global__ __launch_bounds__(256) void stft_fwd_kernel(const float* __restrict__ wav, const float* __restrict__ window,
                                                        int B, int N, int T, int win, int hop,
@@ -53,6 +54,54 @@
     *reinterpret_cast<uint4*>(eo + 4 * lane) = *reinterpret_cast<const uint4*>(&senc[w][4 * lane]);
 }
 
+__device__ __forceinline__ void istft_frame(const float2* __restrict__ sp, const float2* __restrict__ mk, const float* __restrict__ window,
+                                            int win, int mode, int lane, const FftTw& tw, float (&o)[8]) {
+    float re[8], im[8];
+#pragma unroll
+    for (int r = 0; r < 8; ++r) {
+        const int k = lane + 64 * r;
+        float er = 0.f, ei = 0.f;
+        if (k >= 1 && k <= 256) {
+            const float2 z = sp[k];
+            const float2 m = mk[k - 1];
+            apply_mask(mode, z.x, z.y, m.x, m.y, er, ei);
+        }
+        re[r] = er; im[r] = ei;
+    }
+    fft512_wave<1>(re, im, tw, lane);
+    const int n0 = 8 * brev6(lane);
+    constexpr int brev3[8] = {0, 4, 2, 6, 1, 5, 3, 7};
+    float u[8];
+    float s1 = 0.f, s2 = 0.f;
+#pragma unroll
+    for (int j = 0; j < 8; ++j) {
+        const int n = n0 + brev3[j];
+        u[brev3[j]] = re[j];
+        if (n < win) { s1 += re[j]; s2 += (n & 1) ? -re[j] : re[j]; }
+    }
+    s1 = wave_sum(s1);
+    s2 = wave_sum(s2);
+    const float c = 1.0f / (float)(FFT_N + win);
+#pragma unroll
+    for (int q = 0; q < 8; ++q) {
+        const int n = n0 + q;
+        const float corr = c * (s1 + ((n & 1) ? -s2 : s2));
+        o[q] = n < win ? window[n] * (1.0f / 256.0f) * (u[q] - corr) : 0.f;
+    }
+}
+
+__device__ __forceinline__ void istft_store_frame(float* __restrict__ fo, const float (&o)[8], int lane, int win) {
+    const int n0 = 8 * brev6(lane);
+    if (n0 + 8 <= win && (win & 3) == 0) {
+        *reinterpret_cast<float4*>(fo + n0) = make_float4(o[0], o[1], o[2], o[3]);
+        *reinterpret_cast<float4*>(fo + n0 + 4) = make_float4(o[4], o[5], o[6], o[7]);
+        return;
+    }
+#pragma unroll
+    for (int q = 0; q < 8; ++q)
+        if (n0 + q < win) fo[n0 + q] = o[q];
+}
+
 __global__ __launch_bounds__(256) void istft_frames_kernel(const float2* __restrict__ spec, const float2* __restrict__ mask,
                                                            const float* __restrict__ window, int nframes, int win, int mode,
                                                            float* __restrict__ frames) {
@@ -61,55 +110,9 @@
     if (frame >= nframes) return;
     FftTw tw;
     fft_twiddles<1>(tw, lane);
-    float re[8], im[8];
-    const float2* sp = spec + (size_t)frame * NBIN;
-    const float2* mk = mask + (size_t)frame * 256;
-#pragma unroll
-    for (int r = 0; r < 8; ++r) {
-        const int k = lane + 64 * r;
-        float er = 0.f, ei = 0.f;
-        if (k >= 1 && k <= 256) {
-            const float2 z = sp[k];
-            const float2 m = mk[k - 1];
-            apply_mask(mode, z.x, z.y, m.x, m.y, er, ei);
-        }
-        re[r] = er; im[r] = ei;
-    }
-    fft512_wave<1>(re, im, tw, lane);
-    const int n0 = 8 * brev6(lane);
-    constexpr int brev3[8] = {0, 4, 2, 6, 1, 5, 3, 7};
-    float u[8];
-    float s1 = 0.f, s2 = 0.f;
-#pragma unroll
-    for (int j = 0; j < 8; ++j) {
-        const int n = n0 + brev3[j];
-        u[brev3[j]] = re[j];
-        if (n < win) { s1 += re[j]; s2 += (n & 1) ? -re[j] : re[j]; }
-    }
-    s1 = wave_sum(s1);
-    s2 = wave_sum(s2);
-    const float c = 1.0f / (float)(FFT_N + win);
-    float* fo = frames + (size_t)frame * win;
-    if (n0 + 8 <= win && (win & 3) == 0) {
-        float o[8];
-#pragma unroll
-        for (int q = 0; q < 8; ++q) {
-            const int n = n0 + q;
-            const float corr = c * (s1 + ((n & 1) ? -s2 : s2));
-            o[q] = window[n] * (1.0f / 256.0f) * (u[q] - corr);
-        }
-        *reinterpret_cast<float4*>(fo + n0) = make_float4(o[0], o[1], o[2], o[3]);
-        *reinterpret_cast<float4*>(fo + n0 + 4) = make_float4(o[4], o[5], o[6], o[7]);
-        return;
-    }
-#pragma unroll
-    for (int q = 0; q < 8; ++q) {
-        const int n = n0 + q;
-        if (n < win) {
-            const float corr = c * (s1 + ((n & 1) ? -s2 : s2));
-            fo[n] = window[n] * (1.0f / 256.0f) * (u[q] - corr);
-        }
-    }
+    float o[8];
+    istft_frame(spec + (size_t)frame * NBIN, mask + (size_t)frame * 256, window, win, mode, lane, tw, o);
+    istft_store_frame(frames + (size_t)frame * win, o, lane, win);
 }
 
 __global__ __launch_bounds__(256) void istft_ola_kernel(const float* __restrict__ frames, const float* __restrict__ inv_coff,
@@ -129,33 +132,62 @@
     }
 }
 
-__global__ __launch_bounds__(256) void istft_bwd_kernel(const float* __restrict__ dwav, const float* __restrict__ wav,
-                                                        const float* __restrict__ inv_coff, const float* __restrict__ window,
-                                                        const float2* __restrict__ spec, const float2* __restrict__ mask,
-                                                        int B, int T, int win, int hop, int length, int mode,
-                                                        unsigned* __restrict__ dmask_bf16) {
-    const int lane = threadIdx.x & 63;
-    const int frame = blockIdx.x * 4 + (threadIdx.x >> 6);
-    if (frame >= B * T) return;
-    const int b = frame / T, t = frame - b * T;
+#define ISTFT_NF 16
+#define ISTFT_MAXK 8
+template <bool STORE>
+__global__ __launch_bounds__(256) void istft_fused_kernel(const float2* __restrict__ spec, const float2* __restrict__ mask,
+                                                          const float* __restrict__ window, const float* __restrict__ inv_coff, int T,
+                                                          int win, int hop, int length, int mode, int K, int hop0,
+                                                          float* __restrict__ frames, float* __restrict__ wav) {
+    __shared__ float sfr[ISTFT_NF][FFT_N];
+    const int lane = threadIdx.x & 63, w = threadIdx.x >> 6;
+    const int b = blockIdx.y;
+    const int G = ISTFT_NF - (K - 1);
+    const int h0 = hop0 + blockIdx.x * G;
+    const int tf0 = h0 - (K - 1);
+    FftTw tw;
+    fft_twiddles<1>(tw, lane);
+    const int n0 = 8 * brev6(lane);
+    for (int f = w; f < ISTFT_NF; f += 4) {
+        const int t = tf0 + f;
+        if (t < 0 || t >= T) continue;
+        const size_t frame = (size_t)b * T + t;
+        float o[8];
+        istft_frame(spec + frame * NBIN, mask + frame * 256, window, win, mode, lane, tw, o);
+        *reinterpret_cast<float4*>(&sfr[f][n0]) = make_float4(o[0], o[1], o[2], o[3]);
+        *reinterpret_cast<float4*>(&sfr[f][n0 + 4]) = make_float4(o[4], o[5], o[6], o[7]);
+        if (STORE && f >= K - 1) istft_store_frame(frames + frame * win, o, lane, win);
+    }
+    __syncthreads();
+    const int pad = win - hop;
+    const int s0 = h0 * hop;
+    for (int j = threadIdx.x; j < G * hop; j += 256) {
+        const int s = s0 + j, i = s - pad;
+        if (i < 0 || i >= length) continue;
+        int t_hi = s / hop;
+        int t_lo = (s - win + hop) / hop;
+        if (s - win + 1 <= 0) t_lo = 0;
+        if (t_hi > T - 1) t_hi = T - 1;
+        float acc = 0.f;
+        for (int t = t_lo; t <= t_hi; ++t) acc += sfr[t - tf0][s - t * hop];
+        acc *= inv_coff[i];
+        wav[(size_t)b * length + i] = fminf(1.f, fmaxf(-1.f, acc));
+    }
+}
+
+__device__ __forceinline__ void istft_bwd_rows(const float2* __restrict__ sp, const float2* __restrict__ mk, int lane, float2 (&spv)[4],
+                                               float2 (&mkv)[4]) {
+#pragma unroll
+    for (int j = 0; j < 4; ++j) { spv[j] = sp[1 + lane + 64 * j]; mkv[j] = mk[lane + 64 * j]; }
+}
+
+__device__ __forceinline__ void istft_bwd_frame(float (&re)[8], float s1, float s2, const float2 (&spv)[4], const float2 (&mkv)[4],
+                                                int lane, int w, int win, int mode, unsigned* __restrict__ dm) {
     FftTw tw;
     fft_twiddles<-1>(tw, lane);
-    const int pad = win - hop;
-    float re[8], im[8];
-    float s1 = 0.f, s2 = 0.f;
-#pragma unroll
-    for (int r = 0; r < 8; ++r) {
-        const int n = lane + 64 * r;
-        const int i = t * hop + n - pad;
-        float v = 0.f;
-        if (n < win && i >= 0 && i < length) {
-            const size_t o = (size_t)b * length + i;
-            const float y = wav[o];
-            if (y > -1.f && y < 1.f) v = dwav[o] * inv_coff[i] * window[n] * (1.0f / 256.0f);
-        }
-        re[r] = v; im[r] = 0.f;
-        s1 += v; s2 += (n & 1) ? -v : v;
-    }
+    float im[8];
+#pragma unroll
+    for (int r = 0; r < 8; ++r) im[r] = 0.f;
     s1 = wave_sum(s1);
     s2 = wave_sum(s2);
     const float c = 1.0f / (float)(FFT_N + win);
@@ -164,15 +196,9 @@
         const int n = lane + 64 * r;
         if (n < win) re[r] -= c * (s1 + ((n & 1) ? -s2 : s2));
     }
-    const float2* sp = spec + (size_t)frame * NBIN;
-    const float2* mk = mask + (size_t)frame * 256;
-    float2 spv[4], mkv[4];
-#pragma unroll
-    for (int j = 0; j < 4; ++j) { spv[j] = sp[1 + lane + 64 * j]; mkv[j] = mk[lane + 64 * j]; }
     fft512_wave<-1>(re, im, tw, lane);
     __shared__ float2 ssp[4][256 + 32], smk[4][256 + 32];
     __shared__ unsigned sdm[4][256];
-    const int w = threadIdx.x >> 6;
 #pragma unroll
     for (int j = 0; j < 4; ++j) {
         const int i = lane + 64 * j;
@@ -201,8 +227,79 @@
     __builtin_amdgcn_fence(__ATOMIC_RELEASE, "wavefront");
     __builtin_amdgcn_wave_barrier();
     __builtin_amdgcn_fence(__ATOMIC_ACQUIRE, "wavefront");
-    unsigned* dm = dmask_bf16 + (size_t)frame * 256;
     *reinterpret_cast<uint4*>(dm + 4 * lane) = *reinterpret_cast<const uint4*>(&sdm[w][4 * lane]);
+}
+
+__global__ __launch_bounds__(256) void istft_bwd_kernel(const float* __restrict__ dwav, const float* __restrict__ wav,
+                                                        const float* __restrict__ inv_coff, const float* __restrict__ window,
+                                                        const float2* __restrict__ spec, const float2* __restrict__ mask,
+                                                        int B, int T, int win, int hop, int length, int mode,
+                                                        unsigned* __restrict__ dmask_bf16) {
+    const int lane = threadIdx.x & 63;
+    const int frame = blockIdx.x * 4 + (threadIdx.x >> 6);
+    if (frame >= B * T) return;
+    const int b = frame / T, t = frame - b * T;
+    const int pad = win - hop;
+    float2 spv[4], mkv[4];
+    istft_bwd_rows(spec + (size_t)frame * NBIN, mask + (size_t)frame * 256, lane, spv, mkv);
+    float re[8];
+    float s1 = 0.f, s2 = 0.f;
+#pragma unroll
+    for (int r = 0; r < 8; ++r) {
+        const int n = lane + 64 * r;
+        const int i = t * hop + n - pad;
+        float v = 0.f;
+        if (n < win && i >= 0 && i < length) {
+            const size_t o = (size_t)b * length + i;
+            const float y = wav[o];
+            if (y > -1.f && y < 1.f) v = dwav[o] * inv_coff[i] * window[n] * (1.0f / 256.0f);
+        }
+        re[r] = v;
+        s1 += v; s2 += (n & 1) ? -v : v;
+    }
+    istft_bwd_frame(re, s1, s2, spv, mkv, lane, threadIdx.x >> 6, win, mode, dmask_bf16 + (size_t)frame * 256);
+}
+
+__global__ __launch_bounds__(256) void sisnr_istft_bwd_kernel(const float* __restrict__ wav, const float* __restrict__ ref,
+                                                              const float4* __restrict__ rowstat, const float* __restrict__ upstream,
+                                                              const float* __restrict__ inv_coff, const float* __restrict__ window,
+                                                              const float2* __restrict__ spec, const float2* __restrict__ mask,
+                                                              int T, int win, int hop, int length, int mode,
+                                                              unsigned* __restrict__ dmask_bf16) {
+    __shared__ float span[4 * FFT_N];
+    const int lane = threadIdx.x & 63, w = threadIdx.x >> 6;
+    const int b = blockIdx.y, t0 = blockIdx.x * 4;
+    const float4 st = rowstat[b];
+    const float up = upstream ? upstream[0] : 1.f;
+    const float a = st.x * up, bb = st.y * up, alpha = st.w;
+    const int t = t0 + w;
+    const size_t frame = (size_t)b * T + t;
+    float2 spv[4], mkv[4];
+    if (t < T) istft_bwd_rows(spec + frame * NBIN, mask + frame * 256, lane, spv, mkv);
+    const int i0 = t0 * hop - (win - hop);
+    const size_t base = (size_t)b * length;
+    for (int j = threadIdx.x; j < win + 3 * hop; j += 256) {
+        const int i = i0 + j;
+        float v = 0.f;
+        if (i >= 0 && i < length) {
+            const float y = wav[base + i];
+            if (y > -1.f && y < 1.f) v = sisnr_grad(y, ref[base + i], a, bb, alpha) * inv_coff[i];
+        }
+        span[j] = v;
+    }
+    __syncthreads();
+    if (t >= T) return;
+    float re[8];
+    float s1 = 0.f, s2 = 0.f;
+#pragma unroll
+    for (int r = 0; r < 8; ++r) {
+        const int n = lane + 64 * r;
+        float v = 0.f;
+        if (n < win) v = span[w * hop + n] * window[n] * (1.0f / 256.0f);
+        re[r] = v;
+        s1 += v; s2 += (n & 1) ? -v : v;
+    }
+    istft_bwd_frame(re, s1, s2, spv, mkv, lane, w, win, mode, dmask_bf16 + frame * 256);
 }
 
 static int check_stft_cfg(const char* who, int win, int hop, int fft) {
@@ -234,6 +331,23 @@
     SEHIP_REQUIRE(mode >= 0 && mode <= 2, "istft_fwd: masking mode must be 0(E) 1(C) 2(R)");
     SEHIP_REQUIRE(length <= (T - 1) * hop + win - (win - hop), "istft_fwd: length %d exceeds the synthesised signal", length);
     hipStream_t st = (hipStream_t)stream;
+    const int K = cdiv(win, hop);
+    if (K <= ISTFT_MAXK) {
+        const int G = ISTFT_NF - (K - 1), pad = win - hop;
+        const int hop0 = frames_ws ? 0 : pad / hop;
+        int hops = (pad + length - 1) / hop + 1 - hop0;
+        if (frames_ws && hops < T) hops = T;
+        dim3 grid(cdiv(hops, G), B);
+        if (frames_ws)
+            istft_fused_kernel<true><<<grid, 256, 0, st>>>((const float2*)spec, (const float2*)mask, window, inv_coff, T, win, hop,
+                                                           length, mode, K, hop0, frames_ws, wav);
+        else
+            istft_fused_kernel<false><<<grid, 256, 0, st>>>((const float2*)spec, (const float2*)mask, window, inv_coff, T, win, hop,
+                                                            length, mode, K, hop0, nullptr, wav);
+        SEHIP_CHECK_LAUNCH("istft_fwd");
+        return 0;
+    }
+    SEHIP_REQUIRE(frames_ws, "istft_fwd: win %d / hop %d needs the frames workspace (ceil(win / hop) > %d)", win, hop, ISTFT_MAXK);
     istft_frames_kernel<<<cdiv((long)B * T, 4), 256, 0, st>>>((const float2*)spec, (const float2*)mask, window, B * T, win,
                                                              mode, frames_ws);
     dim3 grid(cdiv(length, 256 * 4), B);
@@ -254,3 +368,18 @@
     SEHIP_CHECK_LAUNCH("istft_bwd");
     return 0;
 }
+
+extern "C" int sehip_sisnr_istft_bwd(const float* wav, const float* ref, const float* rowstat, const float* upstream,
+                                     const float* spec, const float* mask, const float* window, const float* inv_coff, int B, int T,
+                                     int win, int hop, int fft, int length, int mode, void* dmask_bf16, void* stream) {
+    if (int e = check_stft_cfg("sisnr_istft_bwd", win, hop, fft)) return e;
+    SEHIP_REQUIRE(B > 0 && T > 0 && length > 0, "sisnr_istft_bwd: empty input");
+    SEHIP_REQUIRE(mode >= 0 && mode <= 2, "sisnr_istft_bwd: masking mode must be 0(E) 1(C) 2(R)");
+    SEHIP_REQUIRE(B <= 65535, "sisnr_istft_bwd: B=%d exceeds the grid's y extent", B);
+    SEHIP_REQUIRE(wav && ref && rowstat && spec && mask && window && inv_coff && dmask_bf16, "sisnr_istft_bwd: null pointer");
+    sisnr_istft_bwd_kernel<<<dim3(cdiv(T, 4), B), 256, 0, (hipStream_t)stream>>>(wav, ref, (const float4*)rowstat, upstream, inv_coff,
+                                                                                window, (const float2*)spec, (const float2*)mask, T,
+                                                                                win, hop, length, mode, (unsigned*)dmask_bf16);
+    SEHIP_CHECK_LAUNCH("sisnr_istft_bwd");
+    return 0;
+}
diff --git a/speech-enhancement-pytorch_amd/sehip/model/dccrn.py b/speech-enhancement-pytorch_amd/sehip/model/dccrn.py
--- a/speech-enhancement-pytorch_amd/sehip/model/dccrn.py
+++ b/speech-enhancement-pytorch_amd/sehip/model/dccrn.py
@@ -108,14 +108,36 @@
     def _output(self, ws, x):
         return ws.wav.view(x.shape[0], 1, -1).clone()
 
-    def _run_backward(self, ws, grad_out):
+    def _run_backward(self, ws, grad_out, loss_grad=None):
         if not self.training:
             raise SehipError("DCCRN.backward in eval mode (running-statistics BatchNorm) is not built")
-        g = grad_out.reshape(ws.B, ws.length).contiguous().float()
+        g = grad_out.reshape(ws.B, ws.length).contiguous().float() if loss_grad is None else None
         hook = self.grad_range_hook if not (self._grads_live and self._params[0][1].grad is not None) else None
         tail = self._tail_for_backward()
-        self._backward_into_flat(lambda dst: ws.backward(g, self._flat, dst, range_ready=hook, tail=tail))
+        self._backward_into_flat(lambda dst: ws.backward(g, self._flat, dst, range_ready=hook, tail=tail, loss_grad=loss_grad))
         self._tail_mark(tail)
+
+    def sisdr_step_applies(self, mixture, sources):
+        if not (self.training and torch.is_grad_enabled() and mixture.is_cuda and sources.is_cuda and mixture.dim() in (2, 3)):
+            return False
+        cfg, n = self.cfg, mixture.shape[-1]
+        frames = ops.stft_frames(n, cfg.win_len, cfg.win_inc)
+        if frames < 1 or mixture.numel() != mixture.shape[0] * n:
+            return False
+        return tuple(sources.shape) == (mixture.shape[0], 1, min(cfg.length, frames * cfg.win_inc))
+
+    def _loss_forward(self, ws, ref):
+        return ws.sisnr_loss(ref)
+
+    def sisdr_step(self, mixture, sources):
+        from .flat import _PlanLossFunction
+        if not self.sisdr_step_applies(mixture, sources):
+            raise SehipError(f"DCCRN.sisdr_step: needs train mode, grad mode, device tensors and sources shaped like the output "
+                             f"(mixture {tuple(mixture.shape)}, sources {tuple(sources.shape)})")
+        if mixture.dim() == 2:
+            mixture = mixture.unsqueeze(1)
+        ref = sources.reshape(sources.shape[0], sources.shape[-1]).contiguous().float()
+        return _PlanLossFunction.apply(self, mixture, ref, self._grad_anchor(mixture.device))
 
     def forward(self, inputs, lens=None):
         if inputs.dim() == 2:
diff --git a/speech-enhancement-pytorch_amd/sehip/model/flat.py b/speech-enhancement-pytorch_amd/sehip/model/flat.py
--- a/speech-enhancement-pytorch_amd/sehip/model/flat.py
+++ b/speech-enhancement-pytorch_amd/sehip/model/flat.py
@@ -39,6 +39,27 @@
         with stream_scope():
             ctx.model._run_backward(ctx.ws, grad_out)
         return None, None, None
+
+
+class _PlanLossFunction(torch.autograd.Function):
+
+    @staticmethod
+    def forward(ctx, model, x, ref, anchor):
+        ctx.model = model
+        ctx.ws = model._run_forward(x)
+        ctx.generation = ctx.ws.generation
+        loss, ctx.rowstat = model._loss_forward(ctx.ws, ref)
+        ctx.ref = ref
+        return loss.reshape(())
+
+    @staticmethod
+    def backward(ctx, grad_out):
+        if ctx.generation != ctx.ws.generation or ctx.ws.closed:
+            raise SehipError(f"{ctx.model.plan_name}.backward: the workspace of this forward was overwritten by a later forward of the same "
+                             "shape (or evicted); run backward before the next forward of that shape")
+        with stream_scope():
+            ctx.model._run_backward(ctx.ws, None, loss_grad=(ctx.ref, ctx.rowstat, grad_out.reshape(1).contiguous().float()))
+        return None, None, None, None
 
 
 class _EvalGuard(torch.autograd.Function):
diff --git a/speech-enhancement-pytorch_amd/sehip/plan.py b/speech-enhancement-pytorch_amd/sehip/plan.py
--- a/speech-enhancement-pytorch_amd/sehip/plan.py
+++ b/speech-enhancement-pytorch_amd/sehip/plan.py
@@ -653,8 +653,9 @@
         add("mask", T, F0, 2, dtype=torch.float32)
         add("dmask", T, F0, 2)
         self.spec = torch.empty(B, T, 257, 2, dtype=torch.float32, device=device)
-        self.frames = torch.empty(B, T, cfg.win_len, dtype=torch.float32, device=device)
+        self.frames = torch.empty(B, T, cfg.win_len, dtype=torch.float32, device=device) if -(-cfg.win_len // cfg.win_inc) > 8 else None
         self.wav = torch.empty(B, self.length, dtype=torch.float32, device=device)
+        self.loss_ticket = torch.zeros(1, dtype=torch.int32, device=device)
         self.inv_coff = torch.from_numpy(ops.inv_window_energy(cfg.win_len, cfg.win_inc, T, self.length, cfg.win_type)).to(device)
         self.gpack = torch.zeros(st.n_gpack, dtype=torch.float32, device=device)
         maxcr = max(cr for _, cr in st.bn)
@@ -1222,15 +1223,27 @@
              cfg.win_inc, cfg.fft_len, self.length, self.mode, ptr(self.frames), ptr(self.wav), stream())
         return self.wav
 
-    def backward(self, dwav, params, grads, range_ready=None, tail=None):
+    def sisnr_loss(self, ref):
+        rowstat = torch.empty(self.B, 4, dtype=torch.float32, device=self.device)
+        loss = torch.empty(1, dtype=torch.float32, device=self.device)
+        call("sehip_sisnr_fwd_fin", ptr(self.wav), ptr(ref), self.B, self.length, ptr(rowstat), ptr(self.loss_ticket), ptr(loss), stream())
+        return loss, rowstat
+
+    def backward(self, dwav, params, grads, range_ready=None, tail=None, loss_grad=None):
         st, cfg, b, tb = self.st, self.st.cfg, self.bufs, self.tb
         B, T, h = self.B, self.T, cfg.hid
         if not getattr(self, "_gpack_clean", False):
             self.gpack.zero_()
         self._gpack_clean = False
         self._chain_dirty = True
-        call("sehip_istft_bwd", ptr(dwav), ptr(self.wav), ptr(self.spec), b["mask"].ptr, ptr(tb.window), ptr(self.inv_coff),
-             B, T, cfg.win_len, cfg.win_inc, cfg.fft_len, self.length, self.mode, b["dmask"].ptr, stream())
+        if loss_grad is not None:
+            ref, rowstat, upstream = loss_grad
+            call("sehip_sisnr_istft_bwd", ptr(self.wav), ptr(ref), ptr(rowstat), ptr(upstream), ptr(self.spec), b["mask"].ptr,
+                 ptr(tb.window), ptr(self.inv_coff), B, T, cfg.win_len, cfg.win_inc, cfg.fft_len, self.length, self.mode,
+                 b["dmask"].ptr, stream())
+        else:
+            call("sehip_istft_bwd", ptr(dwav), ptr(self.wav), ptr(self.spec), b["mask"].ptr, ptr(tb.window), ptr(self.inv_coff),
+                 B, T, cfg.win_len, cfg.win_inc, cfg.fft_len, self.length, self.mode, b["dmask"].ptr, stream())
         for j in range(5, -1, -1):
             if j < 5:
                 self.bn_backward(f"decoder.{j}.", cfg.kernel_num[5 - j] // 2, b[f"dzd{j}"], None, b[f"yd{j}"], b[f"dyd{j}"],
diff --git a/speech-enhancement-pytorch_amd/sehip/solver.py b/speech-enhancement-pytorch_amd/sehip/solver.py
--- a/speech-enhancement-pytorch_amd/sehip/solver.py
+++ b/speech-enhancement-pytorch_amd/sehip/solver.py
@@ -120,6 +120,7 @@
 
         self.optimizer = optimizer
         self.loss_function = loss_function
+        self.fused_turnaround = not os.environ.get("SEHIP_NO_FUSED_TURNAROUND")
         self.model = model.to(self.device)
         self.flat_model = hasattr(self.model, "flat_params")
         if self.world_size > 1:
@@ -318,11 +319,17 @@
             return pit_loss(enhanced, sources, self.loss_function)
         return self._loss(enhanced, sources, mixture)
 
+    def _forward_loss(self, mixture, sources):
+        from . import loss as loss_module
+        if self.fused_turnaround and hasattr(self.model, "sisdr_step") and self.loss_function is loss_module.loss_sisdr \
+                and not self._pit_applies(sources) and self.model.sisdr_step_applies(mixture, sources):
+            return self.model.sisdr_step(mixture, sources)
+        return self._step_loss(self.model(mixture), sources, mixture)
+
     def _train_step(self, mixture, sources):
         if not self.model.training:
             self.model.train()
-        enhanced = self.model(mixture)
-        loss = self._step_loss(enhanced, sources, mixture)
+        loss = self._forward_loss(mixture, sources)
         self.optimizer.zero_grad()
         fused = isinstance(self.optimizer, FlatOptimizer)
         works, early_guard = [], False
@@ -409,8 +416,7 @@
         torch.cuda.synchronize()
         fb, upd = torch.cuda.CUDAGraph(), torch.cuda.CUDAGraph()
         with torch.cuda.graph(fb):
-            enhanced = self.model(mix)
-            loss = self._step_loss(enhanced, src, mix)
+            loss = self._forward_loss(mix, src)
             self.optimizer.zero_grad()
             loss.backward()
             loss_out = loss.detach().clone()
```

Result: no change. 20190 audio-s/s, median of 2 (+0.0%).
